# swoonge/SC-A-LOAM

Measured on AMD Instinct MI355X. Metric: scans/sec (feat-extract + scan-to-map ICP + SC loop search), KITTI HDL-64, higher is better.
Workload: dtype f32 points / f64 pose algebra

## Files before the change

### sc-a-loam_amd/csrc/common.cpp

```cpp
#include "common.hpp"
#include <atomic>
#include <chrono>
#include <cstdlib>
#include <memory>

namespace scal {

thread_local Recorder* g_recorder = nullptr;
long g_forced_flushes = 0;
static std::mutex g_flush_mu;
static std::vector<std::pair<std::string, long>> g_flush_sites;
void note_forced_flush(const char* file, int line) {
    std::lock_guard<std::mutex> lk(g_flush_mu);
    ++g_forced_flushes;
    const std::string key = std::string(file) + ":" + std::to_string(line);
    for (auto& s : g_flush_sites)
        if (s.first == key) {
            ++s.second;
            return;
        }
    g_flush_sites.push_back({key, 1});
}
void print_forced_flushes() {
    std::lock_guard<std::mutex> lk(g_flush_mu);
    for (auto& s : g_flush_sites) std::fprintf(stderr, "[scal_pipeline] forced flush at %s x %ld\n", s.first.c_str(), s.second);
}

static hipError_t run_op(const RecOp& o) {
    if (o.kind != RecOp::LAUNCH) return o.replay();
    const void* one = o.pack;
    return o.fn(o.name, o.grid, o.block, o.lds, o.stream, 1, &one);
}

hipError_t Recorder::flush() {
    Recorder* keep = g_recorder;
    g_recorder = nullptr;
    hipError_t first = hipSuccess;
    for (const RecOp& o : ops) {
        const hipError_t e = run_op(o);
        if (first == hipSuccess) first = e;
    }
    ops.clear();
    g_recorder = keep;
    return first;
}

namespace {
const char* merged_name(const char* a, const char* b) {
    static std::mutex mu;
    static std::vector<std::unique_ptr<std::string>> pool;
    const char* dot = std::strrchr(b, '.');
    const std::string key = std::string(a) + "+" + (dot ? dot + 1 : b);
    std::lock_guard<std::mutex> lk(mu);
    for (auto& s : pool)
        if (*s == key) return s->c_str();
    pool.push_back(std::make_unique<std::string>(key));
    return pool.back()->c_str();
}
struct Span {
    Recorder* r;
    size_t b, e;
};
bool same_op(const RecOp& a, const RecOp& b) {
    if (a.kind != b.kind) return false;
    if (a.kind != RecOp::LAUNCH) return true;
    return a.fn == b.fn && a.grid.x == b.grid.x && a.grid.y == b.grid.y && a.block.x == b.block.x && a.lds == b.lds && a.stream == b.stream &&
           a.pack_size == b.pack_size;
}
hipError_t zip_spans(const std::vector<Span>& spans) {
    hipError_t first = hipSuccess;
    auto note = [&](hipError_t e) { if (first == hipSuccess) first = e; };
    const int n = static_cast<int>(spans.size());
    std::vector<bool> done(n, false);
    for (int i = 0; i < n; ++i) {
        if (done[i]) continue;
        const Span& lead = spans[i];
        const size_t len = lead.e - lead.b;
        std::vector<const Span*> group{&lead};
        done[i] = true;
        if (!lead.r->broken)
            for (int j = i + 1; j < n && static_cast<int>(group.size()) < BATCH_WIDE; ++j) {
                const Span& c = spans[j];
                if (done[j] || c.r->broken || c.e - c.b != len) continue;
                bool ok = true;
                for (size_t k = 0; k < len && ok; ++k) ok = same_op(lead.r->ops[lead.b + k], c.r->ops[c.b + k]);
                if (ok) group.push_back(&c), done[j] = true;
            }
        for (size_t k = 0; k < len; ++k) {
            const RecOp& o = lead.r->ops[lead.b + k];
            if (o.kind == RecOp::LAUNCH) {
                for (size_t g0 = 0; g0 < group.size(); g0 += static_cast<size_t>(o.cap)) {
                    const size_t g1 = std::min(group.size(), g0 + static_cast<size_t>(o.cap));
                    const void* packs[BATCH_WIDE];
                    const char* name = o.name;
                    for (size_t g = g0; g < g1; ++g) {
                        const RecOp& og = group[g]->r->ops[group[g]->b + k];
                        packs[g - g0] = og.pack;
                        if (g > g0 && std::strcmp(og.name, o.name) != 0 && !std::strstr(name, "+")) name = merged_name(o.name, og.name);
                    }
                    note(o.fn(name, o.grid, o.block, o.lds, o.stream, static_cast<int>(g1 - g0), packs));
                }
            } else {
                for (const Span* g : group) note(g->r->ops[g->b + k].replay());
            }
        }
    }
    return first;
}
}

hipError_t zip_and_launch(Recorder* const* recs, int n) {
    Recorder* keep = g_recorder;
    g_recorder = nullptr;
    std::vector<Span> spans;
    for (int i = 0; i < n; ++i) spans.push_back({recs[i], 0, recs[i]->ops.size()});
    const hipError_t e = zip_spans(spans);
    for (int i = 0; i < n; ++i) recs[i]->ops.clear(), recs[i]->broken = false;
    g_recorder = keep;
    return e;
}

hipError_t zip_marked_and_launch(Recorder* const* recs, int n) {
    Recorder* keep = g_recorder;
    g_recorder = nullptr;
    std::vector<Span> before, seg, after;
    for (int i = 0; i < n; ++i) {
        Recorder* r = recs[i];
        size_t b = r->ops.size(), e = r->ops.size();
        for (size_t k = 0; k < r->ops.size(); ++k)
            if (r->ops[k].kind == RecOp::MARK_BEGIN) {
                b = k;
                break;
            }
        for (size_t k = b; k < r->ops.size(); ++k)
            if (r->ops[k].kind == RecOp::MARK_END) {
                e = k + 1;
                break;
            }
        if (r->broken || b == r->ops.size()) {
            before.push_back({r, 0, r->ops.size()});
            continue;
        }
        before.push_back({r, 0, b});
        seg.push_back({r, b, e});
        after.push_back({r, e, r->ops.size()});
    }
    hipError_t first = zip_spans(before);
    hipError_t e2 = zip_spans(seg);
    hipError_t e3 = zip_spans(after);
    if (first == hipSuccess) first = e2 != hipSuccess ? e2 : e3;
    for (int i = 0; i < n; ++i) recs[i]->ops.clear(), recs[i]->broken = false;
    g_recorder = keep;
    return first;
}

static thread_local char g_err[512] = "";

void set_error(const char* fmt, ...) {
    va_list ap;
    va_start(ap, fmt);
    vsnprintf(g_err, sizeof g_err, fmt, ap);
    va_end(ap);
}

int select_device(int device) {
    int n = 0;
    hipError_t e = hipGetDeviceCount(&n);
    if (e != hipSuccess || n <= 0) {
        set_error("no HIP device available (%s): libscaloam_hip has no CPU fallback", e == hipSuccess ? "count 0" : hipGetErrorString(e));
        return SCAL_E_NO_DEVICE;
    }
    if (device < 0 || device >= n) {
        set_error("device ordinal %d out of range (%d devices)", device, n);
        return SCAL_E_ARG;
    }
    hipDeviceProp_t prop;
    e = hipGetDeviceProperties(&prop, device);
    if (e != hipSuccess) {
        set_error("hipGetDeviceProperties failed: %s", hipGetErrorString(e));
        return SCAL_E_HIP;
    }
    if (std::strncmp(prop.gcnArchName, "gfx950", 6) != 0) {
        set_error("device %d is %s; this library carries gfx950 (MI355X) code objects only", device, prop.gcnArchName);
        return SCAL_E_NO_DEVICE;
    }
    e = hipSetDevice(device);
    if (e != hipSuccess) {
        set_error("hipSetDevice(%d) failed: %s", device, hipGetErrorString(e));
        return SCAL_E_HIP;
    }
    return SCAL_OK;
}

namespace {
std::mutex g_stream_mu;
struct DevStream {
    hipStream_t s = nullptr;
    int refs = 0;
};
DevStream g_streams[64][6];
std::atomic<int> g_stream_mode{0};

bool lane_has_own_queue(int lane) { return lane == 0 || lane == 1 || lane == 3 || lane == 4; }

hipStream_t own_queue_stream(int device) {
    int ncu = 0;
    if (hipDeviceGetAttribute(&ncu, hipDeviceAttributeMultiprocessorCount, device) != hipSuccess || ncu <= 0) return nullptr;
    std::vector<uint32_t> mask((ncu + 31) / 32, 0u);
    for (int cu = 0; cu < ncu; ++cu) mask[cu / 32] |= 1u << (cu % 32);
    hipStream_t s = nullptr;
    if (hipExtStreamCreateWithCUMask(&s, (uint32_t)mask.size(), mask.data()) != hipSuccess) {
        (void)hipGetLastError();
        return nullptr;
    }
    return s;
}
}

int acquire_stream(int device, hipStream_t* out, int lane) {
    if (device < 0 || device >= 64 || lane < 0 || lane > 5) {
        set_error("device ordinal %d out of range", device);
        return SCAL_E_ARG;
    }
    std::lock_guard<std::mutex> lk(g_stream_mu);
    DevStream& d = g_streams[device][lane];
    if (!d.s) {
        hipError_t e = hipSetDevice(device);
        if (e == hipSuccess && lane_has_own_queue(lane)) {
            d.s = own_queue_stream(device);
            if (!d.s) e = hipStreamCreateWithFlags(&d.s, hipStreamNonBlocking);
        } else if (e == hipSuccess) {
            e = hipStreamCreateWithFlags(&d.s, hipStreamNonBlocking);
        }
        if (e != hipSuccess) {
            set_error("hipStreamCreate failed: %s", hipGetErrorString(e));
            d.s = nullptr;
            return SCAL_E_HIP;
        }
    }
    d.refs++;
    *out = d.s;
    return SCAL_OK;
}

StreamLayout default_stream_layout() { return g_stream_mode.load() ? StreamLayout::PerStage : StreamLayout::Shared; }

int stage_lane(StreamLayout layout, int stage) {
    if (layout == StreamLayout::Shared) return stage == STAGE_MAP_PREFETCH ? 2 : 0;
    return (stage == STAGE_ODOM || stage == STAGE_SC) ? 3 : stage == STAGE_MAP ? 4 : (stage == STAGE_SC_FILTER || stage == STAGE_MAP_PREFETCH) ? 1 : 0;
}

__global__ void k_queue_ptr(unsigned long long* out) { out[0] = reinterpret_cast<unsigned long long>(__builtin_amdgcn_queue_ptr()); }

int lane_queue(int device, int lane, unsigned long long* out) {
    if (!out || device < 0 || device >= 64 || lane < -1 || lane > 5) {
        set_error("lane_queue: bad argument (device %d, lane %d)", device, lane);
        return SCAL_E_ARG;
    }
    hipStream_t s = nullptr;
    if (lane >= 0) {
        std::lock_guard<std::mutex> lk(g_stream_mu);
        DevStream& d = g_streams[device][lane];
        if (!d.s) {
            set_error("lane_queue: no context holds lane %d of device %d", lane, device);
            return SCAL_E_STATE;
        }
        d.refs++;
        s = d.s;
    }
    unsigned long long* dq = nullptr;
    hipError_t e = hipSetDevice(device);
    if (e == hipSuccess) e = hipMalloc(&dq, sizeof *dq);
    if (e == hipSuccess) {
        hipLaunchKernelGGL(k_queue_ptr, dim3(1), dim3(1), 0, s, dq);
        e = hipGetLastError();
    }
    if (e == hipSuccess) e = hipMemcpyAsync(out, dq, sizeof *dq, hipMemcpyDeviceToHost, s);
    if (e == hipSuccess) e = hipStreamSynchronize(s);
    if (dq) (void)hipFree(dq);
    if (lane >= 0) release_stream(device, lane);
    if (e != hipSuccess) {
        set_error("lane_queue: %s", hipGetErrorString(e));
        return SCAL_E_HIP;
    }
    return SCAL_OK;
}

void release_stream(int device, int lane) {
    if (device < 0 || device >= 64 || lane < 0 || lane > 5) return;
    std::lock_guard<std::mutex> lk(g_stream_mu);
    DevStream& d = g_streams[device][lane];
    if (d.refs > 0 && --d.refs == 0 && d.s) {
        (void)hipSetDevice(device);
        (void)hipStreamSynchronize(d.s);
        (void)hipStreamDestroy(d.s);
        d.s = nullptr;
    }
}

namespace {
struct ProfEntry {
    std::string name;
    std::vector<std::pair<hipEvent_t, hipEvent_t>> pending;
    std::vector<const void*> pending_tl;
    double total_ms = 0;
    long count = 0;
};
std::mutex g_prof_mu;
std::vector<ProfEntry> g_prof;
std::vector<hipEvent_t> g_event_pool;
bool g_prof_on = false;
std::string g_prof_filter;
struct TimelineRow {
    std::string name;
    float t0, t1;
    const void* stream;
};
bool g_timeline_on = false;
hipEvent_t g_timeline_base = nullptr;
std::vector<TimelineRow> g_timeline;

hipEvent_t take_event() {
    if (!g_event_pool.empty()) {
        hipEvent_t e = g_event_pool.back();
        g_event_pool.pop_back();
        return e;
    }
    hipEvent_t e = nullptr;
    (void)hipEventCreate(&e);
    return e;
}
void drain_entry(ProfEntry& p);
void drain_locked() {
    for (auto& p : g_prof) drain_entry(p);
}
void drain_entry(ProfEntry& p) {
    {
        for (size_t q = 0; q < p.pending.size(); ++q) {
            auto& ev = p.pending[q];
            float ms = 0.f;
            if (hipEventSynchronize(ev.second) == hipSuccess && hipEventElapsedTime(&ms, ev.first, ev.second) == hipSuccess) {
                p.total_ms += ms;
                p.count++;
                float a = 0.f;
                if (p.pending_tl[q] && g_timeline_base && hipEventElapsedTime(&a, g_timeline_base, ev.first) == hipSuccess)
                    g_timeline.push_back({p.name, a, a + ms, p.pending_tl[q]});
            }
            g_event_pool.push_back(ev.first);
            g_event_pool.push_back(ev.second);
        }
        p.pending.clear();
        p.pending_tl.clear();
    }
}
}

bool prof_begin(const char* name, hipStream_t stream, hipEvent_t* start, hipEvent_t* stop) {
    static const int delay_us = [] {
        const char* e = std::getenv("SCALOAM_HOST_DELAY_US");
        return e ? std::atoi(e) : 0;
    }();
    if (delay_us > 0) {
        const auto t0 = std::chrono::steady_clock::now();
        while (std::chrono::duration_cast<std::chrono::microseconds>(std::chrono::steady_clock::now() - t0).count() < delay_us) {
        }
    }
    if (!g_prof_on) return false;
    std::lock_guard<std::mutex> lk(g_prof_mu);
    if (!g_prof_filter.empty()) {
        const std::string f = "," + g_prof_filter + ",";
        if (f.find("," + std::string(name) + ",") == std::string::npos) return false;
    }
    int slot = -1;
    for (size_t i = 0; i < g_prof.size(); ++i)
        if (g_prof[i].name == name) slot = static_cast<int>(i);
    if (slot < 0) {
        g_prof.push_back(ProfEntry());
        g_prof.back().name = name;
        slot = static_cast<int>(g_prof.size()) - 1;
    }
    if (g_prof[slot].pending.size() >= 64) drain_entry(g_prof[slot]);
    hipEvent_t a = take_event(), b = take_event();
    if (!a || !b) return false;
    g_prof[slot].pending.push_back({a, b});
    g_prof[slot].pending_tl.push_back(g_timeline_on ? (stream ? static_cast<const void*>(stream) : static_cast<const void*>(&g_timeline_on)) : nullptr);
    *start = a, *stop = b;
    return true;
}

}

extern "C" int scal_prof_enable(int on) {
    std::lock_guard<std::mutex> lk(scal::g_prof_mu);
    scal::g_prof_on = on != 0;
    return SCAL_OK;
}
extern "C" int scal_prof_timeline(int on) {
    std::lock_guard<std::mutex> lk(scal::g_prof_mu);
    if (on && !scal::g_timeline_base) {
        if (hipEventCreate(&scal::g_timeline_base) != hipSuccess) return SCAL_E_HIP;
        if (hipEventRecord(scal::g_timeline_base, nullptr) != hipSuccess) return SCAL_E_HIP;
        if (hipEventSynchronize(scal::g_timeline_base) != hipSuccess) return SCAL_E_HIP;
    }
    scal::g_timeline_on = on != 0;
    return SCAL_OK;
}
extern "C" int scal_prof_timeline_dump(const char* path) {
    std::lock_guard<std::mutex> lk(scal::g_prof_mu);
    scal::drain_locked();
    FILE* f = std::fopen(path, "w");
    if (!f) return SCAL_E_ARG;
    for (auto& r : scal::g_timeline) std::fprintf(f, "%s,%.6f,%.6f,%p\n", r.name.c_str(), r.t0, r.t1, r.stream);
    std::fclose(f);
    scal::g_timeline.clear();
    return SCAL_OK;
}
extern "C" int scal_prof_filter(const char* kernel_name) {
    std::lock_guard<std::mutex> lk(scal::g_prof_mu);
    scal::g_prof_filter = kernel_name ? kernel_name : "";
    return SCAL_OK;
}
extern "C" int scal_prof_reset(void) {
    std::lock_guard<std::mutex> lk(scal::g_prof_mu);
    scal::drain_locked();
    for (auto& p : scal::g_prof) p.total_ms = 0, p.count = 0;
    return SCAL_OK;
}
extern "C" int scal_prof_read(const char* name, double* total_ms, long* count) {
    std::lock_guard<std::mutex> lk(scal::g_prof_mu);
    scal::drain_locked();
    for (auto& p : scal::g_prof)
        if (p.name == name) {
            if (total_ms) *total_ms = p.total_ms;
            if (count) *count = p.count;
            return SCAL_OK;
        }
    if (total_ms) *total_ms = 0;
    if (count) *count = 0;
    return SCAL_OK;
}
extern "C" int scal_prof_names(char* buf, int cap) {
    std::lock_guard<std::mutex> lk(scal::g_prof_mu);
    std::string all;
    for (auto& p : scal::g_prof) all += p.name + ";";
    if (buf && cap > 0) {
        std::strncpy(buf, all.c_str(), cap - 1);
        buf[cap - 1] = 0;
    }
    return static_cast<int>(all.size());
}

extern "C" int scal_set_stream_mode(int mode) {
    if (mode != 0 && mode != 1) {
        scal::set_error("scal_set_stream_mode: mode must be 0 or 1");
        return SCAL_E_ARG;
    }
    scal::g_stream_mode = mode;
    return SCAL_OK;
}

extern "C" int scal_debug_lane_queue(int device, int lane, unsigned long long* queue) { return scal::lane_queue(device, lane, queue); }

extern "C" const char* scal_last_error(void) { return scal::g_err; }
extern "C" int scal_device_count(void) {
    int n = 0;
    if (hipGetDeviceCount(&n) != hipSuccess) return -1;
    return n;
}
extern "C" const char* scal_version(void) { return "scaloam_hip 0.1 (gfx950)"; }
```

### sc-a-loam_amd/csrc/common.hpp

```cpp
#pragma once
#include <hip/hip_runtime.h>
#include <hip/hip_ext.h>
#include <cstdio>
#include <cstdarg>
#include <cstring>
#include <string>
#include <vector>
#include <utility>
#include <mutex>
#include "../../include/scaloam_hip.h"
#include "batch.hpp"

namespace scal {
constexpr unsigned EV_DEVICE_ONLY = hipEventDisableTiming | hipEventDisableSystemFence;


void set_error(const char* fmt, ...);

#define SCAL_HIP(expr)                                                                         \
    do {                                                                                       \
        hipError_t _e = (expr);                                                                \
        if (_e != hipSuccess) {                                                                \
            ::scal::set_error("%s failed: %s (%s:%d)", #expr, hipGetErrorString(_e), __FILE__, __LINE__); \
            return SCAL_E_HIP;                                                                 \
        }                                                                                      \
    } while (0)

#define SCAL_TRY(expr)           \
    do {                         \
        int _rc = (expr);        \
        if (_rc != SCAL_OK) return _rc; \
    } while (0)

int select_device(int device);
enum class StreamLayout { Shared, PerStage };
enum { STAGE_FEATURES = 0, STAGE_SC = 1, STAGE_ODOM = 3, STAGE_MAP = 4, STAGE_MAP_PREFETCH = 2, STAGE_SC_FILTER = 5 };
int stage_lane(StreamLayout layout, int stage);
StreamLayout default_stream_layout();
int acquire_stream(int device, hipStream_t* out, int lane = 0);
void release_stream(int device, int lane = 0);
int odom_create(const scal_odom_config* cfg, StreamLayout layout, scal_odom_t** out);
int map_create(const scal_map_config* cfg, StreamLayout layout, scal_map_t** out);
int sc_create(const scal_sc_config* cfg, StreamLayout layout, scal_sc_t** out);
int icp_create_on_lane(const scal_icp_config* cfg, int lane, scal_icp_t** out);
int refine_create_on_lane(const scal_refine_config* cfg, int lane, scal_refine_t** out);
int posegraph_create_on_lane(const scal_posegraph_config* cfg, int lane, scal_posegraph_t** out);
struct ScFilterOut {
    const float *x, *y, *z, *w;
    const int* d_n;
    int cap;
};
int sc_insert_features_then(scal_sc_t* ctx, scal_features_t* feat, int (*after)(void* user, hipStream_t s, const ScFilterOut& ds), void* user);

struct LaneStream {
    hipStream_t s = nullptr;
    int device = 0, lane = 0;
    LaneStream() = default;
    LaneStream(LaneStream&& o) noexcept { *this = std::move(o); }
    LaneStream& operator=(LaneStream&& o) noexcept {
        release();
        std::swap(s, o.s);
        device = o.device, lane = o.lane;
        return *this;
    }
    ~LaneStream() { release(); }
    operator hipStream_t() const { return s; }
    int acquire(int dev, int ln) {
        release();
        device = dev, lane = ln;
        return acquire_stream(dev, &s, ln);
    }
    void release() {
        if (s) release_stream(device, lane);
        s = nullptr;
    }
};
struct Event {
    hipEvent_t e = nullptr;
    Event() = default;
    Event(Event&& o) noexcept { *this = std::move(o); }
    Event& operator=(Event&& o) noexcept {
        reset();
        std::swap(e, o.e);
        return *this;
    }
    ~Event() { reset(); }
    operator hipEvent_t() const { return e; }
    int create(unsigned flags) {
        reset();
        return ensure(flags);
    }
    int ensure(unsigned flags) {
        const hipError_t r = e ? hipSuccess : hipEventCreateWithFlags(&e, flags);
        if (r == hipSuccess) return SCAL_OK;
        set_error("hipEventCreateWithFlags failed: %s", hipGetErrorString(r));
        e = nullptr;
        return SCAL_E_HIP;
    }
    void reset() {
        if (e) (void)hipEventDestroy(e);
        e = nullptr;
    }
};

template <class T>
struct DevBuf {
    T* p = nullptr;
    size_t n = 0;
    DevBuf() = default;
    DevBuf(const DevBuf&) = delete;
    DevBuf& operator=(const DevBuf&) = delete;
    ~DevBuf() { release(); }
    void release() {
        if (p) (void)hipFree(p);
        p = nullptr;
        n = 0;
    }
    int alloc(size_t count) {
        release();
        if (count == 0) count = 1;
        hipError_t e = hipMalloc(reinterpret_cast<void**>(&p), count * sizeof(T));
        if (e != hipSuccess) {
            set_error("hipMalloc(%zu bytes) failed: %s", count * sizeof(T), hipGetErrorString(e));
            p = nullptr;
            return SCAL_E_HIP;
        }
        n = count;
        return SCAL_OK;
    }
    int zero(hipStream_t s) {
        hipError_t e = op_memset_async(p, 0, n * sizeof(T), s);
        if (e != hipSuccess) {
            set_error("hipMemsetAsync failed: %s", hipGetErrorString(e));
            return SCAL_E_HIP;
        }
        return SCAL_OK;
    }
};

template <class T>
struct PinBuf {
    T* p = nullptr;
    size_t n = 0;
    PinBuf() = default;
    PinBuf(const PinBuf&) = delete;
    PinBuf& operator=(const PinBuf&) = delete;
    ~PinBuf() {
        if (p) (void)hipHostFree(p);
    }
    int alloc(size_t count) {
        if (p) (void)hipHostFree(p);
        p = nullptr;
        if (count == 0) count = 1;
        hipError_t e = hipHostMalloc(reinterpret_cast<void**>(&p), count * sizeof(T), hipHostMallocDefault);
        if (e != hipSuccess) {
            set_error("hipHostMalloc(%zu bytes) failed: %s", count * sizeof(T), hipGetErrorString(e));
            p = nullptr;
            return SCAL_E_HIP;
        }
        n = count;
        return SCAL_OK;
    }
};

inline int div_up(int a, int b) { return (a + b - 1) / b; }

struct HostStage {
    PinBuf<unsigned char> pin;
    size_t used = 0;
    struct Item {
        void* dst;
        size_t off, bytes;
    };
    std::vector<Item> items;
    bool reserve(size_t total) {
        if (pin.p && pin.n >= total) return true;
        if (used) return false;
        if (pin.alloc(total) != SCAL_OK) {
            (void)hipGetLastError();
            return false;
        }
        return true;
    }
    hipError_t d2h(void* user, const void* dev, size_t bytes, hipStream_t s) {
        if (!bytes) return hipSuccess;
        const size_t need = (bytes + 255) & ~static_cast<size_t>(255);
        if (!pin.p || used + need > pin.n) return hipMemcpyAsync(user, dev, bytes, hipMemcpyDeviceToHost, s);
        const hipError_t e = hipMemcpyAsync(pin.p + used, dev, bytes, hipMemcpyDeviceToHost, s);
        items.push_back({user, used, bytes});
        used += need;
        return e;
    }
    hipError_t h2d(void* dev, const void* user, size_t bytes, hipStream_t s) {
        if (!bytes) return hipSuccess;
        const size_t need = (bytes + 255) & ~static_cast<size_t>(255);
        if (!pin.p || used + need > pin.n) return hipMemcpyAsync(dev, user, bytes, hipMemcpyHostToDevice, s);
        std::memcpy(pin.p + used, user, bytes);
        const hipError_t e = hipMemcpyAsync(dev, pin.p + used, bytes, hipMemcpyHostToDevice, s);
        used += need;
        return e;
    }
    void finish() {
        for (const Item& it : items) std::memcpy(it.dst, pin.p + it.off, it.bytes);
        items.clear();
        used = 0;
    }
};

bool prof_begin(const char* name, hipStream_t stream, hipEvent_t* start, hipEvent_t* stop);

#define SCAL_LAUNCH_PROF(name, kernel, grid, block, lds, stream, ...)                                   \
    do {                                                                                                \
        hipEvent_t pe0_ = nullptr, pe1_ = nullptr;                                                      \
        if (::scal::prof_begin(name, stream, &pe0_, &pe1_))                                                     \
            hipExtLaunchKernelGGL(kernel, grid, block, lds, stream, pe0_, pe1_, 0, __VA_ARGS__);        \
        else                                                                                            \
            hipLaunchKernelGGL(kernel, grid, block, lds, stream, __VA_ARGS__);                          \
    } while (0)

}
```

### sc-a-loam_amd/csrc/mapping.hip

```cpp
#include "common.hpp"
#include <mutex>
#include <atomic>
#include "device_utils.hpp"
#include "voxel_dev.hpp"
#include "radix_sort.hpp"
#include "lm_host.hpp"
#include "features_dev.hpp"
#include <cmath>
#include <cstdlib>
#include <algorithm>
#include <deque>

namespace scal {

constexpr int CW = 21, CH = 21, CD = 11;
constexpr int GX = 250, GY = 250, GZ = 150;
constexpr int GCELLS = GX * GY * GZ;
constexpr unsigned long long MAP_NOMERGE = 127ull;

struct MapParams {
    int cenW, cenH, cenD;
    int cI, cJ, cK;
    int ox, oy, oz;
    float inv_line, inv_plane;
// ... 1016 lines not shown
            int cnt = 1;
            if (!key_nomerge(k)) {
                bool run = true;
#pragma unroll
                for (int j = 0; j < 8; ++j)
                    if (j >= cn) {
                        run = run && (e[j] >> MERGE_IDX_BITS) == k;
                        if (run) {
                            const int jn = static_cast<int>(e[j] & (MERGE_MAX - 1));
                            ax += nw.x[jn], ay += nw.y[jn], az += nw.z[jn], aw += nw.w[jn];
                            ++cnt;
                        }
                    }
                if (run) {
                    int u = lo + 8;
                    while (u < n_eff && (nw.sorted[u] >> MERGE_IDX_BITS) == k) {
                        const int jn = static_cast<int>(nw.sorted[u] & (MERGE_MAX - 1));
                        ax += nw.x[jn], ay += nw.y[jn], az += nw.z[jn], aw += nw.w[jn];
                        ++u, ++cnt;
                    }
                }
            }
            const float c = static_cast<float>(cnt);
            const float ox = ax / c, oy = ay / c, oz = az / c;
            out.x[o] = ox, out.y[o] = oy, out.z[o] = oz, out.w[o] = aw / c, out.cube[o] = cube;
            if (a.prebuild) prebuild(o, ox, oy, oz, cube, k);
        }
    } else {
        const int i = b * 256 + threadIdx.x;
        if (i < n_eff && (nw.hm[i] & 3) == 1) {
            const unsigned long long k = nw.sorted[i] >> MERGE_IDX_BITS;
            const int o = nw.lb[i] + pre_at(i);
            float ax = 0.f, ay = 0.f, az = 0.f, aw = 0.f;
            int u = i;
            do {
                const int j = static_cast<int>(nw.sorted[u] & (MERGE_MAX - 1));
                ax += nw.x[j], ay += nw.y[j], az += nw.z[j], aw += nw.w[j];
                ++u;
            } while (!key_nomerge(k) && u < n_eff && (nw.sorted[u] >> MERGE_IDX_BITS) == k);
            const float c = static_cast<float>(u - i);
            const int cube = nw.cube[static_cast<int>(nw.sorted[i] & (MERGE_MAX - 1))];
            const float ox = ax / c, oy = ay / c, oz = az / c;
            out.x[o] = ox, out.y[o] = oy, out.z[o] = oz, out.w[o] = aw / c;
            out.cube[o] = cube;
            if (a.prebuild) prebuild(o, ox, oy, oz, cube, k);
        }
    }
    if (!a.prebuild) return;
    if (drifted) S->next_unsorted = 1;
    if (over) S->next_over = 1;
    for (int o = 32; o >= 1; o >>= 1) n_in += __shfl_xor(n_in, o, 64);
    if (lane_id() == 0 && n_in) atomicAdd(&s_valid, n_in);
    __syncthreads();
    if (threadIdx.x == 0 && s_valid) atomicAdd(&S->next_valid[cls], s_valid);
}

struct MapResult {
    LMState st;
    MapCounters C1, C2;
    MapState S1, S2;
    unsigned seq_pose, seq_done;
};

struct MergeTail {
    int fused;
    unsigned seq;
    CSoA4 full;
    const int* d_nfull;
    int full_cap;
    const LMState* st;
    SoA4 full_out;
};
__device__ __forceinline__ void k_merge_write_body(const MergeArgs& a, MapState* S, MapCounters* C, const MergeTail& t) {
    merge_write_body(a, S, C);
    if (!t.fused) return;
    if (static_cast<int>(blockIdx.x) >= MERGE_WRITE_GRID && S->pose_seq == t.seq) {
        const int i = (blockIdx.x - MERGE_WRITE_GRID) * 256 + threadIdx.x;
        if (i < min(*t.d_nfull, t.full_cap)) {
            double x7[7];
#pragma unroll
            for (int k = 0; k < 7; ++k) x7[k] = t.st->x[k];
            float sel[3];
            associate_to_map(x7, t.full.x[i], t.full.y[i], t.full.z[i], sel);
            t.full_out.x[i] = sel[0], t.full_out.y[i] = sel[1], t.full_out.z[i] = sel[2], t.full_out.w[i] = t.full.w[i];
        }
    }
}
SCAL_KERNEL(256, k_merge_write)

__device__ __forceinline__ void k_transform_cloud_body(const CSoA4& in, const int* __restrict__ d_n, int cap, const LMState* __restrict__ st,
                                                         const MapState* __restrict__ S, const SoA4& out) {
    if (S->abort) return;
    const int i = blockIdx.x * blockDim.x + threadIdx.x;
    if (i >= min(*d_n, cap)) return;
    double x7[7];
#pragma unroll
    for (int k = 0; k < 7; ++k) x7[k] = st->x[k];
    float sel[3];
    associate_to_map(x7, in.x[i], in.y[i], in.z[i], sel);
    out.x[i] = sel[0], out.y[i] = sel[1], out.z[i] = sel[2], out.w[i] = in.w[i];
}
SCAL_KERNEL(256, k_transform_cloud)

__device__ __forceinline__ void k_map_gather_body(const float* __restrict__ less_aos, const int* __restrict__ d_n_less, const CSoA4& less_flat,
                                                    const int* __restrict__ d_n_less_flat, const SoA4& corner_in, const SoA4& surf_in, MapCounters* C, int cap,
                                                    int nbc, unsigned* surf_parts) {
    const bool corner = static_cast<int>(blockIdx.x) < nbc;
    const int b = corner ? blockIdx.x : blockIdx.x - nbc;
    const int n = min(corner ? *d_n_less : *d_n_less_flat, cap);
    const int i = b * 256 + threadIdx.x;
    if (blockIdx.x == 0) {
        int* w = reinterpret_cast<int*>(C);
        for (int t = 2 + threadIdx.x; t < static_cast<int>(sizeof(MapCounters) / sizeof(int)); t += 256) w[t] = 0;
    }
    if (i == 0) (corner ? C->n_corner_in : C->n_surf_in) = n;
    if (corner) {
        if (i >= n) return;
        const float4 p = reinterpret_cast<const float4*>(less_aos)[i];
        corner_in.x[i] = p.x, corner_in.y[i] = p.y, corner_in.z[i] = p.z, corner_in.w[i] = p.w;
    } else {
        float x = 0.f, y = 0.f, z = 0.f;
        if (i < n) {
            x = less_flat.x[i], y = less_flat.y[i], z = less_flat.z[i];
            surf_in.x[i] = x, surf_in.y[i] = y, surf_in.z[i] = z, surf_in.w[i] = less_flat.w[i];
        }
        if (surf_parts) vox_bbox_block_store(surf_parts, b, i < n, x, y, z);
    }
}
SCAL_KERNEL(256, k_map_gather)

__device__ __forceinline__ void k_export_valid_body(const MapCloud& m, const MapState* __restrict__ S, int cls, int* __restrict__ counter,
                                                      float* __restrict__ out, int cap) {
    const MapParams mp = S->mp;
    const int n = S->n_map[cls];
    for (int i = blockIdx.x * blockDim.x + threadIdx.x; i < n; i += gridDim.x * blockDim.x)
        if (cube_valid(mp, m.cube[i])) {
            const int p = atomicAdd(counter, 1);
            if (p < cap) reinterpret_cast<float4*>(out)[p] = make_float4(m.x[i], m.y[i], m.z[i], m.w[i]);
        }
}
SCAL_KERNEL(256, k_export_valid)


__device__ __forceinline__ void copy_words(void* dst, const void* src, int bytes) {
    const unsigned* s = static_cast<const unsigned*>(src);
    unsigned* d = static_cast<unsigned*>(dst);
    for (int i = threadIdx.x; i < bytes / 4; i += blockDim.x) d[i] = s[i];
}

struct PoseDoneNew {
    CSoA4 stack[2];
    const int* d_ns[2];
    float inv_leaf[2];
    float *x[2], *y[2], *z[2], *w[2];
    int* cube[2];
    unsigned long long* pkey[2];
};
struct MapPoseDone {
    int active;
    unsigned seq;
    MapState* S;
    const LMState* st;
    MapCounters* C;
    MapResult* host;
    PoseDoneNew nw;
    __device__ __forceinline__ void operator()(const double* x, int first, int stride, bool aborted) const {
        if (!active) return;
        const bool stop = aborted || S->abort;
        if (!stop) {
            const MapParams mp = S->mp;
            double x7[7];
#pragma unroll
            for (int k = 0; k < 7; ++k) x7[k] = x[k];
#pragma unroll
            for (int cls = 0; cls < 2; ++cls) {
                const int n_new = min(*nw.d_ns[cls], MERGE_MAX);
                const CSoA4 stack = nw.stack[cls];
                for (int i = first; i < n_new; i += stride) {
                    float sel[3];
                    associate_to_map(x7, stack.x[i], stack.y[i], stack.z[i], sel);
                    const int pc = pack_cube(cube_abs(sel[0]), cube_abs(sel[1]), cube_abs(sel[2]));
                    const unsigned long long k = map_key(mp, nw.inv_leaf[cls], sel[0], sel[1], sel[2], pc, C);
                    nw.x[cls][i] = sel[0], nw.y[cls][i] = sel[1], nw.z[cls][i] = sel[2], nw.w[cls][i] = stack.w[i], nw.cube[cls][i] = pc;
                    nw.pkey[cls][i] = k == ~0ull ? ~0ull : ((k << MERGE_IDX_BITS) | static_cast<unsigned long long>(i));
                }
            }
        }
        if (blockIdx.x != 0) return;
        if (first == 0 && !stop) {
            const double* q_wodom = S->q_wodom;
            const double n2 = q_wodom[0] * q_wodom[0] + q_wodom[1] * q_wodom[1] + q_wodom[2] * q_wodom[2] + q_wodom[3] * q_wodom[3];
            const double qi[4] = {-q_wodom[0] / n2, -q_wodom[1] / n2, -q_wodom[2] / n2, q_wodom[3] / n2};
            double qn[4];
            q_mul(x, qi, qn);
            double r2[3];
            q_rot(qn, S->t_wodom, r2);
#pragma unroll
            for (int i = 0; i < 4; ++i) S->q_wmap_wodom[i] = qn[i];
#pragma unroll
            for (int i = 0; i < 3; ++i) S->t_wmap_wodom[i] = x[4 + i] - r2[i];
            S->pose_seq = seq;
        }
        __syncthreads();
        copy_words(&host->st, st, sizeof(LMState));
        copy_words(&host->C1, C, sizeof(MapCounters));
        copy_words(&host->S1, S, sizeof(MapState));
        __threadfence_system();
        __syncthreads();
        if (threadIdx.x == 0) __hip_atomic_store(&host->seq_pose, seq, __ATOMIC_RELEASE, __HIP_MEMORY_SCOPE_SYSTEM);
    }
    __device__ __forceinline__ void operator()(int, int, int) const {}
};

__device__ __forceinline__ void k_map_pose_done_body(const MapPoseDone& pd) {
    pd(pd.st->x, blockIdx.x * blockDim.x + threadIdx.x, gridDim.x * blockDim.x, false);
}
SCAL_KERNEL(256, k_map_pose_done)

__device__ __forceinline__ void k_map_end_body(MapState* S, const MapCounters* C, MapResult* host, unsigned seq) {
    if (threadIdx.x == 0 && !S->abort) S->n_map[0] = C->n_map_new[0], S->n_map[1] = C->n_map_new[1];
    __syncthreads();
    copy_words(&host->C2, C, sizeof(MapCounters));
    copy_words(&host->S2, S, sizeof(MapState));
    __threadfence_system();
    __syncthreads();
    if (threadIdx.x == 0) __hip_atomic_store(&host->seq_done, seq, __ATOMIC_RELEASE, __HIP_MEMORY_SCOPE_SYSTEM);
}
SCAL_KERNEL(256, k_map_end)

struct MapStore {
    SoAStore pts[2];
    DevBuf<int> cube[2];
    int n = 0;
    MapCloud cloud(int b) { return MapCloud{pts[b].x.p, pts[b].y.p, pts[b].z.p, pts[b].w.p, cube[b].p}; }
};

struct GridStore {
    DevBuf<int2> cell[2];
    DevBuf<int> rank[2];
    DevBuf<float4> g;
    DevBuf<float4> fixed[2];
    DevBuf<unsigned long long> okeys[2];
    int fixed_cap = 0;
    GridPts pts(int par, bool fixed_pool = false) { return GridPts{fixed_pool ? fixed[par].p : g.p}; }
};

SCAL_DEFINE_STAMP_READER(scal_debug_stamps_map)
}

using namespace scal;

int voxels_per_cell_axis(float leaf) {
    const double inv = 1.0 / static_cast<double>(leaf);
    int most = 1;
    for (int c = 0; c < 1000; ++c) {
        const int lo = static_cast<int>(std::floor(c * inv + 1e-4)), hi = static_cast<int>(std::floor((c + 1) * inv - 1e-4));
        most = std::max(most, hi - lo + 1);
    }
    return most;
}


struct MapStep {
    scal_features_t* feat = nullptr;
    MapPoseIn pose{};
    int set = 0;
    int slot = 0;
    int par = 0;
    bool prefetched = false, have_full = false, fast = false;
    bool pose_collected = false;
    bool confirmed = false;
    bool failed = false;
    bool prebuilt = false;
    unsigned seq = 0;
    unsigned feat_generation = 0;
    int n_corner_bound = 0, n_surf_bound = 0;
    int insert_path = 0;
};

struct InputSet {
    SoAStore in[2], stack[2];
    DevBuf<MapCounters> C;
    DevBuf<unsigned> surf_parts;
    Event ev_pre;
    Event ev_pre_a;
    int* n_in(int k) const { return k == 0 ? &C.p->n_corner_in : &C.p->n_surf_in; }
    int* n_stack(int k) const { return k == 0 ? &C.p->n_corner_stack : &C.p->n_surf_stack; }
};

template <class T, int N>
struct Fifo {
    T item[N];
    int n = 0;
    void push(const T& v) { item[n++] = v; }
    const T& front() const { return item[0]; }
    void pop() { std::copy(item + 1, item + n, item), --n; }
    void clear() { n = 0; }
};

struct scal_map {
    scal_map_config cfg;
    LaneStream stream;
    LaneStream side;
    static constexpr int NSETS = 8;
    static constexpr int MAX_STEPS = 4;
    static constexpr int MAX_PF = 3;
    static constexpr int NSLOTS = MAX_STEPS + 1;
    struct Prefetch {
        scal_features_t* feat;
        int set;
        unsigned generation;
    };
    std::mutex pf_mu;
    Fifo<Prefetch, MAX_PF> pf_half;
    Fifo<Prefetch, MAX_PF> pf;
    int next_set = 0;
    std::deque<MapStep> steps;
    Event ev_pose[NSLOTS], ev_done[NSLOTS];
    int next_slot = 0;
    PinBuf<MapResult> res;
    bool adapter_active = false;
    MapStep adapter_step;
    BlockAdapter blocks;
    int n_fast = 0, n_general = 0, n_recover_pose = 0, n_recover_insert = 0;
    bool poll_on_enqueue = true;
    int cur = 0;
    bool initialised = false;
    double good_q[4] = {0, 0, 0, 1}, good_t[3] = {0, 0, 0};
    int scan_cap = 0, map_cap = 0;
    double q_wmap_wodom[4] = {0, 0, 0, 1}, t_wmap_wodom[3] = {0, 0, 0};
    bool have_mp = false;
    DevBuf<MapState> d_S;
    DevBuf<float> aos;
    DevBuf<float> export_buf;
    InputSet sets[NSETS];
    SoAStore full_in, full_out;
    float leaf(int k) const { return k == 0 ? cfg.line_res : cfg.plane_res; }
    float inv_leaf(int k) const { return 1.0f / leaf(k); }
    VoxelFilter vf, vf_side, vf_corner;
    MapStore map[2];
    GridStore grid[2];
    HostStage hs_reg;
    bool grid_fixed = false;
    unsigned seq_counter = 0;
    bool grid_prebuilt = false;
    int grid_cap_now[2] = {0, 0};
    RadixSort sorter;
    DevBuf<unsigned long long> keys;
    DevBuf<int> vals, blockcnt;
    bool merge_insert = true;
    int last_insert_path = 0;
    SoAStore mnew[2];
    DevBuf<int> mcube[2], mpre[2], mlb[2], mblocktot[2];
    DevBuf<unsigned long long> msorted[2], mpkey[2], msamp[2];
    DevBuf<unsigned char> mhm[2];
    MergeNew merge_new(int k) {
        return MergeNew{mnew[k].x.p, mnew[k].y.p, mnew[k].z.p, mnew[k].w.p, mcube[k].p, mpkey[k].p, msorted[k].p, msamp[k].p, mpre[k].p, mlb[k].p, mhm[k].p, mblocktot[k].p};
    }
    LMStore lm;
    DevBuf<float> nnrec;
    NNBuf nnbuf() { return NNBuf{nnrec.p, lm.slot_cap}; }
    DevBuf<int> d_nfull;
    PinBuf<MapCounters> h_C;
    PinBuf<MapState> h_S;
    PinBuf<int> h_misc;
    int alloc_set() {
        const int st = next_set;
        next_set = (next_set + 1) % NSETS;
        return st;
    }
};

int scal::map_create(const scal_map_config* cfg, StreamLayout layout, scal_map_t** out) {
    if (!cfg || !out || cfg->max_scan_points <= 0 || cfg->max_map_points <= 0 || !(cfg->line_res > 0) || !(cfg->plane_res > 0)) {
        set_error("scal_map_create: bad argument");
        return SCAL_E_ARG;
    }
    if (cfg->line_res < 0.11f || cfg->plane_res < 0.11f) {
        set_error("mapping resolutions below 0.11 m exceed the 512 voxel/cube key layout");
        return SCAL_E_ARG;
    }
    *out = nullptr;
    SCAL_TRY(select_device(cfg->device));
    auto* c = new scal_map();
    c->cfg = *cfg;
    c->scan_cap = cfg->max_scan_points;
    c->map_cap = cfg->max_map_points;
    int rc = SCAL_OK;
    auto A = [&](int r) { if (rc == SCAL_OK) rc = r; };
    const size_t sc = c->scan_cap, mc = c->map_cap;
    A(c->aos.alloc(sc * 4));
    for (InputSet& I : c->sets) {
        A(I.in[0].alloc(sc)); A(I.in[1].alloc(sc)); A(I.stack[0].alloc(sc)); A(I.stack[1].alloc(sc));
        A(I.C.alloc(1));
        A(I.surf_parts.alloc((size_t)6 * (div_up(c->scan_cap, 256) + 1)));
    }
    A(c->full_in.alloc(sc)); A(c->full_out.alloc(sc));
    A(c->vf.init(c->scan_cap));
    A(c->vf_side.init(c->scan_cap));
    A(c->vf_corner.init(c->scan_cap));
    c->vf.set_tag(".C"), c->vf_side.set_tag(".C"), c->vf_corner.set_tag(".C");
    for (int k = 0; k < 2; ++k) {
        for (int b = 0; b < 2; ++b) {
            A(c->map[k].pts[b].alloc(mc));
            A(c->map[k].cube[b].alloc(mc));
        }
        for (int par = 0; par < 2; ++par) { A(c->grid[k].cell[par].alloc(GCELLS)); A(c->grid[k].rank[par].alloc(mc)); A(c->grid[k].okeys[par].alloc(mc)); }
        A(c->grid[k].g.alloc(mc));
    }
    A(c->sorter.init(c->map_cap));
    A(c->keys.alloc(mc)); A(c->vals.alloc(mc)); A(c->blockcnt.alloc(div_up(c->map_cap, 256) + 1));
    for (int k = 0; k < 2; ++k) {
        A(c->mnew[k].alloc(MERGE_MAX)); A(c->mcube[k].alloc(MERGE_MAX)); A(c->mpre[k].alloc(MERGE_MAX + 1)); A(c->mlb[k].alloc(MERGE_MAX));
        A(c->msorted[k].alloc(MERGE_MAX)); A(c->mhm[k].alloc(MERGE_MAX)); A(c->mblocktot[k].alloc(MERGE_CHUNKS));
        A(c->mpkey[k].alloc(MERGE_MAX)); A(c->msamp[k].alloc(MERGE_MAX / 8));
    }
    A(c->lm.alloc(c->scan_cap));
    A(c->nnrec.alloc(16 * sc));
    A(c->d_S.alloc(1)); A(c->d_nfull.alloc(4));
    A(c->blocks.alloc(c->scan_cap));
    A(c->h_C.alloc(1)); A(c->h_S.alloc(1)); A(c->h_misc.alloc(4)); A(c->res.alloc(scal_map::NSLOTS));
    const char* fixed_env = std::getenv("SCALOAM_MAP_FIXED_GRID");
    if (rc == SCAL_OK && !(fixed_env && fixed_env[0] == '0')) {
        int cap[2];
        for (int k = 0; k < 2; ++k) {
            const int a = voxels_per_cell_axis(c->leaf(k));
            cap[k] = a * a * a;
        }
        if (cap[0] + cap[1] <= 48) {
            c->grid_fixed = true;
            for (int k = 0; k < 2 && c->grid_fixed; ++k) {
                for (int par = 0; par < 2; ++par)
                    if (c->grid[k].fixed[par].alloc(static_cast<size_t>(GCELLS) * cap[k]) != SCAL_OK) c->grid_fixed = false;
                c->grid[k].fixed_cap = c->grid_cap_now[k] = cap[k];
            }
            if (!c->grid_fixed) {
                (void)hipGetLastError();
                for (int k = 0; k < 2; ++k) c->grid[k].fixed[0].release(), c->grid[k].fixed[1].release();
            }
        }
    }
    if (rc == SCAL_OK) std::memset(static_cast<void*>(c->res.p), 0, sizeof(MapResult) * scal_map::NSLOTS);
    if (rc == SCAL_OK) rc = lm_check_residency<AssocFit, MapPoseDone>(c->cfg.device);
    if (rc == SCAL_OK && hipFuncSetAttribute(reinterpret_cast<const void*>(k_merge_keys), hipFuncAttributeMaxDynamicSharedMemorySize,
                                             static_cast<int>(sizeof(unsigned long long) * MERGE_MAX)) != hipSuccess)
        rc = SCAL_E_HIP;
    if (rc == SCAL_OK) rc = c->stream.acquire(c->cfg.device, stage_lane(layout, STAGE_MAP));
    if (rc == SCAL_OK) rc = c->side.acquire(c->cfg.device, stage_lane(layout, STAGE_MAP_PREFETCH));
    for (int k = 0; k < scal_map::NSLOTS && rc == SCAL_OK; ++k) {
        rc = c->ev_pose[k].create(hipEventDisableTiming);
        if (rc == SCAL_OK) rc = c->ev_done[k].create(hipEventDisableTiming);
    }
    if (rc == SCAL_OK) {
        for (int k = 0; k < 4 && rc == SCAL_OK; ++k) rc = c->grid[k & 1].cell[k >> 1].zero(c->stream);
        if (rc == SCAL_OK) rc = c->lm.init(c->stream);
        MapState& H = *c->h_S.p;
        std::memset(&H, 0, sizeof H);
        H.q_wmap_wodom[3] = 1.0;
        H.mp.cenW = 10, H.mp.cenH = 10, H.mp.cenD = 5;
        if (rc == SCAL_OK && op_memcpy_async(c->d_S.p, c->h_S.p, sizeof(MapState), hipMemcpyHostToDevice, c->stream) != hipSuccess) rc = SCAL_E_HIP;
        if (rc == SCAL_OK && op_stream_synchronize(c->stream) != hipSuccess) rc = SCAL_E_HIP;
    }
    if (rc != SCAL_OK) {
        if (rc == SCAL_E_HIP) set_error("scal_map_create: HIP resource creation failed");
        delete c;
        return rc;
    }
    *out = c;
    return SCAL_OK;
}

extern "C" int scal_map_create(const scal_map_config* cfg, scal_map_t** out) { return map_create(cfg, default_stream_layout(), out); }

extern "C" void scal_map_destroy(scal_map_t* c) {
    if (!c) return;
    (void)hipSetDevice(c->cfg.device);
    if (c->stream) (void)op_stream_synchronize(c->stream);
    if (c->side) (void)op_stream_synchronize(c->side);
    delete c;
}

namespace {

void copy_pose(double* q, double* t, const double* q_from, const double* t_from) {
    std::copy(q_from, q_from + 4, q);
    std::copy(t_from, t_from + 3, t);
}

int enqueue_stack_filter(scal_map* c, int k, VoxelFilter& vf, hipStream_t s, int n_bound, int st, bool surf_box_done = false) {
    InputSet& I = c->sets[st];
    VoxTail t;
    t.err_out = &I.C.p->error;
    const int bits = c->leaf(k) >= 0.35f ? 30 : 40;
    const bool box = k == 1 && surf_box_done && n_bound > 8192;
    return vf.run(s, I.in[k].cv(), I.n_in(k), n_bound, c->leaf(k), bits, I.stack[k].v(), I.n_stack(k), &t, box ? I.surf_parts.p : nullptr,
                  box ? std::max(1, div_up(n_bound, 256)) : 0);
}

GridArgs grid_args(scal_map* c, int par, bool fixed_pool = false) {
    GridArgs ga;
    for (int k = 0; k < 2; ++k) {
        GridStore& G = c->grid[k];
        ga.m[k] = c->map[k].cloud(par);
        ga.cell[k] = G.cell[par].p, ga.rank[k] = G.rank[par].p, ga.g[k] = G.pts(par, fixed_pool);
        ga.okeys[k] = G.okeys[par].p;
        ga.inv_leaf[k] = c->inv_leaf(k);
    }
    return ga;
}

int insert_full_sort(scal_map* c, const MapStep& e, const int* n_map) {
    hipStream_t s = c->stream;
    const InputSet& I = c->sets[e.set];
    MapCounters* C = I.C.p;
    LMState* st = c->lm.d_st.p;
    for (int k = 0; k < 2; ++k) {
        MapStore& M = c->map[k];
        const int n_tot_max = std::min(c->map_cap, n_map[k] + c->scan_cap);
        const int nb = std::max(1, div_up(n_tot_max, 256));
        MapCloud in = M.cloud(e.par), outc = M.cloud(e.par ^ 1);
        SCAL_LAUNCH("k_insert_keys", k_insert_keys, dim3(nb), dim3(256), 0, s, in, c->d_S.p, I.stack[k].cv(), I.n_stack(k), st, c->inv_leaf(k),
                           c->map_cap, c->keys.p, c->vals.p, C, k);
        SortedPairs sp;
        SCAL_TRY(c->sorter.sort(s, c->keys.p, c->vals.p, &C->n_total[k], n_tot_max, 36, nullptr, &sp));
        SCAL_LAUNCH("k_map_heads", k_map_heads, dim3(nb), dim3(256), 0, s, sp, &C->n_total[k], c->blockcnt.p);
        launch_scan_inplace(s, c->blockcnt.p, &C->n_total[k], 256, 1, &C->n_map_new[k]);
        SCAL_LAUNCH("k_map_reduce", k_map_reduce, dim3(nb), dim3(256), 0, s, sp, &C->n_total[k], c->blockcnt.p, in, outc);
    }
    SCAL_HIP(hipGetLastError());
    return SCAL_OK;
}

struct FullCloud {
    CSoA4 pts;
    const int* d_n;
};
FullCloud full_cloud(scal_map* c, const MapStep& e) {
    if (!(e.have_full && e.feat)) return FullCloud{c->full_in.cv(), c->d_nfull.p};
    FeatDeviceView v = features_view(e.feat);
    return FullCloud{CSoA4{v.x, v.y, v.z, v.i}, &v.P->n_kept};
}

int launch_insert_merge(scal_map* c, const MapStep& e, bool fused = false) {
    hipStream_t s = c->stream;
    const InputSet& I = c->sets[e.set];
    MapCounters* C = I.C.p;
    MergeArgs a;
    for (int k = 0; k < 2; ++k) {
        MapStore& M = c->map[k];
        a.in[k] = M.cloud(e.par), a.out[k] = M.cloud(e.par ^ 1);
        a.stack[k] = I.stack[k].cv();
        a.d_ns[k] = I.n_stack(k);
        a.inv_leaf[k] = c->inv_leaf(k);
        GridStore& G = c->grid[k];
        a.okeys[k] = G.okeys[e.par].p;
        a.nw[k] = c->merge_new(k);
        a.grid_cell[k] = G.cell[e.par].p, a.grid_rank[k] = G.rank[e.par].p;
        a.next_cell[k] = G.cell[e.par ^ 1].p, a.next_rank[k] = G.rank[e.par ^ 1].p, a.next_pool[k] = G.fixed[e.par ^ 1].p;
        a.next_okeys[k] = G.okeys[e.par ^ 1].p, a.next_cap[k] = c->grid_cap_now[k];
    }
    a.prebuild = fused && c->grid_fixed ? 1 : 0;
    a.cap = c->map_cap;
    const int lds = sizeof(unsigned long long) * MERGE_MAX;
    if (!(fused && c->grid_fixed)) SCAL_LAUNCH("k_merge_okeys", k_merge_okeys, dim3(MERGE_KB0 + MERGE_KB1), dim3(1024), 0, s, a, c->d_S.p, C);
    SCAL_LAUNCH("k_merge_keys", k_merge_keys, dim3(MERGE_KEYS_GRID), dim3(1024), lds, s, a, c->lm.d_st.p, c->d_S.p, C);
    SCAL_LAUNCH("k_merge_lookup", k_merge_lookup, dim3(2 * MERGE_CHUNKS), dim3(512), 0, s, a, c->d_S.p, C);
    MergeTail t{};
    int grid = MERGE_WRITE_GRID;
    if (fused) {
        t.fused = 1, t.seq = e.seq, t.st = c->lm.d_st.p, t.full_out = c->full_out.v(), t.full_cap = c->scan_cap;
        const FullCloud f = full_cloud(c, e);
        t.full = f.pts, t.d_nfull = f.d_n;
        if (e.have_full) grid += std::max(1, div_up(c->scan_cap, 256));
        else t.full_cap = 0;
    }
    SCAL_LAUNCH("k_merge_write", k_merge_write, dim3(grid), dim3(256), 0, s, a, c->d_S.p, C, t);
    SCAL_HIP(hipGetLastError());
    return SCAL_OK;
}

void launch_grid_clear(scal_map* c, int par) {
    SCAL_LAUNCH("k_grid_clear", k_grid_clear, dim3(GRID_BLOCKS), dim3(256), 0, c->stream, grid_args(c, par), c->d_S.p);
}
int clear_abort(scal_map* c) {
    hipStream_t s = c->stream;
    SCAL_HIP(op_memset_async(&c->d_S.p->abort, 0, sizeof(int), s));
    return SCAL_OK;
}
void launch_map_end(scal_map* c, const MapStep& e) {
    SCAL_LAUNCH("k_map_end", k_map_end, dim3(1), dim3(256), 0, c->stream, c->d_S.p, c->sets[e.set].C.p, c->res.p + e.slot, e.seq);
}
bool stopped_before_pose(const MapResult& R) { return R.S1.abort || R.st.termination == 5; }
bool stopped_in_insertion(const MapResult& R) { return R.S2.abort != 0; }

int launch_tail(scal_map* c, const MapStep& e, bool registered = false) {
    hipStream_t s = c->stream;
    if (e.have_full && !registered) {
        const int nb = std::max(1, div_up(c->scan_cap, 256));
        const FullCloud f = full_cloud(c, e);
        SCAL_LAUNCH("k_transform_cloud", k_transform_cloud, dim3(nb), dim3(256), 0, s, f.pts, f.d_n, c->scan_cap, c->lm.d_st.p, c->d_S.p, c->full_out.v());
    }
    launch_map_end(c, e);
    SCAL_HIP(hipGetLastError());
    SCAL_HIP(op_event_record(c->ev_done[e.slot], s));
    if (e.feat && !registered) SCAL_TRY(features_note_reader(e.feat, s));
    return SCAL_OK;
}

MapPoseDone make_pose_done(scal_map* c, const MapStep& e) {
    const InputSet& I = c->sets[e.set];
    MapPoseDone pd;
    pd.active = 1, pd.seq = e.seq;
    pd.S = c->d_S.p, pd.st = c->lm.d_st.p, pd.C = I.C.p, pd.host = c->res.p + e.slot;
    for (int k = 0; k < 2; ++k) {
        pd.nw.stack[k] = I.stack[k].cv();
        pd.nw.d_ns[k] = I.n_stack(k);
        pd.nw.inv_leaf[k] = c->inv_leaf(k);
        pd.nw.x[k] = c->mnew[k].x.p, pd.nw.y[k] = c->mnew[k].y.p, pd.nw.z[k] = c->mnew[k].z.p, pd.nw.w[k] = c->mnew[k].w.p;
        pd.nw.cube[k] = c->mcube[k].p, pd.nw.pkey[k] = c->mpkey[k].p;
    }
    return pd;
}

int launch_pose_part(scal_map* c, const MapStep& e, bool prepare_only = false) {
    hipStream_t s = c->stream;
    const int st_ = e.set;
    InputSet& I = c->sets[st_];
    MapCounters* C = I.C.p;
    LMState* st = c->lm.d_st.p;
    MapState* S = c->d_S.p;
    if (e.feat) {
        if (e.prefetched) {
            SCAL_HIP(op_stream_wait_event(s, I.ev_pre, 0));
        } else {
            FeatDeviceView v = features_view(e.feat);
            SCAL_TRY(features_wait_done(e.feat, s));
            const int nbc = std::max(1, div_up(e.n_corner_bound, 256));
            SCAL_LAUNCH("k_map_gather", k_map_gather, dim3(nbc + std::max(1, div_up(e.n_surf_bound, 256))), dim3(256), 0, s, v.less_xyzi, &v.P->n_less_sharp,
                               CSoA4{v.lfx, v.lfy, v.lfz, v.lfi}, &v.P->n_less_flat, I.in[0].v(), I.in[1].v(), C, c->scan_cap, nbc,
                               static_cast<unsigned*>(nullptr));
        }
    }
    if (!e.prefetched) {
        SCAL_TRY(enqueue_stack_filter(c, 0, c->vf, s, e.n_corner_bound, st_));
        SCAL_TRY(enqueue_stack_filter(c, 1, c->vf, s, e.n_surf_bound, st_));
    }
    MapBeginArgs mb;
    mb.active = 0, mb.in = e.pose, mb.allow_window_change = e.fast ? 0 : 1, mb.inv_line = c->inv_leaf(0), mb.inv_plane = c->inv_leaf(1);
    mb.slot_cap = c->lm.slot_cap, mb.prebuilt = e.prebuilt ? 1 : 0, mb.S = S;
    const bool begin_in_knn = e.fast && e.prebuilt && c->grid_fixed && !prepare_only;
    if (!begin_in_knn) SCAL_LAUNCH("k_map_begin", k_map_begin, dim3(1), dim3(64), 0, s, mb, st, C);
    const bool fixed_pool = e.fast && c->grid_fixed && !prepare_only;
    const GridArgs ga = grid_args(c, e.par, fixed_pool);
    if (fixed_pool) {
        if (!e.prebuilt) SCAL_LAUNCH("k_grid_build", k_grid_build, dim3(GRID_BLOCKS), dim3(256), 0, s, ga, c->grid_cap_now[0], c->grid_cap_now[1], S, C);
    } else {
        SCAL_LAUNCH("k_grid_count", k_grid_count, dim3(GRID_BLOCKS), dim3(256), 0, s, ga, S, C);
        SCAL_LAUNCH("k_grid_alloc", k_grid_alloc, dim3(GRID_BLOCKS), dim3(256), 0, s, ga, S, C);
        SCAL_LAUNCH("k_grid_fill", k_grid_fill, dim3(GRID_BLOCKS), dim3(256), 0, s, ga, S);
    }
    if (prepare_only) {
        SCAL_HIP(hipGetLastError());
        return SCAL_OK;
    }
    FactorSoA F = c->lm.factors();
    const int assoc_blocks = std::max(1, std::min(3072, div_up(c->lm.slot_cap, 8)));
    MapPoseDone pd = make_pose_done(c, e);
    const AssocFit fit{I.stack[0].cv(), I.stack[1].cv(), c->nnbuf(), C, F};
    for (int outer = 0; outer < 2; ++outer) {
        {
            mb.active = (begin_in_knn && outer == 0) ? 1 : 0;
            SCAL_LAUNCH(mb.active ? "k_assoc_knn.0" : "k_assoc_knn", k_assoc_knn, dim3(assoc_blocks), dim3(256), 0, s, I.stack[0].cv(), I.stack[1].cv(), S,
                             c->grid[0].cell[e.par].p, c->grid[0].pts(e.par, fixed_pool), c->grid[1].cell[e.par].p, c->grid[1].pts(e.par, fixed_pool), st, C, c->nnbuf(), mb);
        }
        pd.active = outer == 1;
        launch_lm_solve(s, F, &C->n_slots, st, &C->solve_on, c->lm.partials.p, c->lm.lm_sync.p, outer, &S->abort, fit, pd, "k_lm_solve_map");
    }
    SCAL_HIP(hipGetLastError());
    if (!e.fast) SCAL_HIP(op_event_record(c->ev_pose[e.slot], s));
    return SCAL_OK;
}

static bool step_flag_set(const volatile unsigned* w, unsigned seq) {
    if (*w != seq) return false;
    std::atomic_thread_fence(std::memory_order_acquire);
    return true;
}
static int step_flag_wait(scal_map* c, const volatile unsigned* w, unsigned seq) {
    if (g_recorder) SCAL_HIP(op_flush_for_wait(__FILE__, __LINE__));
    for (unsigned spins = 0;; ++spins) {
        if (step_flag_set(w, seq)) return SCAL_OK;
        if ((spins & 0xfff) == 0xfff && hipStreamQuery(c->stream) == hipSuccess) {
            if (step_flag_set(w, seq)) return SCAL_OK;
            set_error("scal_map: the stream is idle and the step never reported (a kernel launch failed?)");
            return SCAL_E_HIP;
        }
        __builtin_ia32_pause();
    }
}
static int wait_pose(scal_map* c, const MapStep& e) {
    if (e.fast) return step_flag_wait(c, &c->res.p[e.slot].seq_pose, e.seq);
    SCAL_HIP(op_event_synchronize(c->ev_pose[e.slot]));
    return SCAL_OK;
}
static int wait_done(scal_map* c, const MapStep& e) {
    if (e.fast) return step_flag_wait(c, &c->res.p[e.slot].seq_done, e.seq);
    SCAL_HIP(op_event_synchronize(c->ev_done[e.slot]));
    return SCAL_OK;
}
static bool done_ready(scal_map* c, const MapStep& e) {
    if (e.fast) return step_flag_set(&c->res.p[e.slot].seq_done, e.seq);
    return op_event_query(c->ev_done[e.slot]) == hipSuccess;
}

int report_device_error(scal_map* c, int err) {
    set_error("scal_map_step: device capacity exceeded (map pool of %d points per class, or a voxel outside its cube)", c->map_cap);
    return err;
}

constexpr int MAP_RC_LM = 1000;
bool lm_gave_up(const MapResult& R) { return R.st.termination == 5 || R.S1.abort == MAP_ABORT_LM; }
int lm_reset(scal_map* c, bool restore_pose) {
    hipStream_t s = c->stream;
    SCAL_TRY(c->lm.clear_exchange(s));
    SCAL_TRY(clear_abort(c));
    if (restore_pose) {
        static_assert(offsetof(MapState, t_wmap_wodom) == offsetof(MapState, q_wmap_wodom) + 4 * sizeof(double), "pose fields are contiguous");
        SCAL_TRY(c->blocks.set_pose(s, c->d_S.p->q_wmap_wodom, c->good_q, c->good_t));
    }
    SCAL_HIP(op_stream_synchronize(s));
    return SCAL_OK;
}

int general_insert(scal_map* c, MapStep& e);
int drop_prebuilt_grid(scal_map* c) {
    if (!c->grid_prebuilt) return SCAL_OK;
    launch_grid_clear(c, c->cur);
    SCAL_HIP(hipGetLastError());
    c->grid_prebuilt = false;
    return SCAL_OK;
}
int run_general_once(scal_map* c, MapStep& e) {
    e.fast = false, e.prebuilt = false;
    e.par = c->cur;
    e.seq = ++c->seq_counter;
    SCAL_TRY(drop_prebuilt_grid(c));
    c->n_general++;
    SCAL_TRY(launch_pose_part(c, e));
    SCAL_HIP(op_event_synchronize(c->ev_pose[e.slot]));
    if (lm_gave_up(c->res.p[e.slot])) return MAP_RC_LM;
    return general_insert(c, e);
}
int run_general(scal_map* c, MapStep& e) {
    int rc = run_general_once(c, e);
    for (int attempt = 0; rc == MAP_RC_LM; ++attempt) {
        SCAL_TRY(lm_reset(c, true));
        launch_grid_clear(c, e.par);
        if (attempt == 1) {
            SCAL_HIP(op_stream_synchronize(c->stream));
            e.failed = true;
            set_error("LM solve abandoned: grid barrier timed out");
            return SCAL_E_HIP;
        }
        rc = run_general_once(c, e);
    }
    return rc;
}

int finish_step_sync(scal_map* c, MapStep& e, const int* n_map_before, bool registered) {
    if (n_map_before) {
        e.insert_path = 0;
        SCAL_TRY(insert_full_sort(c, e, n_map_before));
    }
    SCAL_TRY(launch_tail(c, e, registered));
    SCAL_HIP(op_event_synchronize(c->ev_done[e.slot]));
    const MapResult& R = c->res.p[e.slot];
    if (R.C2.error) return report_device_error(c, R.C2.error);
    c->cur = e.par ^ 1;
    return SCAL_OK;
}

// ... 68 lines not shown
}

int recover(scal_map* c) {
    hipStream_t s = c->stream;
    SCAL_HIP(op_stream_synchronize(s));
    size_t origin = 0;
    for (; origin < c->steps.size(); ++origin) {
        MapStep& f = c->steps[origin];
        if (f.confirmed) continue;
        const MapResult& Rf = c->res.p[f.slot];
        if (stopped_before_pose(Rf) || stopped_in_insertion(Rf)) break;
        if (Rf.C2.error) return report_device_error(c, Rf.C2.error);
        confirm(c, f);
    }
    if (origin == c->steps.size()) return SCAL_OK;
    MapStep& e = c->steps[origin];
    const MapResult& R = c->res.p[e.slot];
    trace_stop(R);
    c->cur = e.par;
    c->grid_prebuilt = false;
    bool dropped = false;
    if (stopped_before_pose(R)) {
        c->n_recover_pose++;
        const bool lm = lm_gave_up(R);
        if (lm) SCAL_TRY(lm_reset(c, true));
        else SCAL_TRY(clear_abort(c));
        if (lm || R.S1.abort == MAP_ABORT_GRID || e.prebuilt) launch_grid_clear(c, e.par);
        SCAL_TRY(check_generation(e, !e.prefetched));
        const int rc = run_general(c, e);
        if (rc != SCAL_OK && !e.failed) return rc;
        dropped = e.failed;
    } else {
        c->n_recover_insert++;
        const bool lm = R.S2.abort == MAP_ABORT_LM;
        if (lm) {
            SCAL_TRY(lm_reset(c, false));
            launch_grid_clear(c, e.par);
        } else {
            SCAL_TRY(clear_abort(c));
        }
        const bool registered = R.S2.pose_seq == e.seq;
        if (!registered) SCAL_TRY(check_generation(e, false));
        const int n_map[2] = {R.S2.n_map[0], R.S2.n_map[1]};
        e.fast = false;
        SCAL_TRY(finish_step_sync(c, e, n_map, registered));
    }
    if (dropped) e.confirmed = true;
    else confirm(c, e);
    for (size_t i = origin + 1; i < c->steps.size(); ++i) {
        SCAL_TRY(check_generation(c->steps[i], !c->steps[i].prefetched));
        SCAL_TRY(launch_fast(c, c->steps[i]));
    }
    return SCAL_OK;
}

int confirm_steps(scal_map* c, bool wait) {
    for (size_t i = 0; i < c->steps.size(); ++i) {
        if (c->steps[i].confirmed) continue;
        if (wait) {
            SCAL_TRY(wait_done(c, c->steps[i]));
        } else if (!done_ready(c, c->steps[i])) {
            break;
        }
        const MapResult& R = c->res.p[c->steps[i].slot];
        if (stopped_before_pose(R) || stopped_in_insertion(R)) {
            SCAL_TRY(recover(c));
            if (!c->steps[i].confirmed) {
                set_error("scal_map: internal error (recovery did not complete the stopped step)");
                return SCAL_E_STATE;
            }
            continue;
        }
        confirm(c, c->steps[i]);
        if (R.C2.error) return report_device_error(c, R.C2.error);
    }
    return SCAL_OK;
}
int map_settle(scal_map* c, bool wait) {
    SCAL_TRY(confirm_steps(c, wait));
    pop_done(c);
    return SCAL_OK;
}
int map_make_room(scal_map* c) {
    if (c->poll_on_enqueue) SCAL_TRY(map_settle(c, false));
    while (static_cast<int>(c->steps.size()) >= scal_map::MAX_STEPS) {
        if (!c->steps.front().pose_collected) {
            set_error("scal_map: %d steps are queued and not collected", scal_map::MAX_STEPS);
            return SCAL_E_STATE;
        }
        SCAL_TRY(wait_done(c, c->steps.front()));
        SCAL_TRY(map_settle(c, false));
    }
    return SCAL_OK;
}

MapStep new_step(scal_map* c) {
    MapStep e;
    e.slot = c->next_slot;
    c->next_slot = (c->next_slot + 1) % scal_map::NSLOTS;
    return e;
}

int run_general_and_confirm(scal_map* c, MapStep& e) {
    SCAL_TRY(run_general(c, e));
    c->steps.push_back(e);
    confirm(c, c->steps.back());
    return SCAL_OK;
}

int map_enqueue(scal_map* c, MapStep& e) {
    const int queued = static_cast<int>(c->steps.size()) + 1;
    const bool room = c->map[0].n + queued * MERGE_MAX <= c->map_cap && c->map[1].n + queued * MERGE_MAX <= c->map_cap;
    const bool fast = c->initialised && c->merge_insert && room && e.feat != nullptr;
    if (fast) {
        SCAL_TRY(launch_fast(c, e));
        c->steps.push_back(e);
        return SCAL_OK;
    }
    SCAL_TRY(map_settle(c, true));
    return run_general_and_confirm(c, e);
}

void stats_at_pose(const MapCounters& H, scal_map_stats* stats) {
    std::memset(stats, 0, sizeof *stats);
    stats->n_corner_stack = H.n_corner_stack, stats->n_surf_stack = H.n_surf_stack;
    stats->n_corner_map = H.n_valid[0], stats->n_surf_map = H.n_valid[1];
    stats->solved = H.solve_on;
}

void publish_correction(scal_map* c, const MapState& S1) {
    copy_pose(c->q_wmap_wodom, c->t_wmap_wodom, S1.q_wmap_wodom, S1.t_wmap_wodom);
    c->have_mp = true;
}

int map_collect_pose(scal_map* c, double* q_out, double* t_out, scal_map_stats* stats) {
    MapStep* pe = nullptr;
    for (auto& e : c->steps)
        if (!e.pose_collected) {
            pe = &e;
            break;
        }
    if (!pe) {
        set_error("scal_map_collect: no step enqueued");
        return SCAL_E_STATE;
    }
    const int slot = pe->slot;
    for (int round = 0;; ++round) {
        SCAL_TRY(wait_pose(c, *pe));
        if (pe->failed || !stopped_before_pose(c->res.p[slot])) break;
        if (round > scal_map::MAX_STEPS + 1) {
            set_error("scal_map_collect: internal error (recovery does not converge)");
            return SCAL_E_STATE;
        }
        SCAL_TRY(recover(c));
    }
    pe->pose_collected = true;
    const MapResult& R = c->res.p[slot];
    const MapCounters& H = R.C1;
    if (pe->failed) {
        pop_done(c);
        set_error("LM solve abandoned: grid barrier timed out");
        return SCAL_E_HIP;
    }
    if (H.error) return report_device_error(c, H.error);
    copy_pose(q_out, t_out, R.st.x, R.st.x + 4);
    publish_correction(c, R.S1);
    if (stats) {
        stats_at_pose(H, stats);
        for (int o = 0; o < 2; ++o) {
            const LMState& L = R.st;
            stats->n_edge[o] = H.solve_on ? L.log_n_edge[o] : 0, stats->n_plane[o] = H.solve_on ? L.log_n_plane[o] : 0;
            stats->lm_iters[o] = H.solve_on ? L.log_iters[o] : 0, stats->lm_success[o] = H.solve_on ? L.log_success[o] : 0;
            stats->cost_init[o] = H.solve_on ? L.log_cost_init[o] : 0.0, stats->cost_final[o] = H.solve_on ? L.log_cost_final[o] : 0.0;
        }
        stats->n_map_corner_total = R.S1.n_map[0], stats->n_map_surf_total = R.S1.n_map[1];
        stats->insert_path = -1;
    }
    pop_done(c);
    return SCAL_OK;
}

int check_host_arrays(const char* fn, const scal_map* c, const float* corner_last, int n_corner, const float* surf_last, int n_surf, int n_full,
                      const double* q_wodom, const double* t_wodom, const double* q_w_curr, const double* t_w_curr) {
    if (!c || !q_wodom || !t_wodom || !q_w_curr || !t_w_curr || n_corner < 0 || n_surf < 0 || n_full < 0 || (n_corner > 0 && !corner_last) ||
        (n_surf > 0 && !surf_last)) {
        set_error("%s: bad argument", fn);
        return SCAL_E_ARG;
    }
    if (n_corner > c->scan_cap || n_surf > c->scan_cap || n_full > c->scan_cap) {
        set_error("%s: input cloud larger than max_scan_points (%d)", fn, c->scan_cap);
        return SCAL_E_TOO_MANY;
    }
    return SCAL_OK;
}

void drop_prefetches(scal_map* c) { c->pf.clear(), c->pf_half.clear(); }

int begin_sync_step(scal_map* c, bool adapter_counts, const char* open_text, MapStep* e) {
    SCAL_HIP(hipSetDevice(c->cfg.device));
    SCAL_TRY(map_settle(c, true));
    if (!c->steps.empty() || (adapter_counts && c->adapter_active)) {
        set_error("%s", open_text);
        return SCAL_E_STATE;
    }
    *e = new_step(c);
    std::lock_guard<std::mutex> lk(c->pf_mu);
    drop_prefetches(c);
    e->set = c->alloc_set();
    return SCAL_OK;
}

int upload_step_inputs(scal_map* c, MapStep& e, const float* corner_last, int n_corner, const float* surf_last, int n_surf, const float* full_res,
                       int n_full) {
    hipStream_t s = c->stream;
    InputSet& I = c->sets[e.set];
    MapCounters z;
    std::memset(&z, 0, sizeof z);
    z.n_corner_in = n_corner, z.n_surf_in = n_surf;
    *c->h_C.p = z;
    SCAL_HIP(op_memcpy_async(I.C.p, c->h_C.p, sizeof(MapCounters), hipMemcpyHostToDevice, s));
    c->h_misc.p[0] = n_full;
    SCAL_HIP(op_memcpy_async(c->d_nfull.p, c->h_misc.p, sizeof(int), hipMemcpyHostToDevice, s));
    auto up = [&](const float* src, int n, SoAStore& dst) -> int {
        if (n > 0) {
            SCAL_HIP(op_memcpy_async(c->aos.p, src, sizeof(float) * 4 * n, hipMemcpyHostToDevice, s));
            launch_deinterleave(s, c->aos.p, n, dst.v());
            SCAL_HIP(op_stream_synchronize(s));
        }
        return SCAL_OK;
    };
    SCAL_TRY(up(corner_last, n_corner, I.in[0]));
    SCAL_TRY(up(surf_last, n_surf, I.in[1]));
    if (n_full > 0) SCAL_TRY(up(full_res, n_full, c->full_in));
    e.have_full = n_full > 0, e.n_corner_bound = n_corner, e.n_surf_bound = n_surf;
    return SCAL_OK;
}

int download_registered(scal_map* c, float* registered, int n_full) {
    hipStream_t s = c->stream;
    launch_interleave(s, c->d_nfull.p, n_full, c->full_out.cv(), c->aos.p);
    (void)c->hs_reg.reserve((size_t)c->scan_cap * 16 + 4096);
    SCAL_HIP(c->hs_reg.d2h(registered, c->aos.p, sizeof(float) * 4 * n_full, s));
    SCAL_HIP(op_stream_synchronize(s));
    c->hs_reg.finish();
    return SCAL_OK;
}

void stats_after_insertion(const scal_map* c, scal_map_stats* stats) {
    if (!stats) return;
    stats->n_map_corner_total = c->map[0].n, stats->n_map_surf_total = c->map[1].n;
    stats->insert_path = c->last_insert_path;
}

int need_adapter_step(const scal_map* c, const char* fn) {
    if (c->adapter_active) return SCAL_OK;
    set_error("%s: no scal_map_adapter_begin", fn);
    return SCAL_E_STATE;
}

int check_features_device(const scal_map* c, const FeatDeviceView& v) {
    if (v.device == c->cfg.device) return SCAL_OK;
    set_error("features context lives on device %d, map context on %d", v.device, c->cfg.device);
    return SCAL_E_ARG;
}

}

extern "C" int scal_map_step(scal_map_t* c, const float* corner_last, int n_corner, const float* surf_last, int n_surf, const float* full_res,
                             int n_full, const double* q_wodom, const double* t_wodom, double* q_w_curr, double* t_w_curr, float* registered,
                             scal_map_stats* stats) {
    SCAL_TRY(check_host_arrays("scal_map_step", c, corner_last, n_corner, surf_last, n_surf, n_full, q_wodom, t_wodom, q_w_curr, t_w_curr));
    const bool have_full = full_res != nullptr && n_full > 0;
    MapStep e;
    SCAL_TRY(begin_sync_step(c, false, "scal_map_step: a queued step has not been collected", &e));
    SCAL_TRY(upload_step_inputs(c, e, corner_last, n_corner, surf_last, n_surf, full_res, have_full ? n_full : 0));
    copy_pose(e.pose.q_wodom, e.pose.t_wodom, q_wodom, t_wodom);
    SCAL_TRY(run_general_and_confirm(c, e));
    SCAL_TRY(map_collect_pose(c, q_w_curr, t_w_curr, stats));
    SCAL_TRY(map_settle(c, true));
    stats_after_insertion(c, stats);
    if (have_full && registered) SCAL_TRY(download_registered(c, registered, n_full));
    return SCAL_OK;
}

extern "C" int scal_map_prefetch_begin(scal_map_t* c, scal_features_t* feat) {
    if (!c || !feat) {
        set_error("scal_map_prefetch_begin: null argument");
        return SCAL_E_ARG;
    }
    FeatDeviceView v = features_view(feat);
    SCAL_TRY(check_features_device(c, v));
    SCAL_HIP(hipSetDevice(c->cfg.device));
    const int ls_cap = std::min(c->scan_cap, v.n_scans * 120);
    const int cap = std::min(c->scan_cap, v.cap);
    std::lock_guard<std::mutex> lk(c->pf_mu);
    if (c->pf.n + c->pf_half.n >= scal_map::MAX_PF) {
        set_error("scal_map_prefetch_features: %d prefetches are already queued ahead of their steps", scal_map::MAX_PF);
        return SCAL_E_STATE;
    }
    const int nset = c->alloc_set();
    InputSet& I = c->sets[nset];
    SCAL_TRY(I.ev_pre.ensure(EV_DEVICE_ONLY));
    SCAL_TRY(I.ev_pre_a.ensure(EV_DEVICE_ONLY));
    hipStream_t sa = v.stream;
    const int nbc = std::max(1, div_up(ls_cap, 256));
    SCAL_LAUNCH("k_map_gather", k_map_gather, dim3(nbc + std::max(1, div_up(cap, 256))), dim3(256), 0, sa, v.less_xyzi, &v.P->n_less_sharp,
                     CSoA4{v.lfx, v.lfy, v.lfz, v.lfi}, &v.P->n_less_flat, I.in[0].v(), I.in[1].v(), I.C.p, c->scan_cap, nbc, I.surf_parts.p);
    SCAL_HIP(hipGetLastError());
    SCAL_TRY(enqueue_stack_filter(c, 0, c->vf_corner, sa, ls_cap, nset));
    SCAL_HIP(op_event_record(I.ev_pre_a, sa));
    c->pf_half.push(scal_map::Prefetch{feat, nset, v.generation});
    return SCAL_OK;
}

extern "C" int scal_map_prefetch_finish(scal_map_t* c, scal_features_t* feat) {
    if (!c || !feat) {
        set_error("scal_map_prefetch_finish: null argument");
        return SCAL_E_ARG;
    }
    SCAL_HIP(hipSetDevice(c->cfg.device));
    FeatDeviceView v = features_view(feat);
    const int cap = std::min(c->scan_cap, v.cap);
    std::lock_guard<std::mutex> lk(c->pf_mu);
    if (c->pf_half.n == 0 || c->pf_half.front().feat != feat) {
        set_error("scal_map_prefetch_finish: no scal_map_prefetch_begin of this features context is waiting (halves are finished in the order they were begun)");
        return SCAL_E_STATE;
    }
    const scal_map::Prefetch h = c->pf_half.front();
    c->pf_half.pop();
    InputSet& I = c->sets[h.set];
    SCAL_HIP(op_stream_wait_event(c->side, I.ev_pre_a, 0));
    SCAL_TRY(enqueue_stack_filter(c, 1, c->vf_side, c->side, cap, h.set, true));
    SCAL_HIP(op_event_record(I.ev_pre, c->side));
    c->pf.push(h);
    return SCAL_OK;
}

extern "C" int scal_map_prefetch_features(scal_map_t* c, scal_features_t* feat) {
    SCAL_TRY(scal_map_prefetch_begin(c, feat));
    return scal_map_prefetch_finish(c, feat);
}

static int map_enqueue_features(scal_map* c, scal_features_t* feat, const double* q_wodom, const double* t_wodom) {
    FeatDeviceView v = features_view(feat);
    SCAL_TRY(check_features_device(c, v));
    SCAL_HIP(hipSetDevice(c->cfg.device));
    SCAL_TRY(map_make_room(c));
    MapStep e = new_step(c);
    e.feat = feat;
    e.feat_generation = v.generation;
    e.n_corner_bound = std::min(c->scan_cap, v.n_scans * 120);
    e.n_surf_bound = std::min(c->scan_cap, v.cap);
    e.have_full = true;
    copy_pose(e.pose.q_wodom, e.pose.t_wodom, q_wodom, t_wodom);
    {
        std::lock_guard<std::mutex> lk(c->pf_mu);
        if (c->pf.n > 0 && c->pf.front().feat == feat) {
            if (c->pf.front().generation != v.generation) {
                drop_prefetches(c);
                set_error("scal_map_enqueue_features: the features context was run again between scal_map_prefetch_features and this call");
                return SCAL_E_STATE;
            }
            e.prefetched = true;
            e.set = c->pf.front().set;
            c->pf.pop();
        } else {
            drop_prefetches(c);
            e.set = c->alloc_set();
        }
    }
    return map_enqueue(c, e);
}

extern "C" int scal_map_step_features(scal_map_t* c, scal_features_t* feat, const double* q_wodom, const double* t_wodom, double* q_w_curr,
                                      double* t_w_curr, scal_map_stats* stats) {
    if (!c || !feat || !q_wodom || !t_wodom || !q_w_curr || !t_w_curr) {
        set_error("scal_map_step_features: null argument");
        return SCAL_E_ARG;
    }
    SCAL_TRY(map_enqueue_features(c, feat, q_wodom, t_wodom));
    SCAL_TRY(map_collect_pose(c, q_w_curr, t_w_curr, stats));
    SCAL_TRY(map_settle(c, true));
    stats_after_insertion(c, stats);
    return SCAL_OK;
}

extern "C" int scal_map_enqueue_features(scal_map_t* c, scal_features_t* feat, const double* q_wodom, const double* t_wodom) {
    if (!c || !feat || !q_wodom || !t_wodom) {
        set_error("scal_map_enqueue_features: null argument");
        return SCAL_E_ARG;
    }
    return map_enqueue_features(c, feat, q_wodom, t_wodom);
}

extern "C" int scal_map_collect(scal_map_t* c, double* q_w_curr, double* t_w_curr, scal_map_stats* stats) {
    if (!c || !q_w_curr || !t_w_curr) {
        set_error("scal_map_collect: null argument");
        return SCAL_E_ARG;
    }
    SCAL_HIP(hipSetDevice(c->cfg.device));
    return map_collect_pose(c, q_w_curr, t_w_curr, stats);
}

extern "C" int scal_map_finish(scal_map_t* c) {
    if (!c) return SCAL_E_ARG;
    SCAL_HIP(hipSetDevice(c->cfg.device));
    return map_settle(c, true);
}

extern "C" int scal_map_export(scal_map_t* c, int which, float* out_xyzi, int cap) {
    if (!c || (which != 0 && which != 1) || cap < 0) {
        set_error("scal_map_export: bad argument");
        return SCAL_E_ARG;
    }
    SCAL_HIP(hipSetDevice(c->cfg.device));
    if (map_settle(c, true) != SCAL_OK) return -1;
    if (!c->have_mp || c->map[which].n == 0) return 0;
    hipStream_t s = c->stream;
    MapStore& M = c->map[which];
    c->h_misc.p[1] = 0;
    SCAL_HIP(op_memcpy_async(c->d_nfull.p + 1, c->h_misc.p + 1, sizeof(int), hipMemcpyHostToDevice, s));
    if (out_xyzi && c->export_buf.n < static_cast<size_t>(c->map_cap) * 4) SCAL_TRY(c->export_buf.alloc(static_cast<size_t>(c->map_cap) * 4));
    const int room = std::min(cap, c->map_cap);
    SCAL_LAUNCH("k_export_valid", k_export_valid, dim3(std::max(1, std::min(1024, div_up(M.n, 256)))), dim3(256), 0, s, M.cloud(c->cur), c->d_S.p, which,
                       c->d_nfull.p + 1, out_xyzi ? c->export_buf.p : nullptr, out_xyzi ? room : 0);
    SCAL_HIP(op_memcpy_async(c->h_misc.p + 2, c->d_nfull.p + 1, sizeof(int), hipMemcpyDeviceToHost, s));
    SCAL_HIP(op_stream_synchronize(s));
    const int n = c->h_misc.p[2];
    if (out_xyzi && room > 0) {
        const int m = std::min(n, room);
        SCAL_HIP(op_memcpy_async(out_xyzi, c->export_buf.p, sizeof(float) * 4 * m, hipMemcpyDeviceToHost, s));
        SCAL_HIP(op_stream_synchronize(s));
        return m;
    }
    return n;
}

extern "C" int scal_map_export_all(scal_map_t* c, int which, float* out_xyzi, int cap) {
    if (!c || (which != 0 && which != 1) || cap < 0) {
        set_error("scal_map_export_all: bad argument");
        return SCAL_E_ARG;
    }
    SCAL_HIP(hipSetDevice(c->cfg.device));
    if (map_settle(c, true) != SCAL_OK) return -1;
    MapStore& M = c->map[which];
    if (!out_xyzi || cap == 0) return M.n;
    const int m = std::min(M.n, cap);
    if (m == 0) return 0;
    hipStream_t s = c->stream;
    if (c->export_buf.n < static_cast<size_t>(c->map_cap) * 4) SCAL_TRY(c->export_buf.alloc(static_cast<size_t>(c->map_cap) * 4));
    c->h_misc.p[1] = m;
    SCAL_HIP(op_memcpy_async(c->d_nfull.p + 1, c->h_misc.p + 1, sizeof(int), hipMemcpyHostToDevice, s));
    const MapCloud mc = M.cloud(c->cur);
    launch_interleave(s, c->d_nfull.p + 1, m, CSoA4{mc.x, mc.y, mc.z, mc.w}, c->export_buf.p);
    SCAL_HIP(op_memcpy_async(out_xyzi, c->export_buf.p, sizeof(float) * 4 * m, hipMemcpyDeviceToHost, s));
    SCAL_HIP(op_stream_synchronize(s));
    return m;
}

extern "C" int scal_map_set_merge_insert(scal_map_t* c, int enable) {
    if (!c) return SCAL_E_ARG;
    c->merge_insert = enable != 0;
    return SCAL_OK;
}

extern "C" int scal_map_get_wmap_wodom(scal_map_t* c, double* q, double* t) {
    if (!c || !q || !t) return SCAL_E_ARG;
    copy_pose(q, t, c->q_wmap_wodom, c->t_wmap_wodom);
    return SCAL_OK;
}

extern "C" int scal_map_get_path_counters(scal_map_t* c, int* out4) {
    if (!c || !out4) return SCAL_E_ARG;
    out4[0] = c->n_fast, out4[1] = c->n_general, out4[2] = c->n_recover_pose, out4[3] = c->n_recover_insert;
    return SCAL_OK;
}

extern "C" int scal_map_set_poll(scal_map_t* c, int enable) {
    if (!c) return SCAL_E_ARG;
    c->poll_on_enqueue = enable != 0;
    return SCAL_OK;
}

extern "C" int scal_map_adapter_begin(scal_map_t* c, const float* corner_last, int n_corner, const float* surf_last, int n_surf, const float* full_res,
                                      int n_full, const double* q_wodom, const double* t_wodom, double* q_w_curr, double* t_w_curr) {
    SCAL_TRY(check_host_arrays("scal_map_adapter_begin", c, corner_last, n_corner, surf_last, n_surf, n_full, q_wodom, t_wodom, q_w_curr, t_w_curr));
    const bool have_full = full_res != nullptr && n_full > 0;
    MapStep e;
    SCAL_TRY(begin_sync_step(c, true, "scal_map_adapter_begin: a step is still open", &e));
    SCAL_TRY(upload_step_inputs(c, e, corner_last, n_corner, surf_last, n_surf, full_res, have_full ? n_full : 0));
    copy_pose(e.pose.q_wodom, e.pose.t_wodom, q_wodom, t_wodom);
    e.fast = false, e.par = c->cur;
    SCAL_TRY(drop_prebuilt_grid(c));
    c->n_general++;
    SCAL_TRY(launch_pose_part(c, e, true));
    hipStream_t s = c->stream;
    SCAL_HIP(op_memcpy_async(c->h_S.p, c->d_S.p, sizeof(MapState), hipMemcpyDeviceToHost, s));
    SCAL_HIP(op_memcpy_async(c->res.p + e.slot, c->lm.d_st.p, sizeof(LMState), hipMemcpyDeviceToHost, s));
    SCAL_HIP(op_stream_synchronize(s));
    const double* x = c->res.p[e.slot].st.x;
    copy_pose(q_w_curr, t_w_curr, x, x + 4);
    c->adapter_step = e;
    c->adapter_active = true;
    return SCAL_OK;
}

extern "C" int scal_map_associate(scal_map_t* c, const double* q_w_curr, const double* t_w_curr, int* n_blocks, int* n_residuals) {
    if (!c || !q_w_curr || !t_w_curr || !n_blocks || !n_residuals) {
        set_error("scal_map_associate: null argument");
        return SCAL_E_ARG;
    }
    SCAL_TRY(need_adapter_step(c, "scal_map_associate"));
    SCAL_HIP(hipSetDevice(c->cfg.device));
    hipStream_t s = c->stream;
    const MapStep& e = c->adapter_step;
    const InputSet& I = c->sets[e.set];
    MapCounters* C = I.C.p;
    SCAL_TRY(c->blocks.set_pose(s, c->lm.d_st.p->x, q_w_curr, t_w_curr));
    FactorSoA F = c->lm.factors();
    const int assoc_blocks = std::max(1, std::min(3072, div_up(c->lm.slot_cap, 8)));
    SCAL_LAUNCH("k_assoc_knn", k_assoc_knn, dim3(assoc_blocks), dim3(256), 0, s, I.stack[0].cv(), I.stack[1].cv(), c->d_S.p,
                     c->grid[0].cell[e.par].p, c->grid[0].pts(e.par), c->grid[1].cell[e.par].p, c->grid[1].pts(e.par), c->lm.d_st.p, C, c->nnbuf(), MapBeginArgs{});
    const AssocFit fit{I.stack[0].cv(), I.stack[1].cv(), c->nnbuf(), C, F};
    SCAL_LAUNCH("k_assoc_fit", k_assoc_fit, dim3(std::max(1, div_up(c->lm.slot_cap, 64))), dim3(64), 0, s, fit, c->d_S.p);
    SCAL_TRY(c->blocks.compact(s, F, &C->n_slots));
    SCAL_HIP(op_memcpy_async(c->h_C.p, C, sizeof(MapCounters), hipMemcpyDeviceToHost, s));
    SCAL_HIP(op_stream_synchronize(s));
    if (!c->h_C.p->solve_on) c->blocks.set_empty();
    *n_blocks = c->blocks.n_blocks(), *n_residuals = c->blocks.n_residuals();
    return SCAL_OK;
}

extern "C" int scal_map_get_blocks(scal_map_t* c, scal_block* out, int cap) {
    if (!c || (!out && cap > 0) || cap < 0) {
        set_error("scal_map_get_blocks: bad argument");
        return SCAL_E_ARG;
    }
    SCAL_TRY(need_adapter_step(c, "scal_map_get_blocks"));
    SCAL_HIP(hipSetDevice(c->cfg.device));
    return c->blocks.get_blocks(c->stream, c->lm.factors(), out, cap);
}

extern "C" int scal_map_eval_blocks(scal_map_t* c, const double* x7, int want_jac, double* residuals, double* jacobians) {
    if (!c || !x7 || !residuals || (want_jac && !jacobians)) {
        set_error("scal_map_eval_blocks: bad argument");
        return SCAL_E_ARG;
    }
    SCAL_TRY(need_adapter_step(c, "scal_map_eval_blocks"));
    SCAL_HIP(hipSetDevice(c->cfg.device));
    return c->blocks.eval_blocks(c->stream, c->lm.factors(), x7, want_jac, residuals, jacobians);
}

extern "C" int scal_map_adapter_finish(scal_map_t* c, const double* q_w_curr, const double* t_w_curr, float* registered, scal_map_stats* stats) {
    if (!c || !q_w_curr || !t_w_curr) {
        set_error("scal_map_adapter_finish: null argument");
        return SCAL_E_ARG;
    }
    SCAL_TRY(need_adapter_step(c, "scal_map_adapter_finish"));
    SCAL_HIP(hipSetDevice(c->cfg.device));
    hipStream_t s = c->stream;
    MapStep& e = c->adapter_step;
    c->adapter_active = false;
    SCAL_TRY(c->blocks.set_pose(s, c->lm.d_st.p->x, q_w_curr, t_w_curr));
    SCAL_LAUNCH("k_map_pose_done", k_map_pose_done, dim3(64), dim3(256), 0, s, make_pose_done(c, e));
    SCAL_HIP(hipGetLastError());
    SCAL_HIP(op_event_record(c->ev_pose[e.slot], s));
    SCAL_HIP(op_event_synchronize(c->ev_pose[e.slot]));
    SCAL_TRY(general_insert(c, e));
    const MapResult& R = c->res.p[e.slot];
    publish_correction(c, R.S1);
    for (int k = 0; k < 2; ++k) c->map[k].n = R.S2.n_map[k];
    c->last_insert_path = e.insert_path;
    if (stats) stats_at_pose(R.C1, stats);
    stats_after_insertion(c, stats);
    if (e.have_full && registered) SCAL_TRY(download_registered(c, registered, c->h_misc.p[0]));
    return SCAL_OK;
}

extern "C" void* scal_map_stream(scal_map_t* c) { return c ? static_cast<void*>(c->stream) : nullptr; }

extern "C" int scal_map_debug_set_grid_cap(scal_map_t* c, int cap_corner, int cap_surf) {
    if (!c || cap_corner < 1 || cap_surf < 1) {
        set_error("scal_map_debug_set_grid_cap: bad argument");
        return SCAL_E_ARG;
    }
    if (!c->grid_fixed) return SCAL_OK;
    SCAL_TRY(map_settle(c, true));
    SCAL_HIP(hipSetDevice(c->cfg.device));
    SCAL_TRY(drop_prebuilt_grid(c));
    c->grid_cap_now[0] = std::min(cap_corner, c->grid[0].fixed_cap);
    c->grid_cap_now[1] = std::min(cap_surf, c->grid[1].fixed_cap);
    return SCAL_OK;
}

extern "C" int scal_map_debug_set_lm_polls(scal_map_t* c, int polls) {
    if (!c || polls < 0) return SCAL_E_ARG;
    SCAL_HIP(hipSetDevice(c->cfg.device));
    SCAL_HIP(op_stream_synchronize(c->stream));
    return lm_set_poll_budget(polls);
}
```

### sc-a-loam_amd/csrc/odometry.hip

```cpp
#include "common.hpp"
#include <deque>
#include "device_utils.hpp"
#include "voxel_dev.hpp"
#include "lm_host.hpp"
#include "features_dev.hpp"
#include <cmath>
#include <algorithm>

namespace scal {

struct OdomCounters {
    int n_corner_last, n_surf_last;
    int n_sharp, n_flat, n_less_sharp, n_less_flat;
    int n_slots, enable;
    int n_live[2], n_edge[2], n_plane[2];
};

__device__ __forceinline__ float sqdist(float ax, float ay, float az, float bx, float by, float bz) {
    return (ax - bx) * (ax - bx) + (ay - by) * (ay - by) + (az - bz) * (az - bz);
}

__device__ __forceinline__ unsigned long long make_key(float d, unsigned seq) {
    return (static_cast<unsigned long long>(__float_as_uint(d)) << 32) | seq;
}

constexpr int RING_TAB = 96;

__device__ __forceinline__ void transform_to_start(const double* x7, float ox, float oy, float oz, float* o) {
    double r[3];
    quat_rotate(x7, static_cast<double>(ox), static_cast<double>(oy), static_cast<double>(oz), r);
    o[0] = static_cast<float>(r[0] + 1.0 * x7[4]);
    o[1] = static_cast<float>(r[1] + 1.0 * x7[5]);
    o[2] = static_cast<float>(r[2] + 1.0 * x7[6]);
}

constexpr int OD_H = 8192;
constexpr int OD_LEVELS = 2;
__device__ constexpr float OD_INV_CELL[OD_LEVELS] = {1.0f, 0.2f};
__device__ constexpr float OD_EXACT_D2[OD_LEVELS] = {0.99f, 24.9f};
struct CellIndex {
    const int* start[OD_LEVELS];
    const float4* pts[OD_LEVELS];
};
__device__ __forceinline__ int od_cell(float v, int level) { return static_cast<int>(floorf(v * OD_INV_CELL[level])); }
__device__ __forceinline__ unsigned od_hash(int cx, int cy, int cz) {
    return (static_cast<unsigned>(cx) * 73856093u ^ static_cast<unsigned>(cy) * 19349663u ^ static_cast<unsigned>(cz) * 83492791u) & (OD_H - 1);
}
__device__ __forceinline__ unsigned od_bucket(float x, float y, float z, int level) { return od_hash(od_cell(x, level), od_cell(y, level), od_cell(z, level)); }
__device__ __forceinline__ unsigned long long od_cell_nn(const int* __restrict__ start, const float4* __restrict__ pts, int level, float sx, float sy, float sz,
                                                          int* s_beg, int* s_pre, unsigned long long* s_nn) {
    const int lane = lane_id(), wv = wave_id();
    if (wv == 0) {
        int b = 0, cnt = 0;
        if (lane < 27) {
            const unsigned h = od_hash(od_cell(sx, level) + lane % 3 - 1, od_cell(sy, level) + (lane / 3) % 3 - 1, od_cell(sz, level) + lane / 9 - 1);
            b = start[h];
            cnt = start[h + 1] - b;
        }
        int incl = cnt;
#pragma unroll
        for (int o = 1; o < 32; o <<= 1) {
            const int v = __shfl_up(incl, o, 64);
            if (lane >= o) incl += v;
        }
        if (lane < 27) s_beg[lane] = b, s_pre[lane + 1] = incl;
        if (lane == 0) s_pre[0] = 0;
    }
    __syncthreads();
    unsigned long long best = ~0ull;
    const int n_cand = s_pre[27];
    for (int m = threadIdx.x; m < n_cand; m += 256) {
        int j = 0;
#pragma unroll
        for (int o = 16; o >= 1; o >>= 1)
            if (j + o <= 26 && s_pre[j + o] <= m) j += o;
        const float4 p = pts[s_beg[j] + (m - s_pre[j])];
        const float dx = sx - p.x, dy = sy - p.y, dz = sz - p.z;
        float d = dx * dx;
        d += dy * dy;
        d += dz * dz;
        best = min(best, make_key(d, __float_as_uint(p.w)));
    }
    best = wave_min_u64(best);
    if (lane == 0) s_nn[wv] = best;
    __syncthreads();
    best = min(min(s_nn[0], s_nn[1]), min(s_nn[2], s_nn[3]));
    __syncthreads();
    return best;
}

__device__ __forceinline__ void k_odom_assoc_body(const CSoA4& sharp, const CSoA4& flat, const CSoA4& CL, const CSoA4& SL, const LMState* __restrict__ st, OdomCounters* C,
                                                    int outer, const FactorSoA& f, const CellIndex& ci_corner, const CellIndex& ci_surf,
                                                    const int* __restrict__ ring_tab) {
    if (!C->enable) return;
    const int ns = C->n_sharp, nf = C->n_flat;
    if (blockIdx.x == 0 && threadIdx.x == 0) C->n_slots = min(ns + nf, f.cap);
    __shared__ unsigned long long s_k2[4], s_k3[4];
    const int q = blockIdx.x;
    if (q >= ns + nf || q >= f.cap) return;
    const int lane = lane_id(), wv = wave_id();
    const bool is_edge = q < ns;
    const int j = is_edge ? q : q - ns;
    const CSoA4& Q = is_edge ? sharp : flat;
    const CSoA4& T = is_edge ? CL : SL;
    const int nT = is_edge ? C->n_corner_last : C->n_surf_last;
    double x7[7];
#pragma unroll
    for (int k = 0; k < 7; ++k) x7[k] = st->x[k];
    const float ox = Q.x[j], oy = Q.y[j], oz = Q.z[j];
    float sel[3];
    transform_to_start(x7, ox, oy, oz, sel);
    const float sx = sel[0], sy = sel[1], sz = sel[2];

    __shared__ int s_beg[27], s_pre[28];
    __shared__ unsigned long long s_nn[4];
    const CellIndex& ci = is_edge ? ci_corner : ci_surf;
    unsigned long long best = od_cell_nn(ci.start[0], ci.pts[0], 0, sx, sy, sz, s_beg, s_pre, s_nn);
    auto dist_of = [](unsigned long long k) { return __uint_as_float(static_cast<unsigned>(k >> 32)); };
    if (best == ~0ull || !(dist_of(best) < OD_EXACT_D2[0])) {
        best = od_cell_nn(ci.start[1], ci.pts[1], 1, sx, sy, sz, s_beg, s_pre, s_nn);
        if (best == ~0ull || !(dist_of(best) < OD_EXACT_D2[1])) {
            best = ~0ull;
            for (int t0 = threadIdx.x; t0 < nT; t0 += 1024) {
                float txx[4], tyy[4], tzz[4];
#pragma unroll
                for (int u = 0; u < 4; ++u) {
                    const int t = min(t0 + 256 * u, nT - 1);
                    txx[u] = T.x[t], tyy[u] = T.y[t], tzz[u] = T.z[t];
                }
#pragma unroll
                for (int u = 0; u < 4; ++u) {
                    const int t = min(t0 + 256 * u, nT - 1);
                    const float dx = sx - txx[u], dy = sy - tyy[u], dz = sz - tzz[u];
                    float d = dx * dx;
                    d += dy * dy;
                    d += dz * dz;
                    best = min(best, make_key(d, static_cast<unsigned>(t)));
                }
            }
            best = wave_min_u64(best);
            if (lane == 0) s_nn[wv] = best;
            __syncthreads();
            best = min(min(s_nn[0], s_nn[1]), min(s_nn[2], s_nn[3]));
        }
    }
    int valid = 0;
    int kind = is_edge ? 0 : 1;
    double pa[3] = {0, 0, 0}, pb[3] = {0, 0, 0};
    const float nnd = __uint_as_float(static_cast<unsigned>(best >> 32));
    if (best != ~0ull && static_cast<double>(nnd) < 25.0) {
        const int c = static_cast<int>(best & 0xffffffffu);
        const int id = static_cast<int>(T.w[c]);
        unsigned long long k2 = ~0ull, k3 = ~0ull;
        const int* first_idx = ring_tab + (is_edge ? 0 : 2 * RING_TAB);
        const int* last_idx = first_idx + RING_TAB;
        int fi = 0x7f7f7f7f, li = -1;
        for (int r = lane; r < RING_TAB; r += 64) {
            if (r >= id + 3) fi = min(fi, first_idx[r]);
            if (r <= id - 3) li = max(li, last_idx[r]);
        }
        const int hi = min(wave_min_i(fi), nT);
        const int lo = wave_max_i(li);
        for (int t0 = c + 1 + lane + 64 * wv; t0 < hi; t0 += 1024) {
            float tw[4], txx[4], tyy[4], tzz[4];
#pragma unroll
            for (int u = 0; u < 4; ++u) {
                const int t = t0 + 256 * u;
                if (t < hi) tw[u] = T.w[t], txx[u] = T.x[t], tyy[u] = T.y[t], tzz[u] = T.z[t];
            }
#pragma unroll
            for (int u = 0; u < 4; ++u) {
                const int t = t0 + 256 * u;
                if (t < hi) {
                    const int rj = static_cast<int>(tw[u]);
                    const float d = sqdist(txx[u], tyy[u], tzz[u], sx, sy, sz);
                    if (static_cast<double>(d) < 25.0) {
                        const unsigned seq = static_cast<unsigned>(t - c - 1);
                        if (is_edge) {
                            if (rj > id) k2 = min(k2, make_key(d, seq));
                        } else {
                            if (rj <= id) k2 = min(k2, make_key(d, seq));
                            else k3 = min(k3, make_key(d, seq));
                        }
                    }
                }
            }
        }
        for (int t0 = c - 1 - lane - 64 * wv; t0 > lo; t0 -= 1024) {
            float tw[4], txx[4], tyy[4], tzz[4];
#pragma unroll
            for (int u = 0; u < 4; ++u) {
                const int t = t0 - 256 * u;
                if (t > lo) tw[u] = T.w[t], txx[u] = T.x[t], tyy[u] = T.y[t], tzz[u] = T.z[t];
            }
#pragma unroll
            for (int u = 0; u < 4; ++u) {
                const int t = t0 - 256 * u;
                if (t > lo) {
                    const int rj = static_cast<int>(tw[u]);
                    const float d = sqdist(txx[u], tyy[u], tzz[u], sx, sy, sz);
                    if (static_cast<double>(d) < 25.0) {
                        const unsigned seq = 0x40000000u + static_cast<unsigned>(c - 1 - t);
                        if (is_edge) {
                            if (rj < id) k2 = min(k2, make_key(d, seq));
                        } else {
                            if (rj >= id) k2 = min(k2, make_key(d, seq));
                            else k3 = min(k3, make_key(d, seq));
                        }
                    }
                }
            }
        }
        k2 = wave_min_u64(k2);
        k3 = wave_min_u64(k3);
        if (lane == 0) s_k2[wv] = k2, s_k3[wv] = k3;
        __syncthreads();
        k2 = min(min(s_k2[0], s_k2[1]), min(s_k2[2], s_k2[3]));
        k3 = min(min(s_k3[0], s_k3[1]), min(s_k3[2], s_k3[3]));
        auto decode = [&](unsigned long long k) {
            const unsigned seq = static_cast<unsigned>(k & 0xffffffffu);
            return (seq & 0x40000000u) ? c - 1 - static_cast<int>(seq & 0x3fffffffu) : c + 1 + static_cast<int>(seq);
        };
        if (is_edge) {
            if (k2 != ~0ull) {
                const int i2 = decode(k2);
                valid = 1;
                pa[0] = T.x[c], pa[1] = T.y[c], pa[2] = T.z[c];
                pb[0] = T.x[i2], pb[1] = T.y[i2], pb[2] = T.z[i2];
            }
        } else if (k2 != ~0ull && k3 != ~0ull) {
            const int i2 = decode(k2), i3 = decode(k3);
            valid = 1;
            const double jx = T.x[c], jy = T.y[c], jz = T.z[c];
            const double lx = T.x[i2], ly = T.y[i2], lz = T.z[i2];
            const double mx = T.x[i3], my = T.y[i3], mz = T.z[i3];
            const double ax = jx - lx, ay = jy - ly, az = jz - lz, bx = jx - mx, by = jy - my, bz = jz - mz;
            double nx = ay * bz - az * by, ny = az * bx - ax * bz, nz = ax * by - ay * bx;
            const double z = nx * nx + ny * ny + nz * nz;
            if (z > 0) {
                const double s = sqrt(z);
                nx /= s, ny /= s, nz /= s;
            }
            pa[0] = jx, pa[1] = jy, pa[2] = jz;
            pb[0] = nx, pb[1] = ny, pb[2] = nz;
        }
    }
    if (lane == 0 && wv == 0) {
        f.valid[q] = valid;
        f.kind[q] = kind;
        f.cp[q] = ox, f.cp[f.cap + q] = oy, f.cp[2 * f.cap + q] = oz;
        f.pa[q] = pa[0], f.pa[f.cap + q] = pa[1], f.pa[2 * f.cap + q] = pa[2];
        f.pb[q] = pb[0], f.pb[f.cap + q] = pb[1], f.pb[2 * f.cap + q] = pb[2];
    }
}
SCAL_KERNEL(256, k_odom_assoc)

__device__ __forceinline__ void k_odom_init_pose_body(LMState* st, int* ring_tab) {
    if (threadIdx.x == 0) {
        st->x[0] = st->x[1] = st->x[2] = 0.0, st->x[3] = 1.0;
        st->x[4] = st->x[5] = st->x[6] = 0.0;
    }
    for (int t = threadIdx.x; t < 8 * RING_TAB; t += blockDim.x) ring_tab[t] = ((t / RING_TAB) & 1) ? -1 : 0x7f7f7f7f;
}
SCAL_KERNEL(1024, k_odom_init_pose)
struct HandoverArgs {
    CSoA4 in[2];
    const int* d_n[2];
    SoA4 out[2];
    int* d_n_out[2];
    int cap[2];
    int nb0;
    int* tab_write;
    int* tab_reset;
    const LMState* st;
    LMState* host_st;
    const LMSync* sync;
    int* cell_cnt[2][OD_LEVELS];
    int* cell_rank[2][OD_LEVELS];
};
__device__ __forceinline__ void k_odom_handover_body(const HandoverArgs& a) {
    int b = blockIdx.x;
    const int k = b < a.nb0 ? 0 : 1;
    if (k) b -= a.nb0;
    if (blockIdx.x == 0) {
        for (int t = threadIdx.x; t < 4 * RING_TAB; t += 256) a.tab_reset[t] = ((t / RING_TAB) & 1) ? -1 : 0x7f7f7f7f;
        const unsigned* src = reinterpret_cast<const unsigned*>(a.st);
        unsigned* dst = reinterpret_cast<unsigned*>(a.host_st);
        const bool abandoned = a.sync->abandoned != 0;
        constexpr int TERM_WORD = static_cast<int>(offsetof(LMState, termination) / 4);
        for (int t = threadIdx.x; t < static_cast<int>(sizeof(LMState) / 4); t += 256) dst[t] = (abandoned && t == TERM_WORD) ? 5u : src[t];
    }
    int* first_idx = a.tab_write + 2 * k * RING_TAB;
    int* last_idx = first_idx + RING_TAB;
    const CSoA4 in = a.in[k];
    const SoA4 out = a.out[k];
    const int n = min(*a.d_n[k], a.cap[k]);
    const int i = b * 256 + threadIdx.x;
    if (i == 0) *a.d_n_out[k] = n;
    if (b * 256 >= n) return;
    const int lane = lane_id();
    float x = 0, y = 0, z = 0;
    if (i < n) {
        const float w = in.w[i];
        x = in.x[i], y = in.y[i], z = in.z[i];
        out.x[i] = x, out.y[i] = y, out.z[i] = z, out.w[i] = w;
        const int r = min(max(static_cast<int>(w), 0), RING_TAB - 1);
        const int rp = __shfl_up(r, 1, 64);
        const int rn = __shfl_down(r, 1, 64);
        if (lane == 0 || rp != r) atomicMin(&first_idx[r], i);
        if (lane == 63 || rn != r || i == n - 1) atomicMax(&last_idx[r], i);
    }
#pragma unroll
    for (int l = 0; l < OD_LEVELS; ++l) {
        const unsigned h = i < n ? od_bucket(x, y, z, l) : 0xffffffffu;
        const unsigned hp = __shfl_up(h, 1, 64);
        const unsigned long long heads = __ballot(lane == 0 || hp != h);
        const int head = 63 - __clzll(heads & (~0ull >> (63 - lane)));
        const unsigned long long above = lane == 63 ? 0ull : heads & (~0ull << (lane + 1));
        const int next = above ? __ffsll(static_cast<long long>(above)) - 1 : 64;
        int base = 0;
        if (lane == head && i < n) {
            base = atomicAdd(&a.cell_cnt[k][l][h], next - head);
        }
        base = __shfl(base, head, 64);
        if (i < n) a.cell_rank[k][l][i] = base + (lane - head);
    }
}
SCAL_KERNEL(256, k_odom_handover)
constexpr int OD_START_STRIDE = OD_H + 4;
__device__ __forceinline__ void k_odom_cellscan_body(int* cnt_all, int* start_all) {
    constexpr int PER = OD_H / 1024;
    static_assert(PER % 4 == 0, "int4 loads");
    int* cnt = cnt_all + blockIdx.x * OD_H;
    int* start = start_all + blockIdx.x * OD_START_STRIDE;
    __shared__ int s_w[16];
    int v[PER];
    int4* c4 = reinterpret_cast<int4*>(cnt + threadIdx.x * PER);
    int sum = 0;
#pragma unroll
    for (int u = 0; u < PER / 4; ++u) {
        const int4 q = c4[u];
        v[4 * u] = q.x, v[4 * u + 1] = q.y, v[4 * u + 2] = q.z, v[4 * u + 3] = q.w;
        sum += q.x + q.y + q.z + q.w;
        c4[u] = make_int4(0, 0, 0, 0);
    }
    int incl = sum;
    const int lane = lane_id(), wv = wave_id();
#pragma unroll
    for (int o = 1; o < 64; o <<= 1) {
        const int t = __shfl_up(incl, o, 64);
        if (lane >= o) incl += t;
    }
    if (lane == 63) s_w[wv] = incl;
    __syncthreads();
    int base = incl - sum;
    for (int w = 0; w < wv; ++w) base += s_w[w];
    int4* s4 = reinterpret_cast<int4*>(start + threadIdx.x * PER);
#pragma unroll
    for (int u = 0; u < PER / 4; ++u) {
        int4 o;
        o.x = base, base += v[4 * u];
        o.y = base, base += v[4 * u + 1];
        o.z = base, base += v[4 * u + 2];
        o.w = base, base += v[4 * u + 3];
        s4[u] = o;
    }
    if (threadIdx.x == 1023) start[OD_H] = base;
}
SCAL_KERNEL(1024, k_odom_cellscan)
struct CellFillArgs {
    CSoA4 in[2];
    const int* d_n[2];
    const int* rank[2][OD_LEVELS];
    const int* start[2][OD_LEVELS];
    float4* pts[2][OD_LEVELS];
    int nb0;
};
__device__ __forceinline__ void k_odom_cellfill_body(const CellFillArgs& a) {
    int b = blockIdx.x;
    const int k = b < a.nb0 ? 0 : 1;
    if (k) b -= a.nb0;
    const int i = b * 256 + threadIdx.x;
    if (i >= *a.d_n[k]) return;
    const float x = a.in[k].x[i], y = a.in[k].y[i], z = a.in[k].z[i];
    const float4 rec = make_float4(x, y, z, __uint_as_float(static_cast<unsigned>(i)));
#pragma unroll
    for (int l = 0; l < OD_LEVELS; ++l) a.pts[k][l][a.start[k][l][od_bucket(x, y, z, l)] + a.rank[k][l][i]] = rec;
}
SCAL_KERNEL(256, k_odom_cellfill)
struct OdomGatherArgs {
    const float *sharp, *flat, *less;
    CSoA4 less_flat;
    const int *n_sharp, *n_flat, *n_less, *n_less_flat;
    SoA4 o_sharp, o_flat, o_less, o_less_flat;
    int slot_cap, feat_cap, cap, nbs, nbf;
};
__device__ __forceinline__ void k_odom_gather_body(const OdomGatherArgs& a, OdomCounters* C) {
    int b = blockIdx.x;
    const float* aos = nullptr;
    const int* d_n;
    int* d_n_out;
    SoA4 out;
    int cap;
    if (b < a.nbs) {
        aos = a.sharp, d_n = a.n_sharp, d_n_out = &C->n_sharp, out = a.o_sharp, cap = a.slot_cap;
        if (b == 0 && threadIdx.x == 0) {
            C->n_slots = 0, C->enable = 1;
            C->n_live[0] = C->n_live[1] = C->n_edge[0] = C->n_edge[1] = C->n_plane[0] = C->n_plane[1] = 0;
        }
    } else if (b < 2 * a.nbs) {
        b -= a.nbs, aos = a.flat, d_n = a.n_flat, d_n_out = &C->n_flat, out = a.o_flat, cap = a.slot_cap;
    } else if (b < 2 * a.nbs + a.nbf) {
        b -= 2 * a.nbs, aos = a.less, d_n = a.n_less, d_n_out = &C->n_less_sharp, out = a.o_less, cap = a.feat_cap;
    } else {
        b -= 2 * a.nbs + a.nbf, d_n = a.n_less_flat, d_n_out = &C->n_less_flat, out = a.o_less_flat, cap = a.cap;
    }
    const int n = min(*d_n, cap);
    const int i = b * 256 + threadIdx.x;
    if (i == 0) *d_n_out = n;
    if (i >= n) return;
    if (aos) {
        const float4 p = reinterpret_cast<const float4*>(aos)[i];
        out.x[i] = p.x, out.y[i] = p.y, out.z[i] = p.z, out.w[i] = p.w;
    } else {
        out.x[i] = a.less_flat.x[i], out.y[i] = a.less_flat.y[i], out.z[i] = a.less_flat.z[i], out.w[i] = a.less_flat.w[i];
    }
}
SCAL_KERNEL(256, k_odom_gather)

}

using namespace scal;

struct scal_odom {
    scal_odom_config cfg;
    LaneStream stream;
    int cap = 0, feat_cap = 0;
    bool systemInited = false;
    static constexpr int MAX_STEPS = 4;
    struct Pending {
        int slot;
        bool solve;
    };
    std::deque<Pending> pending;
    Event ev[MAX_STEPS];
    int next_slot = 0;
    double q_w_curr[4] = {0, 0, 0, 1}, t_w_curr[3] = {0, 0, 0};
    DevBuf<float> aos;
    SoAStore sharp, flat, less_sharp, less_flat;
    SoAStore corner_last, surf_last;
    LMStore lm;
    DevBuf<int> cell_cnt, cell_start, cell_rank;
    DevBuf<float4> cell_pts;
    int* cell_cnt_of(int k, int l) const { return cell_cnt.p + (k * OD_LEVELS + l) * OD_H; }
    int* cell_start_of(int k, int l) const { return cell_start.p + (k * OD_LEVELS + l) * OD_START_STRIDE; }
    int* cell_rank_of(int k, int l) const { return cell_rank.p + (size_t)l * (feat_cap + cap) + (k ? feat_cap : 0); }
    float4* cell_pts_of(int k, int l) const { return cell_pts.p + (size_t)l * (feat_cap + cap) + (k ? feat_cap : 0); }
    CellIndex cell_index(int k) const {
        CellIndex ci;
        for (int l = 0; l < OD_LEVELS; ++l) ci.start[l] = cell_start_of(k, l), ci.pts[l] = cell_pts_of(k, l);
        return ci;
    }
    DevBuf<int> ring_tab;
    int tab_cur = 0;
    DevBuf<OdomCounters> d_C;
    PinBuf<LMState> h_st;
    PinBuf<OdomCounters> h_up;
    HostStage hs;
    bool adapter_active = false, adapter_solve = false;
    BlockAdapter blocks;
    int outer_next = 0;
};

int scal::odom_create(const scal_odom_config* cfg, StreamLayout layout, scal_odom_t** out) {
    if (!cfg || !out || cfg->max_points <= 0) {
        set_error("scal_odom_create: bad argument");
        return SCAL_E_ARG;
    }
    *out = nullptr;
    SCAL_TRY(select_device(cfg->device));
    auto* c = new scal_odom();
    c->cfg = *cfg;
    c->cap = cfg->max_points;
    c->feat_cap = 120 * 64;
    int rc = SCAL_OK;
    auto A = [&](int r) { if (rc == SCAL_OK) rc = r; };
    A(c->lm.alloc(36 * 64));
    A(c->aos.alloc((size_t)c->cap * 4));
    A(c->sharp.alloc(c->lm.slot_cap)); A(c->flat.alloc(c->lm.slot_cap));
    A(c->less_sharp.alloc(c->feat_cap)); A(c->corner_last.alloc(c->feat_cap));
    A(c->less_flat.alloc(c->cap)); A(c->surf_last.alloc(c->cap));
    A(c->cell_cnt.alloc(2 * OD_LEVELS * OD_H)); A(c->cell_start.alloc(2 * OD_LEVELS * OD_START_STRIDE));
    A(c->cell_rank.alloc(OD_LEVELS * ((size_t)c->feat_cap + c->cap))); A(c->cell_pts.alloc(OD_LEVELS * ((size_t)c->feat_cap + c->cap)));
    A(c->ring_tab.alloc(8 * RING_TAB));
    A(c->blocks.alloc(c->lm.slot_cap));
    A(c->d_C.alloc(1)); A(c->h_st.alloc(scal_odom::MAX_STEPS)); A(c->h_up.alloc(1));
    if (rc == SCAL_OK) rc = lm_check_residency<LMNoHook, LMNoHook>(c->cfg.device);
    if (rc == SCAL_OK) rc = c->stream.acquire(c->cfg.device, stage_lane(layout, STAGE_ODOM));
    for (int k = 0; k < scal_odom::MAX_STEPS && rc == SCAL_OK; ++k) rc = c->ev[k].create(hipEventDisableTiming);
    if (rc == SCAL_OK) {
        rc = c->lm.init(c->stream);
        if (rc == SCAL_OK && op_memset_async(c->d_C.p, 0, sizeof(OdomCounters), c->stream) != hipSuccess) rc = SCAL_E_HIP;
        if (rc == SCAL_OK) rc = c->cell_cnt.zero(c->stream);
        if (rc == SCAL_OK) rc = c->cell_start.zero(c->stream);
        SCAL_LAUNCH("k_odom_init_pose", k_odom_init_pose, dim3(1), dim3(256), 0, c->stream, c->lm.d_st.p, c->ring_tab.p);
        if (rc == SCAL_OK && op_stream_synchronize(c->stream) != hipSuccess) rc = SCAL_E_HIP;
    }
    if (rc != SCAL_OK) {
        if (rc == SCAL_E_HIP) set_error("scal_odom_create: HIP resource creation failed");
        delete c;
        return rc;
    }
    *out = c;
    return SCAL_OK;
}

extern "C" int scal_odom_create(const scal_odom_config* cfg, scal_odom_t** out) { return odom_create(cfg, default_stream_layout(), out); }

extern "C" void scal_odom_destroy(scal_odom_t* c) {
    if (!c) return;
    (void)hipSetDevice(c->cfg.device);
    if (c->stream) (void)op_stream_synchronize(c->stream);
    delete c;
}

namespace {

int launch_handover(scal_odom* c, int slot, hipEvent_t ev);
int odom_enqueue(scal_odom* c) {
    hipStream_t s = c->stream;
    OdomCounters* C = c->d_C.p;
    LMState* st = c->lm.d_st.p;
    FactorSoA F = c->lm.factors();
    const bool solve = c->systemInited;
    c->systemInited = true;
    const int slot = c->next_slot;
    c->next_slot = (c->next_slot + 1) % scal_odom::MAX_STEPS;
    if (solve) {
        for (int outer = 0; outer < 2; ++outer) {
            {
                SCAL_LAUNCH("k_odom_assoc", k_odom_assoc, dim3(std::max(1, c->lm.slot_cap)), dim3(256), 0, s, c->sharp.cv(), c->flat.cv(),
                                   c->corner_last.cv(), c->surf_last.cv(), st, C, outer, F, c->cell_index(0), c->cell_index(1), c->ring_tab.p + c->tab_cur * 4 * RING_TAB);
            }
            {
                                launch_lm_solve(s, F, &C->n_slots, st, &C->enable, c->lm.partials.p, c->lm.lm_sync.p, outer, nullptr, LMNoHook(), LMNoHook(), "k_lm_solve_odom");
            }
        }
    }
    SCAL_TRY(launch_handover(c, slot, c->ev[slot]));
    c->pending.push_back({slot, solve});
    return SCAL_OK;
}

int launch_handover(scal_odom* c, int slot, hipEvent_t ev) {
    hipStream_t s = c->stream;
    OdomCounters* C = c->d_C.p;
    LMState* st = c->lm.d_st.p;
    {
        HandoverArgs h;
        h.in[0] = c->less_sharp.cv(), h.in[1] = c->less_flat.cv();
        h.d_n[0] = &C->n_less_sharp, h.d_n[1] = &C->n_less_flat;
        h.out[0] = c->corner_last.v(), h.out[1] = c->surf_last.v();
        h.d_n_out[0] = &C->n_corner_last, h.d_n_out[1] = &C->n_surf_last;
        h.cap[0] = c->feat_cap, h.cap[1] = c->cap;
        h.nb0 = std::max(1, div_up(c->feat_cap, 256));
        h.tab_write = c->ring_tab.p + (c->tab_cur ^ 1) * 4 * RING_TAB;
        h.tab_reset = c->ring_tab.p + c->tab_cur * 4 * RING_TAB;
        h.st = st, h.host_st = c->h_st.p + slot, h.sync = c->lm.lm_sync.p;
        for (int k = 0; k < 2; ++k)
            for (int l = 0; l < OD_LEVELS; ++l) h.cell_cnt[k][l] = c->cell_cnt_of(k, l), h.cell_rank[k][l] = c->cell_rank_of(k, l);
        const dim3 grid(h.nb0 + std::max(1, div_up(c->cap, 256)));
        SCAL_LAUNCH("k_odom_handover", k_odom_handover, grid, dim3(256), 0, s, h);
        c->tab_cur ^= 1;
        if (ev) SCAL_HIP(op_event_record(ev, s));
        SCAL_LAUNCH("k_odom_cellscan", k_odom_cellscan, dim3(2 * OD_LEVELS), dim3(1024), 0, s, c->cell_cnt.p, c->cell_start.p);
        CellFillArgs f;
        f.in[0] = c->corner_last.cv(), f.in[1] = c->surf_last.cv();
        f.d_n[0] = &C->n_corner_last, f.d_n[1] = &C->n_surf_last;
        for (int k = 0; k < 2; ++k)
            for (int l = 0; l < OD_LEVELS; ++l) f.rank[k][l] = c->cell_rank_of(k, l), f.start[k][l] = c->cell_start_of(k, l), f.pts[k][l] = c->cell_pts_of(k, l);
        f.nb0 = h.nb0;
        SCAL_LAUNCH("k_odom_cellfill", k_odom_cellfill, grid, dim3(256), 0, s, f);
    }
    SCAL_HIP(hipGetLastError());
    return SCAL_OK;
}

int odom_collect(scal_odom* c, double* q_lc, double* t_lc, double* q_w, double* t_w, scal_odom_stats* stats) {
    if (c->pending.empty()) {
        set_error("scal_odom_collect: no step enqueued");
        return SCAL_E_STATE;
    }
    const int slot = c->pending.front().slot;
    const bool solve = c->pending.front().solve;
    c->pending.pop_front();
    SCAL_HIP(op_event_synchronize(c->ev[slot]));
    const LMState& L = c->h_st.p[slot];
    if (L.termination == 5) {
        (void)c->lm.clear_exchange(c->stream);
        set_error("LM solve abandoned: grid barrier timed out");
        return SCAL_E_HIP;
    }
    const double* x = L.x;
    if (solve) {
        double r[3];
        q_rot(c->q_w_curr, x + 4, r);
        for (int i = 0; i < 3; ++i) c->t_w_curr[i] = c->t_w_curr[i] + r[i];
        double qn[4];
        q_mul(c->q_w_curr, x, qn);
        for (int i = 0; i < 4; ++i) c->q_w_curr[i] = qn[i];
    }
    for (int i = 0; i < 4; ++i) q_lc[i] = x[i], q_w[i] = c->q_w_curr[i];
    for (int i = 0; i < 3; ++i) t_lc[i] = x[4 + i], t_w[i] = c->t_w_curr[i];
    if (stats) {
        std::memset(stats, 0, sizeof *stats);
        if (solve) {
            for (int o = 0; o < 2; ++o) {
                stats->n_edge[o] = L.log_n_edge[o], stats->n_plane[o] = L.log_n_plane[o];
                stats->lm_iters[o] = L.log_iters[o], stats->lm_success[o] = L.log_success[o];
                stats->cost_init[o] = L.log_cost_init[o], stats->cost_final[o] = L.log_cost_final[o];
            }
        }
    }
    return SCAL_OK;
}

}

static int odom_upload(scal_odom* c, const float* sharp, int n_sharp, const float* less_sharp, int n_less_sharp, const float* flat, int n_flat,
                       const float* less_flat, int n_less_flat) {
    hipStream_t s = c->stream;
    SCAL_HIP(op_stream_synchronize(s));
    c->hs.finish();
    (void)c->hs.reserve(((size_t)2 * c->lm.slot_cap + c->feat_cap + c->cap) * 16 + 4096);
    OdomCounters& H = *c->h_up.p;
    OdomCounters fresh;
    std::memset(&fresh, 0, sizeof fresh);
    fresh.n_sharp = n_sharp, fresh.n_flat = n_flat, fresh.n_less_sharp = n_less_sharp, fresh.n_less_flat = n_less_flat, fresh.enable = 1;
    H = fresh;
    const size_t off = offsetof(OdomCounters, n_sharp);
    SCAL_HIP(op_memcpy_async(reinterpret_cast<char*>(c->d_C.p) + off, reinterpret_cast<char*>(&H) + off, sizeof(OdomCounters) - off,
                            hipMemcpyHostToDevice, s));
    auto up = [&](const float* src, int n, SoAStore& dst) -> int {
        if (n > 0) {
            SCAL_HIP(c->hs.h2d(c->aos.p, src, sizeof(float) * 4 * n, s));
            launch_deinterleave(s, c->aos.p, n, dst.v());
        }
        return SCAL_OK;
    };
    SCAL_TRY(up(sharp, n_sharp, c->sharp));
    SCAL_TRY(up(flat, n_flat, c->flat));
    SCAL_TRY(up(less_sharp, n_less_sharp, c->less_sharp));
    SCAL_TRY(up(less_flat, n_less_flat, c->less_flat));
    return SCAL_OK;
}

extern "C" int scal_odom_step(scal_odom_t* c, const float* sharp, int n_sharp, const float* less_sharp, int n_less_sharp, const float* flat,
                              int n_flat, const float* less_flat, int n_less_flat, double* q_lc, double* t_lc, double* q_w, double* t_w,
                              scal_odom_stats* stats) {
    if (!c || !q_lc || !t_lc || !q_w || !t_w || n_sharp < 0 || n_less_sharp < 0 || n_flat < 0 || n_less_flat < 0 || (n_sharp && !sharp) ||
        (n_less_sharp && !less_sharp) || (n_flat && !flat) || (n_less_flat && !less_flat)) {
        set_error("scal_odom_step: bad argument");
        return SCAL_E_ARG;
    }
    if (n_sharp + n_flat > c->lm.slot_cap || n_sharp > c->lm.slot_cap || n_flat > c->lm.slot_cap || n_less_sharp > c->feat_cap || n_less_flat > c->cap) {
        set_error("scal_odom_step: cloud larger than the context capacity (sharp+flat <= %d, lessSharp <= %d, lessFlat <= %d)", c->lm.slot_cap,
                  c->feat_cap, c->cap);
        return SCAL_E_TOO_MANY;
    }
    SCAL_HIP(hipSetDevice(c->cfg.device));
    if (!c->pending.empty()) {
        set_error("scal_odom_step: a queued step has not been collected");
        return SCAL_E_STATE;
    }
    SCAL_TRY(odom_upload(c, sharp, n_sharp, less_sharp, n_less_sharp, flat, n_flat, less_flat, n_less_flat));
    SCAL_TRY(odom_enqueue(c));
    return odom_collect(c, q_lc, t_lc, q_w, t_w, stats);
}

extern "C" int scal_odom_enqueue_features(scal_odom_t* c, scal_features_t* feat) {
    if (!c || !feat) {
        set_error("scal_odom_enqueue_features: null argument");
        return SCAL_E_ARG;
    }
    if (static_cast<int>(c->pending.size()) >= scal_odom::MAX_STEPS) {
        set_error("scal_odom_enqueue_features: %d steps are queued and not collected", scal_odom::MAX_STEPS);
        return SCAL_E_STATE;
    }
    FeatDeviceView v = features_view(feat);
    if (v.device != c->cfg.device) {
        set_error("features context lives on device %d, odometry context on %d", v.device, c->cfg.device);
        return SCAL_E_ARG;
    }
    SCAL_HIP(hipSetDevice(c->cfg.device));
    hipStream_t s = c->stream;
    OdomGatherArgs a;
    a.sharp = v.sharp_xyzi, a.flat = v.flat_xyzi, a.less = v.less_xyzi;
    a.less_flat = CSoA4{v.lfx, v.lfy, v.lfz, v.lfi};
    a.n_sharp = &v.P->n_sharp, a.n_flat = &v.P->n_flat, a.n_less = &v.P->n_less_sharp, a.n_less_flat = &v.P->n_less_flat;
    a.o_sharp = c->sharp.v(), a.o_flat = c->flat.v(), a.o_less = c->less_sharp.v(), a.o_less_flat = c->less_flat.v();
    a.slot_cap = c->lm.slot_cap, a.feat_cap = c->feat_cap, a.cap = std::min(c->cap, v.cap);
    a.nbs = std::max(1, div_up(c->lm.slot_cap, 256)), a.nbf = std::max(1, div_up(c->feat_cap, 256));
    SCAL_TRY(features_wait_done(feat, s));
    SCAL_LAUNCH("k_odom_gather", k_odom_gather, dim3(2 * a.nbs + a.nbf + std::max(1, div_up(a.cap, 256))), dim3(256), 0, s, a, c->d_C.p);
    SCAL_TRY(features_note_reader(feat, s));
    return odom_enqueue(c);
}

extern "C" int scal_odom_collect(scal_odom_t* c, double* q_lc, double* t_lc, double* q_w, double* t_w, scal_odom_stats* stats) {
    if (!c || !q_lc || !t_lc || !q_w || !t_w) {
        set_error("scal_odom_collect: null argument");
        return SCAL_E_ARG;
    }
    SCAL_HIP(hipSetDevice(c->cfg.device));
    return odom_collect(c, q_lc, t_lc, q_w, t_w, stats);
}

extern "C" int scal_odom_step_features(scal_odom_t* c, scal_features_t* feat, double* q_lc, double* t_lc, double* q_w, double* t_w,
                                       scal_odom_stats* stats) {
    if (!c || !feat || !q_lc || !t_lc || !q_w || !t_w) {
        set_error("scal_odom_step_features: null argument");
        return SCAL_E_ARG;
    }
    SCAL_TRY(scal_odom_enqueue_features(c, feat));
    return odom_collect(c, q_lc, t_lc, q_w, t_w, stats);
}

extern "C" int scal_odom_adapter_begin(scal_odom_t* c, const float* sharp, int n_sharp, const float* less_sharp, int n_less_sharp, const float* flat,
                                       int n_flat, const float* less_flat, int n_less_flat, double* q_last_curr, double* t_last_curr, int* need_solve) {
    if (!c || !q_last_curr || !t_last_curr || !need_solve || n_sharp < 0 || n_less_sharp < 0 || n_flat < 0 || n_less_flat < 0 || (n_sharp && !sharp) ||
        (n_less_sharp && !less_sharp) || (n_flat && !flat) || (n_less_flat && !less_flat)) {
        set_error("scal_odom_adapter_begin: bad argument");
        return SCAL_E_ARG;
    }
    if (n_sharp + n_flat > c->lm.slot_cap || n_less_sharp > c->feat_cap || n_less_flat > c->cap) {
        set_error("scal_odom_adapter_begin: cloud larger than the context capacity");
        return SCAL_E_TOO_MANY;
    }
    if (!c->pending.empty() || c->adapter_active) {
        set_error("scal_odom_adapter_begin: a step is still open");
        return SCAL_E_STATE;
    }
    SCAL_HIP(hipSetDevice(c->cfg.device));
    hipStream_t s = c->stream;
    SCAL_HIP(op_stream_synchronize(s));
    SCAL_TRY(odom_upload(c, sharp, n_sharp, less_sharp, n_less_sharp, flat, n_flat, less_flat, n_less_flat));
    SCAL_HIP(op_memcpy_async(c->h_st.p, c->lm.d_st.p, sizeof(LMState), hipMemcpyDeviceToHost, s));
    SCAL_HIP(op_stream_synchronize(s));
    for (int i = 0; i < 4; ++i) q_last_curr[i] = c->h_st.p->x[i];
    for (int i = 0; i < 3; ++i) t_last_curr[i] = c->h_st.p->x[4 + i];
    c->adapter_solve = c->systemInited;
    c->systemInited = true;
    *need_solve = c->adapter_solve ? 1 : 0;
    c->adapter_active = true;
    c->outer_next = 0;
    return SCAL_OK;
}

extern "C" int scal_odom_associate(scal_odom_t* c, const double* q_last_curr, const double* t_last_curr, int* n_blocks, int* n_residuals) {
    if (!c || !q_last_curr || !t_last_curr || !n_blocks || !n_residuals) {
        set_error("scal_odom_associate: null argument");
        return SCAL_E_ARG;
    }
    if (!c->adapter_active || !c->adapter_solve) {
        set_error("scal_odom_associate: no open step that needs a solve");
        return SCAL_E_STATE;
    }
    SCAL_HIP(hipSetDevice(c->cfg.device));
    hipStream_t s = c->stream;
    OdomCounters* C = c->d_C.p;
    LMState* st = c->lm.d_st.p;
    FactorSoA F = c->lm.factors();
    SCAL_TRY(c->blocks.set_pose(c->stream, c->lm.d_st.p->x, q_last_curr, t_last_curr));
    SCAL_LAUNCH("k_odom_assoc", k_odom_assoc, dim3(std::max(1, c->lm.slot_cap)), dim3(256), 0, s, c->sharp.cv(), c->flat.cv(), c->corner_last.cv(),
                     c->surf_last.cv(), st, C, std::min(c->outer_next, 1), F, c->cell_index(0), c->cell_index(1), c->ring_tab.p + c->tab_cur * 4 * RING_TAB);
    c->outer_next++;
    SCAL_TRY(c->blocks.compact(s, F, &C->n_slots));
    SCAL_HIP(op_stream_synchronize(s));
    *n_blocks = c->blocks.n_blocks(), *n_residuals = c->blocks.n_residuals();
    return SCAL_OK;
}

extern "C" int scal_odom_get_blocks(scal_odom_t* c, scal_block* out, int cap) {
    if (!c || (!out && cap > 0) || cap < 0) {
        set_error("scal_odom_get_blocks: bad argument");
        return SCAL_E_ARG;
    }
    if (!c->adapter_active) {
        set_error("scal_odom_get_blocks: no scal_odom_adapter_begin");
        return SCAL_E_STATE;
    }
    SCAL_HIP(hipSetDevice(c->cfg.device));
    return c->blocks.get_blocks(c->stream, c->lm.factors(), out, cap);
}

extern "C" int scal_odom_eval_blocks(scal_odom_t* c, const double* x7, int want_jac, double* residuals, double* jacobians) {
    if (!c || !x7 || !residuals || (want_jac && !jacobians)) {
        set_error("scal_odom_eval_blocks: bad argument");
        return SCAL_E_ARG;
    }
    if (!c->adapter_active) {
        set_error("scal_odom_eval_blocks: no scal_odom_adapter_begin");
        return SCAL_E_STATE;
    }
    SCAL_HIP(hipSetDevice(c->cfg.device));
    return c->blocks.eval_blocks(c->stream, c->lm.factors(), x7, want_jac, residuals, jacobians);
}

extern "C" int scal_odom_adapter_finish(scal_odom_t* c, const double* q_last_curr, const double* t_last_curr, double* q_w_curr, double* t_w_curr) {
    if (!c || !q_last_curr || !t_last_curr || !q_w_curr || !t_w_curr) {
        set_error("scal_odom_adapter_finish: null argument");
        return SCAL_E_ARG;
    }
    if (!c->adapter_active) {
        set_error("scal_odom_adapter_finish: no scal_odom_adapter_begin");
        return SCAL_E_STATE;
    }
    SCAL_HIP(hipSetDevice(c->cfg.device));
    c->adapter_active = false;
    SCAL_TRY(c->blocks.set_pose(c->stream, c->lm.d_st.p->x, q_last_curr, t_last_curr));
    const int slot = c->next_slot;
    c->next_slot = (c->next_slot + 1) % scal_odom::MAX_STEPS;
    SCAL_TRY(launch_handover(c, slot, c->ev[slot]));
    c->pending.push_back({slot, c->adapter_solve});
    double q_lc[4], t_lc[3];
    return odom_collect(c, q_lc, t_lc, q_w_curr, t_w_curr, nullptr);
}

extern "C" void* scal_odom_stream(scal_odom_t* c) { return c ? static_cast<void*>(c->stream) : nullptr; }
```

### sc-a-loam_amd/csrc/pipeline.cpp

```cpp
#include "common.hpp"
#include "keyframes.hpp"
#include <algorithm>
#include <cmath>
#include <condition_variable>
#include <deque>
#include <chrono>
#include <cstdlib>
#include <string>
#include <thread>

namespace scal {
void print_forced_flushes();
}
using namespace scal;

namespace {
constexpr int REC_N = 64;
constexpr int MAX_UNPOPPED = 32;
constexpr int MAX_LOOPS_UNPOPPED = 64;
int env_int(const char* name, int dflt, int lo, int hi) {
    const char* e = std::getenv(name);
    if (!e) return dflt;
    const int v = std::atoi(e);
    return v < lo ? lo : (v > hi ? hi : v);
}
const int B_AHEAD = env_int("SCALOAM_PIPE_B_AHEAD", 2, 1, 3);
const int PF_AHEAD = env_int("SCALOAM_PIPE_PF_AHEAD", 3, 1, 3);

const bool TIMING = env_int("SCALOAM_PIPE_TIMING", 0, 0, 1) != 0;
struct HostTimer {
    const char* name[12] = {};
    double total[12] = {};
    long calls[12] = {};
    template <class F>
    int run(int slot, const char* nm, F&& f) {
        if (!TIMING) return f();
        const auto t0 = std::chrono::steady_clock::now();
        const int rc = f();
        name[slot] = nm;
        total[slot] += std::chrono::duration<double, std::micro>(std::chrono::steady_clock::now() - t0).count();
        calls[slot]++;
        return rc;
    }
    void print(const char* thread) const {
        for (int i = 0; i < 12; ++i)
            if (calls[i]) std::fprintf(stderr, "[scal_pipeline] %-6s %-28s %8.1f us/call x %ld\n", thread, name[i], total[i] / calls[i], calls[i]);
    }
};

constexpr int SMAX = scal::BATCH_MAX;
struct Rec {
    const float* d_xyz[SMAX] = {};
    const void* h_xyz[SMAX] = {};
    int n[SMAX] = {};
    int stride = 0;
    bool host = false;
    scal_pipeline_result res[SMAX] = {};
};
}

struct scal_pipeline {
    scal_pipeline_config cfg{};
    int ring = 6, depth = 2;
    int S = 1;
    std::vector<scal_features_t*> regs[SMAX];
    scal_odom_t* od[SMAX] = {};
    scal_map_t* mp[SMAX] = {};
    scal_sc_t* sc[SMAX] = {};
    double* d_desc = nullptr;
    bool own_desc = false;
    Rec rec[REC_N];
    std::mutex mu;
    std::condition_variable cv;
    long long pushed = 0, a_run = 0, a_done = 0, pf_done = 0, b_enq = 0, b_coll = 0, c_enq = 0, c_coll = 0, d_ins = 0, d_coll = 0, popped = 0;
    int pop_waiting = 0;
    bool drain_req = false, drained = true;
    bool stop = false;
    int err = SCAL_OK;
    std::string errmsg;
    std::thread t_front, t_side, t_odom, t_pose, t_loop;
    HostTimer tm_front, tm_side, tm_odom, tm_pose, tm_loop;
    KeyframeStore* kf = nullptr;
    scal_keyframe_gate_state gate{};
    double fitness_thres = 0.3;
    std::deque<KfLoopJob> jobs;
    std::deque<scal_pipeline_loop> loops;
    bool verifying = false;
    long long verifying_seq = 0;
    long long loops_owed = 0;
    std::thread t_verify;
    struct AcceptedLoop {
        int curr_kf, loop_kf;
        double q[4], t[3];
    };
    std::vector<AcceptedLoop> accepted;
    int verifying_kf = -1;
    int kf_passed_end = 0;
    scal_posegraph_t* pg = nullptr;

    bool sc_on() const { return cfg.sc_mode != SCAL_PIPE_SC_OFF; }
    bool side_sc() const { return cfg.sc_mode == SCAL_PIPE_SC_EVERY_SCAN || cfg.sc_mode == SCAL_PIPE_SC_DESCRIPTOR; }
    bool kf_mode() const { return cfg.sc_mode == SCAL_PIPE_SC_KEYFRAME; }
    bool verify_idle() const { return jobs.empty() && !verifying; }
    Rec& r(long long k) { return rec[k % REC_N]; }
    template <class F>
    int for_all(F&& f) {
        if (S == 1) return f(0);
        Recorder recs[SMAX];
        Recorder* ptr[SMAX];
        int rc = SCAL_OK;
        for (int q = 0; q < S && rc == SCAL_OK; ++q) {
            ptr[q] = &recs[q];
            g_recorder = &recs[q];
            rc = f(q);
            g_recorder = nullptr;
        }
        if (rc != SCAL_OK) {
            for (int q = 0; q < S; ++q) (void)recs[q].flush();
            return rc;
        }
        if (zip_and_launch(ptr, S) != hipSuccess) {
            set_error("scal_pipeline: a batched launch failed: %s", hipGetErrorString(hipGetLastError()));
            return SCAL_E_HIP;
        }
        return SCAL_OK;
    }
    template <class F>
    int for_each(F&& f) {
        for (int q = 0; q < S; ++q) SCAL_TRY(f(q));
        return SCAL_OK;
    }
    void fail(int rc) {
        if (err == SCAL_OK) {
            err = rc;
            errmsg = scal_last_error();
        }
        cv.notify_all();
    }
};

namespace {

void front_thread(scal_pipeline* p) {
    std::unique_lock<std::mutex> lk(p->mu);
    for (;;) {
        const long long k = p->a_done;
        p->cv.wait(lk, [&] {
            if (p->stop || p->err) return true;
            if (p->pushed <= k) return false;
            const long long old = k - p->ring;
            if (old >= 0 && (p->c_coll <= old || p->b_enq <= old || (p->sc_on() && p->d_ins <= old))) return false;
            return k - p->c_enq < PF_AHEAD;
        });
        if (p->stop || p->err) return;
        const Rec& rc = p->r(k);
        const int slot = static_cast<int>(k % p->ring);
        lk.unlock();
        int st = p->tm_front.run(0, "A: features_run", [&] {
            return p->for_all([&](int q) {
                scal_features_t* reg = p->regs[q][slot];
                return rc.host ? scal_features_enqueue_host(reg, rc.h_xyz[q], rc.n[q], rc.stride) : scal_features_run_device(reg, rc.d_xyz[q], rc.n[q], rc.stride);
            });
        });
        if (st == SCAL_OK) {
            lk.lock();
            p->a_run = k + 1;
            p->cv.notify_all();
            lk.unlock();
            st = p->tm_front.run(1, "C: prefetch, lane 0 half", [&] { return p->for_all([&](int q) { return scal_map_prefetch_begin(p->mp[q], p->regs[q][slot]); }); });
        }
        lk.lock();
        if (st != SCAL_OK) {
            p->fail(st);
            return;
        }
        p->a_done = k + 1;
        p->cv.notify_all();
    }
}

void side_thread(scal_pipeline* p) {
    std::unique_lock<std::mutex> lk(p->mu);
    const bool search = p->cfg.sc_mode == SCAL_PIPE_SC_EVERY_SCAN;
    for (;;) {
        const long long k = p->pf_done;
        p->cv.wait(lk, [&] {
            if (p->stop || p->err) return true;
            if (p->a_done <= k) return false;
            return !(p->side_sc() && k - p->d_coll >= 3);
        });
        if (p->stop || p->err) return;
        const int slot = static_cast<int>(k % p->ring);
        lk.unlock();
        double* dd = p->d_desc ? p->d_desc + static_cast<size_t>(slot) * 1200 : nullptr;
        int st = p->tm_side.run(1, "C: prefetch, side half + D: insert", [&]() -> int {
            if (!p->side_sc() && p->S == 1) return scal_map_prefetch_finish(p->mp[0], p->regs[0][slot]);
            Recorder recs[2 * SMAX];
            Recorder* ptr[2 * SMAX];
            int nr = 0, rc2 = SCAL_OK;
            rc2 = p->tm_side.run(3, "   record prefetch", [&] {
                int r3 = SCAL_OK;
                for (int q = 0; q < p->S && r3 == SCAL_OK; ++q) {
                    g_recorder = ptr[nr] = &recs[nr];
                    ++nr;
                    r3 = scal_map_prefetch_finish(p->mp[q], p->regs[q][slot]);
                    g_recorder = nullptr;
                }
                return r3;
            });
            if (rc2 == SCAL_OK && p->side_sc())
                rc2 = p->tm_side.run(4, "   record insert", [&] {
                    int r3 = SCAL_OK;
                    for (int q = 0; q < p->S && r3 == SCAL_OK; ++q) {
                        g_recorder = ptr[nr] = &recs[nr];
                        ++nr;
                        r3 = search ? scal_sc_insert_features(p->sc[q], p->regs[q][slot]) : scal_sc_make_features_enqueue(p->sc[q], p->regs[q][slot], dd);
                        g_recorder = nullptr;
                    }
                    return r3;
                });
            if (rc2 != SCAL_OK) {
                for (int i = 0; i < nr; ++i) (void)recs[i].flush();
                return rc2;
            }
            return p->tm_side.run(5, "   zip + launch", [&]() -> int {
                if (zip_marked_and_launch(ptr, nr) != hipSuccess) {
                    set_error("scal_pipeline: a batched launch failed: %s", hipGetErrorString(hipGetLastError()));
                    return SCAL_E_HIP;
                }
                return SCAL_OK;
            });
        });
        if (st == SCAL_OK && search) st = p->tm_side.run(2, "D: sc_detect_enqueue", [&] { return p->for_all([&](int q) { return scal_sc_detect_enqueue(p->sc[q]); }); });
        lk.lock();
        if (st != SCAL_OK) {
            p->fail(st);
            return;
        }
        p->r(k).res[0].d_descriptor = dd;
        p->pf_done = k + 1;
        if (p->side_sc()) p->d_ins = k + 1;
        p->cv.notify_all();
    }
}

void odom_thread(scal_pipeline* p) {
    std::unique_lock<std::mutex> lk(p->mu);
    for (;;) {
        enum { NONE, B_ENQ, B_COLL } what = NONE;
        p->cv.wait(lk, [&] {
            if (p->stop || p->err) return true;
            if (p->b_enq < p->a_run && p->b_enq - p->b_coll < B_AHEAD) { what = B_ENQ; return true; }
            if (p->b_coll < p->b_enq && p->b_coll - p->c_enq < 2) { what = B_COLL; return true; }
            return false;
        });
        if (p->stop || p->err) return;
        int st = SCAL_OK;
        if (what == B_ENQ) {
            const long long k = p->b_enq;
            const int slot = static_cast<int>(k % p->ring);
            lk.unlock();
            st = p->tm_odom.run(0, "B: odom_enqueue_features", [&] { return p->for_all([&](int q) { return scal_odom_enqueue_features(p->od[q], p->regs[q][slot]); }); });
            lk.lock();
            if (st == SCAL_OK) p->b_enq = k + 1;
        } else {
            const long long k = p->b_coll;
            scal_pipeline_result* R = p->r(k).res;
            lk.unlock();
            st = p->tm_odom.run(1, "B: odom_collect (wait)", [&] {
                return p->for_each([&](int q) {
                    double qlc[4], tlc[3];
                    return scal_odom_collect(p->od[q], qlc, tlc, R[q].q_odom, R[q].t_odom, &R[q].odom);
                });
            });
            lk.lock();
            if (st == SCAL_OK) p->b_coll = k + 1;
        }
        if (st != SCAL_OK) {
            p->fail(st);
            return;
        }
        p->cv.notify_all();
    }
}

void pose_thread(scal_pipeline* p) {
    std::unique_lock<std::mutex> lk(p->mu);
    for (;;) {
        enum { NONE, C_ENQ, C_COLL, FINISH } what = NONE;
        p->cv.wait(lk, [&] {
            if (p->stop || p->err) return true;
            const long long inflight = p->c_enq - p->c_coll;
            if (p->c_enq < p->b_coll && p->c_enq < p->pf_done && inflight <= p->depth) { what = C_ENQ; return true; }
            if (inflight > p->depth || (inflight > 0 && (p->pop_waiting || p->drain_req) && p->c_enq == p->pushed)) { what = C_COLL; return true; }
            if (p->drain_req && p->c_coll == p->pushed) { what = FINISH; return true; }
            return false;
        });
        if (p->stop || p->err) return;
        int st = SCAL_OK;
        if (what == C_ENQ) {
            const long long k = p->c_enq;
            const int slot = static_cast<int>(k % p->ring);
            scal_pipeline_result* R = p->r(k).res;
            lk.unlock();
            st = p->tm_pose.run(2, "C: map_enqueue_features", [&] {
                return p->for_all([&](int q) { return scal_map_enqueue_features(p->mp[q], p->regs[q][slot], R[q].q_odom, R[q].t_odom); });
            });
            lk.lock();
            if (st == SCAL_OK) p->c_enq = k + 1;
        } else if (what == C_COLL) {
            const long long k = p->c_coll;
            scal_pipeline_result* R = p->r(k).res;
            lk.unlock();
            st = p->tm_pose.run(3, "C: map_collect (wait)", [&] {
                return p->for_each([&](int q) { return scal_map_collect(p->mp[q], R[q].q_w_curr, R[q].t_w_curr, &R[q].map); });
            });
            lk.lock();
            if (st == SCAL_OK) p->c_coll = k + 1;
        } else if (what == FINISH) {
            lk.unlock();
            st = p->for_each([&](int q) { return scal_map_finish(p->mp[q]); });
            lk.lock();
            if (st == SCAL_OK) p->drain_req = false, p->drained = true;
        }
        if (st != SCAL_OK) {
            p->fail(st);
            return;
        }
        p->cv.notify_all();
    }
}

void loop_thread(scal_pipeline* p) {
    std::unique_lock<std::mutex> lk(p->mu);
    const bool search = p->cfg.sc_mode == SCAL_PIPE_SC_EVERY_SCAN;
    for (;;) {
        p->cv.wait(lk, [&] {
            if (p->stop || p->err) return true;
            const long long infl = p->d_ins - p->d_coll;
            return infl >= 2 || (infl > 0 && (p->pop_waiting || p->drain_req));
        });
        if (p->stop || p->err) return;
        const long long k = p->d_coll;
        scal_pipeline_result* R = p->r(k).res;
        lk.unlock();
        int st;
        if (search) {
            st = p->tm_loop.run(2, "D: sc_detect_collect (wait)", [&] {
                return p->for_each([&](int q) {
                    const int rc = scal_sc_detect_collect(p->sc[q], &R[q].loop);
                    R[q].have_loop = rc == SCAL_OK;
                    return rc;
                });
            });
        } else {
            st = scal_sc_wait_descriptor(p->sc[0]);
        }
        lk.lock();
        if (st != SCAL_OK) {
            p->fail(st);
            return;
        }
        p->d_coll = k + 1;
        p->cv.notify_all();
    }
}

void keyframe_thread(scal_pipeline* p) {
    std::unique_lock<std::mutex> lk(p->mu);
    for (;;) {
        const long long k = p->d_coll;
        p->cv.wait(lk, [&] { return p->stop || p->err || p->c_coll > k; });
        if (p->stop || p->err) return;
        scal_pipeline_result& R = p->r(k).res[0];
        const int slot = static_cast<int>(k % p->ring);
        lk.unlock();
        int is_kf = 0;
        bool detect = false;
        int st = scal_keyframe_gate(&p->gate, R.q_w_curr, R.t_w_curr, &is_kf);
        R.is_keyframe = is_kf, R.keyframe_id = -1, R.have_loop = 0;
        if (st == SCAL_OK && is_kf) {
            const int id = scal_sc_size(p->sc[0]);
            double p6[6];
            pose6_from(R.q_w_curr, R.t_w_curr, p6);
            st = p->tm_loop.run(0, "D: insert + append", [&] { return p->kf->insert(p->sc[0], p->regs[0][slot], id, p6); });
            if (st == SCAL_OK) {
                R.keyframe_id = id;
                detect = p->kf->own_count() >= 30;
                if (detect) st = p->tm_loop.run(1, "D: sc_detect_enqueue", [&] { return scal_sc_detect_enqueue(p->sc[0]); });
            }
        }
        lk.lock();
        if (st != SCAL_OK) {
            p->fail(st);
            return;
        }
        p->d_ins = k + 1;
        p->cv.notify_all();
        lk.unlock();
        if (detect) {
            st = p->tm_loop.run(2, "D: sc_detect_collect (wait)", [&] { return scal_sc_detect_collect(p->sc[0], &R.loop); });
            R.have_loop = st == SCAL_OK;
        }
        if (st == SCAL_OK && is_kf) st = p->kf->check();
        lk.lock();
        if (st != SCAL_OK) {
            p->fail(st);
            return;
        }
        if (detect && R.loop.loop_id >= 0) {
            p->jobs.push_back(KfLoopJob{k, R.keyframe_id, R.loop.loop_id, R.loop.yaw_rad, R.loop.min_dist});
            p->loops_owed++;
        }
        if (is_kf) p->kf_passed_end = R.keyframe_id + 1;
        p->d_coll = k + 1;
        p->cv.notify_all();
    }
}

void verify_thread(scal_pipeline* p) {
    std::unique_lock<std::mutex> lk(p->mu);
    for (;;) {
        p->cv.wait(lk, [&] { return p->stop || p->err || !p->jobs.empty(); });
        if (p->stop || p->err) return;
        const KfLoopJob job = p->jobs.front();
        p->jobs.pop_front();
        p->verifying = true, p->verifying_seq = job.seq, p->verifying_kf = job.curr_kf;
        lk.unlock();
        scal_pipeline_loop rec;
        const int st = p->kf->verify(job, p->fitness_thres, &rec);
        lk.lock();
        p->verifying = false;
        if (st != SCAL_OK) {
            p->fail(st);
            return;
        }
        p->loops.push_back(rec);
        if (rec.verified == 1) {
            scal_pipeline::AcceptedLoop a{rec.curr_kf, rec.loop_kf, {rec.q_rel[0], rec.q_rel[1], rec.q_rel[2], rec.q_rel[3]}, {rec.t_rel[0], rec.t_rel[1], rec.t_rel[2]}};
            p->accepted.push_back(a);
        }
        p->cv.notify_all();
    }
}

int report(scal_pipeline* p) {
    set_error("%s", p->errmsg.c_str());
    return p->err;
}

int push(scal_pipeline* p, const float* const* d_xyz, const void* const* h_xyz, const int* n, int stride, bool host) {
    std::unique_lock<std::mutex> lk(p->mu);
    if (p->err) return report(p);
    if (p->pushed - p->popped >= MAX_UNPOPPED) {
        set_error("scal_pipeline_push: %d results wait to be popped", MAX_UNPOPPED);
        return SCAL_E_STATE;
    }
    if (p->loops_owed >= MAX_LOOPS_UNPOPPED) {
        set_error("scal_pipeline_push: %d loop records wait to be popped (scal_pipeline_pop_loop)", MAX_LOOPS_UNPOPPED);
        return SCAL_E_STATE;
    }
    const long long k = p->pushed;
    Rec& rc = p->r(k);
    rc = Rec();
    for (int q = 0; q < p->S; ++q) {
        rc.d_xyz[q] = d_xyz ? d_xyz[q] : nullptr, rc.h_xyz[q] = h_xyz ? h_xyz[q] : nullptr, rc.n[q] = n[q];
        rc.res[q].seq = k;
    }
    rc.stride = stride, rc.host = host;
    p->pushed = k + 1;
    p->drained = false;
    p->cv.notify_all();
    p->cv.wait(lk, [&] { return p->err || (host ? p->a_done > k : p->a_done + p->ring > k); });
    if (p->err) return report(p);
    return SCAL_OK;
}

int pop(scal_pipeline* p, scal_pipeline_result* out) {
    std::unique_lock<std::mutex> lk(p->mu);
    if (p->popped >= p->pushed && !p->err) {
        set_error("scal_pipeline_pop: nothing pushed");
        return SCAL_E_STATE;
    }
    const long long k = p->popped;
    p->pop_waiting++;
    p->cv.notify_all();
    p->cv.wait(lk, [&] { return p->err || (p->c_coll > k && (!p->sc_on() || p->d_coll > k)); });
    p->pop_waiting--;
    if (p->err) return report(p);
    for (int q = 0; q < p->S; ++q) out[q] = p->r(k).res[q];
    p->popped = k + 1;
    p->cv.notify_all();
    return SCAL_OK;
}

int create(const scal_pipeline_config* cfg, int n_seqs, scal_pipeline_t** out) {
    if (!cfg || !out) {
        set_error("scal_pipeline_create: null argument");
        return SCAL_E_ARG;
    }
    *out = nullptr;
    const int ring = cfg->ring == 0 ? 6 : cfg->ring, depth = cfg->depth == 0 ? 2 : cfg->depth;
    if (ring < 4 || ring > 16 || depth < 1 || depth > 3 || cfg->sc_mode < 0 || cfg->sc_mode > 3) {
        set_error("scal_pipeline_create: ring must be 4..16, depth 1..3, sc_mode 0..3");
        return SCAL_E_ARG;
    }
    if (n_seqs < 1 || n_seqs > SMAX || (n_seqs > 1 && (cfg->sc_mode == SCAL_PIPE_SC_DESCRIPTOR || cfg->sc_mode == SCAL_PIPE_SC_KEYFRAME))) {
        set_error("scal_pipeline_create_multi: 1..%d sequences (sc_mode 2 and 3 only with one)", SMAX);
        return SCAL_E_ARG;
    }
    scal_keyframe_gate_state gate{};
    if (cfg->sc_mode == SCAL_PIPE_SC_KEYFRAME) {
        if (cfg->kf_max_points < 0 || !(cfg->loop_fitness_thres >= 0) || cfg->sc_max_keyframes <= 0 ||
            scal_keyframe_gate_init(&gate, cfg->keyframe_meter_gap == 0 ? 2.0 : cfg->keyframe_meter_gap,
                                    cfg->keyframe_deg_gap == 0 ? 10.0 : cfg->keyframe_deg_gap) != SCAL_OK) {
            set_error("scal_pipeline_create: sc_mode 3 needs keyframe gaps >= 0, kf_max_points >= 0, loop_fitness_thres >= 0, sc_max_keyframes > 0");
            return SCAL_E_ARG;
        }
    }
    if (cfg->pgo_map_max_points < 0 || (cfg->pgo_map_max_points > 0 && (cfg->sc_mode != SCAL_PIPE_SC_KEYFRAME || cfg->kf_max_points == 0))) {
        set_error("scal_pipeline_create: pgo_map_max_points must be >= 0, and > 0 only in sc_mode 3 with kf_max_points > 0");
        return SCAL_E_ARG;
    }
    SCAL_TRY(select_device(cfg->device));
    auto* p = new scal_pipeline();
    p->cfg = *cfg, p->ring = ring, p->depth = depth, p->S = n_seqs;
    p->gate = gate;
    p->fitness_thres = cfg->loop_fitness_thres == 0 ? 0.3 : cfg->loop_fitness_thres;
    int rc = SCAL_OK;
    if (p->kf_mode()) {
        p->kf = new KeyframeStore();
        rc = p->kf->init(cfg->device, cfg->kf_max_points, cfg->sc_max_keyframes, cfg->pgo_map_max_points);
    }
    scal_features_config fc{};
    fc.lidar_type = cfg->lidar_type, fc.n_scans = cfg->n_scans, fc.minimum_range = cfg->minimum_range, fc.max_points = cfg->max_points;
    fc.float_math = cfg->float_math, fc.check_finite = cfg->check_finite, fc.device = cfg->device;
    for (int q = 0; q < n_seqs && rc == SCAL_OK; ++q) {
        for (int i = 0; i < ring && rc == SCAL_OK; ++i) {
            scal_features_t* f = nullptr;
            rc = scal_features_create(&fc, &f);
            if (rc == SCAL_OK) p->regs[q].push_back(f);
        }
        if (rc == SCAL_OK) {
            scal_odom_config oc{};
            oc.max_points = cfg->max_points, oc.device = cfg->device;
            rc = odom_create(&oc, StreamLayout::PerStage, &p->od[q]);
        }
        if (rc == SCAL_OK) {
            scal_map_config mc{};
            mc.line_res = cfg->line_res, mc.plane_res = cfg->plane_res, mc.max_scan_points = cfg->max_points, mc.max_map_points = cfg->max_map_points;
            mc.device = cfg->device;
            rc = map_create(&mc, StreamLayout::PerStage, &p->mp[q]);
        }
        if (rc == SCAL_OK && p->sc_on()) {
            scal_sc_config sc{};
            sc.max_radius = cfg->sc_max_radius, sc.dist_thres = cfg->sc_dist_thres, sc.max_keyframes = cfg->sc_max_keyframes;
            sc.float_math = cfg->float_math, sc.device = cfg->device, sc.n_shards = 1, sc.shard = 0, sc.side_stream = env_int("SCALOAM_PIPE_SC_LANE", 1, 0, 5);
            rc = sc_create(&sc, StreamLayout::PerStage, &p->sc[q]);
            if (rc == SCAL_OK && cfg->sc_mode == SCAL_PIPE_SC_DESCRIPTOR) {
                if (cfg->d_desc_ring) {
                    p->d_desc = cfg->d_desc_ring;
                } else if (hipMalloc(reinterpret_cast<void**>(&p->d_desc), sizeof(double) * 1200 * ring) != hipSuccess) {
                    set_error("scal_pipeline_create: hipMalloc of the descriptor ring failed");
                    rc = SCAL_E_HIP;
                } else {
                    p->own_desc = true;
                }
            }
        }
    }
    if (rc != SCAL_OK) {
        const std::string keep = scal_last_error();
        scal_pipeline_destroy(p);
        set_error("%s", keep.c_str());
        return rc;
    }
    p->t_front = std::thread(front_thread, p);
    p->t_side = std::thread(side_thread, p);
    p->t_odom = std::thread(odom_thread, p);
    p->t_pose = std::thread(pose_thread, p);
    if (p->side_sc()) p->t_loop = std::thread(loop_thread, p);
    if (p->kf_mode()) p->t_loop = std::thread(keyframe_thread, p), p->t_verify = std::thread(verify_thread, p);
    *out = p;
    return SCAL_OK;
}

}

extern "C" int scal_pipeline_create(const scal_pipeline_config* cfg, scal_pipeline_t** out) { return create(cfg, 1, out); }
extern "C" int scal_pipeline_create_multi(const scal_pipeline_config* cfg, int n_seqs, scal_pipeline_t** out) { return create(cfg, n_seqs, out); }
extern "C" int scal_pipeline_seqs(scal_pipeline_t* p) { return p ? p->S : 0; }

extern "C" void scal_pipeline_destroy(scal_pipeline_t* p) {
    if (!p) return;
    {
        std::lock_guard<std::mutex> lk(p->mu);
        p->stop = true;
        p->cv.notify_all();
    }
    if (p->t_front.joinable()) p->t_front.join();
    if (p->t_side.joinable()) p->t_side.join();
    if (p->t_odom.joinable()) p->t_odom.join();
    if (p->t_pose.joinable()) p->t_pose.join();
    if (p->t_loop.joinable()) p->t_loop.join();
    if (p->t_verify.joinable()) p->t_verify.join();
    if (TIMING) {
        p->tm_front.print("front"), p->tm_side.print("side"), p->tm_odom.print("odom"), p->tm_pose.print("pose"), p->tm_loop.print("loop");
        std::fprintf(stderr, "[scal_pipeline] sequences %d, recorded lists flushed in the middle of an entry point: %ld\n", p->S, g_forced_flushes);
        print_forced_flushes();
    }
    (void)hipSetDevice(p->cfg.device);
    for (int q = 0; q < SMAX; ++q) {
        if (p->sc[q]) scal_sc_destroy(p->sc[q]);
        if (p->mp[q]) scal_map_destroy(p->mp[q]);
        if (p->od[q]) scal_odom_destroy(p->od[q]);
    }
    for (int q = 0; q < SMAX; ++q)
        for (auto* f : p->regs[q]) scal_features_destroy(f);
    if (p->pg) scal_posegraph_destroy(p->pg);
    delete p->kf;
    if (p->d_desc && p->own_desc) (void)hipFree(p->d_desc);
    delete p;
}

static int check_scan(scal_pipeline_t* p, const void* ptr, int n) {
    if ((!ptr && n > 0) || n < 0) {
        set_error("scal_pipeline_push: bad argument");
        return SCAL_E_ARG;
    }
    if (n > p->cfg.max_points) {
        set_error("scan has %d points, capacity is %d", n, p->cfg.max_points);
        return SCAL_E_TOO_MANY;
    }
    return SCAL_OK;
}

extern "C" int scal_pipeline_push_device(scal_pipeline_t* p, const float* d_xyz, int n, int stride_floats) {
    if (!p || stride_floats < 3 || p->S != 1) {
        set_error("scal_pipeline_push_device: bad argument (a pipeline of several sequences takes scal_pipeline_push_device_multi)");
        return SCAL_E_ARG;
    }
    SCAL_TRY(check_scan(p, d_xyz, n));
    return push(p, &d_xyz, nullptr, &n, stride_floats, false);
}

extern "C" int scal_pipeline_push_device_multi(scal_pipeline_t* p, const float* const* d_xyz, const int* n, int stride_floats) {
    if (!p || !d_xyz || !n || stride_floats < 3) {
        set_error("scal_pipeline_push_device_multi: bad argument");
        return SCAL_E_ARG;
    }
    for (int q = 0; q < p->S; ++q) SCAL_TRY(check_scan(p, d_xyz[q], n[q]));
    return push(p, d_xyz, nullptr, n, stride_floats, false);
}

extern "C" int scal_pipeline_push_host(scal_pipeline_t* p, const void* xyz, int n, int stride_bytes) {
    if (!p || stride_bytes < 12 || (stride_bytes % 4) != 0 || stride_bytes > 32 || p->S != 1) {
        set_error("scal_pipeline_push_host: bad argument (stride_bytes must be a multiple of 4 in [12, 32]; one sequence)");
        return SCAL_E_ARG;
    }
    SCAL_TRY(check_scan(p, xyz, n));
    return push(p, nullptr, &xyz, &n, stride_bytes, true);
}

extern "C" int scal_pipeline_pop(scal_pipeline_t* p, scal_pipeline_result* out) {
    if (!p || !out || p->S != 1) {
        set_error("scal_pipeline_pop: bad argument (a pipeline of several sequences takes scal_pipeline_pop_multi)");
        return SCAL_E_ARG;
    }
    return pop(p, out);
}

extern "C" int scal_pipeline_pop_multi(scal_pipeline_t* p, scal_pipeline_result* out) {
    if (!p || !out) {
        set_error("scal_pipeline_pop_multi: null argument");
        return SCAL_E_ARG;
    }
    return pop(p, out);
}

extern "C" int scal_pipeline_drain(scal_pipeline_t* p) {
    if (!p) return SCAL_E_ARG;
    std::unique_lock<std::mutex> lk(p->mu);
    if (p->err) return report(p);
    if (p->drained) return SCAL_OK;
    p->drain_req = true;
    p->pop_waiting++;
    p->cv.notify_all();
    p->cv.wait(lk, [&] { return p->err || (p->drained && (!p->sc_on() || p->d_coll == p->pushed) && p->verify_idle()); });
    p->pop_waiting--;
    if (p->err) return report(p);
    return SCAL_OK;
}

extern "C" int scal_pipeline_pop_loop(scal_pipeline_t* p, scal_pipeline_loop* out, int wait) {
    if (!p || !out) {
        set_error("scal_pipeline_pop_loop: null argument");
        return SCAL_E_ARG;
    }
    std::unique_lock<std::mutex> lk(p->mu);
    if (!p->kf_mode()) {
        set_error("scal_pipeline_pop_loop: only in sc_mode 3");
        return SCAL_E_STATE;
    }
    for (;;) {
        if (p->err) return report(p);
        if (!p->loops.empty()) {
            *out = p->loops.front();
            p->loops.pop_front();
            p->loops_owed--;
            return 1;
        }
        if (!wait || p->verify_idle()) return 0;
        p->cv.wait(lk);
    }
}

extern "C" int scal_pipeline_keyframe(scal_pipeline_t* p, int kf, double pose6[6], float* xyzi, int cap, int* n) {
    if (!p || !pose6 || !n || cap < 0 || (cap > 0 && !xyzi)) {
        set_error("scal_pipeline_keyframe: bad argument");
        return SCAL_E_ARG;
    }
    std::lock_guard<std::mutex> lk(p->mu);
    if (p->err) return report(p);
    if (!p->kf_mode() || !p->drained || p->d_coll != p->pushed || !p->verify_idle()) {
        set_error("scal_pipeline_keyframe: only in sc_mode 3, while the pipeline is drained");
        return SCAL_E_STATE;
    }
    return p->kf->read(kf, pose6, xyzi, cap, n);
}

static int update_poses_locked(scal_pipeline_t* p, const int* kf, const double* pose6, int n);

extern "C" int scal_pipeline_update_keyframe_poses(scal_pipeline_t* p, const int* kf, const double* pose6, int n) {
    if (!p || n < 0 || (n > 0 && (!kf || !pose6))) {
        set_error("scal_pipeline_update_keyframe_poses: bad argument");
        return SCAL_E_ARG;
    }
    std::lock_guard<std::mutex> lk(p->mu);
    if (p->err) return report(p);
    if (!p->kf_mode()) {
        set_error("scal_pipeline_update_keyframe_poses: only in sc_mode 3");
        return SCAL_E_STATE;
    }
    return update_poses_locked(p, kf, pose6, n);
}

static int update_poses_locked(scal_pipeline_t* p, const int* kf, const double* pose6, int n) {
    long long floor = p->d_coll;
    if (!p->jobs.empty()) floor = std::min(floor, p->jobs.front().seq);
    if (p->verifying) floor = std::min(floor, p->verifying_seq);
    return p->kf->update_poses(kf, pose6, n, p->pushed, floor);
}

static int pgo_map_state(scal_pipeline_t* p) {
    std::lock_guard<std::mutex> lk(p->mu);
    if (p->err) return report(p);
    if (!p->kf_mode() || p->cfg.pgo_map_max_points == 0) {
        set_error("scal_pipeline_pgo_map: only in sc_mode 3 with pgo_map_max_points > 0");
        return SCAL_E_STATE;
    }
    return SCAL_OK;
}

extern "C" int scal_pipeline_pgo_map(scal_pipeline_t* p, int kf_end, int skip, float leaf, float* out_xyzi, long long cap, long long* n_out) {
    if (!p || !n_out || cap < 0 || (cap > 0 && !out_xyzi)) {
        set_error("scal_pipeline_pgo_map: bad argument");
        return SCAL_E_ARG;
    }
    *n_out = 0;
    SCAL_TRY(pgo_map_state(p));
    if (!(leaf > 0.f) || !std::isfinite(leaf) || skip < 1 || kf_end < 0) {
        set_error("scal_pipeline_pgo_map: leaf must be finite and > 0, skip >= 1, kf_end >= 0");
        return SCAL_E_ARG;
    }
    return p->kf->pgo_map(kf_end, skip, leaf, out_xyzi, cap, n_out);
}

extern "C" const float* scal_pipeline_pgo_map_device(scal_pipeline_t* p, long long* n) {
    if (n) *n = 0;
    if (!p || !n || !p->kf_mode() || p->cfg.pgo_map_max_points == 0) return nullptr;
    return p->kf->pgo_map_device(n);
}

namespace {
void pose7_from6(const double* p6, double* p7) {
    const double cr = std::cos(p6[3] / 2), sr = std::sin(p6[3] / 2), cp = std::cos(p6[4] / 2), sp = std::sin(p6[4] / 2);
    const double cy = std::cos(p6[5] / 2), sy = std::sin(p6[5] / 2);
    p7[0] = sr * cp * cy - cr * sp * sy, p7[1] = cr * sp * cy + sr * cp * sy, p7[2] = cr * cp * sy - sr * sp * cy, p7[3] = cr * cp * cy + sr * sp * sy;
    p7[4] = p6[0], p7[5] = p6[1], p7[6] = p6[2];
}
void pose7_between(const double* a, const double* b, double* o) {
    const double x = -a[0], y = -a[1], z = -a[2], w = a[3];
    o[0] = w * b[0] + x * b[3] + y * b[2] - z * b[1];
    o[1] = w * b[1] - x * b[2] + y * b[3] + z * b[0];
    o[2] = w * b[2] + x * b[1] - y * b[0] + z * b[3];
    o[3] = w * b[3] - x * b[0] - y * b[1] - z * b[2];
    const double d[3] = {b[4] - a[4], b[5] - a[5], b[6] - a[6]};
    const double R[3][3] = {{1 - 2 * (y * y + z * z), 2 * (x * y - w * z), 2 * (x * z + w * y)},
                            {2 * (x * y + w * z), 1 - 2 * (x * x + z * z), 2 * (y * z - w * x)},
                            {2 * (x * z - w * y), 2 * (y * z + w * x), 1 - 2 * (x * x + y * y)}};
    for (int r = 0; r < 3; ++r) o[4 + r] = (R[r][0] * d[0] + R[r][1] * d[1]) + R[r][2] * d[2];
}
}

extern "C" int scal_pipeline_optimize_keyframes(scal_pipeline_t* p, int kf_end, int apply, int* kf_ids, double* pose6, int cap, scal_pipeline_pgo_result* res) {
    if (res) std::memset(res, 0, sizeof *res);
    if (!p || cap < 0 || (cap > 0 && (!kf_ids || !pose6))) {
        set_error("scal_pipeline_optimize_keyframes: bad argument");
        return SCAL_E_ARG;
    }
    {
        std::lock_guard<std::mutex> lk(p->mu);
        if (p->err) return report(p);
        if (!p->kf_mode()) {
            set_error("scal_pipeline_optimize_keyframes: only in sc_mode 3");
            return SCAL_E_STATE;
        }
    }
    if (kf_end < 0) {
        set_error("scal_pipeline_optimize_keyframes: kf_end must be >= 0");
        return SCAL_E_ARG;
    }
    std::vector<int> ids;
    std::vector<std::array<double, 6>> gated, current;
    SCAL_TRY(p->kf->pgo_snapshot(kf_end, &ids, &gated, &current));
    const int n = static_cast<int>(ids.size());
    if (res) res->n_nodes = n;
    if (cap < n) {
        set_error("scal_pipeline_optimize_keyframes: %d keyframes, room for %d", n, cap);
        return SCAL_E_CAPACITY;
    }
    if (n == 0) return SCAL_OK;
    std::vector<scal_pipeline::AcceptedLoop> loops;
    {
        std::unique_lock<std::mutex> lk(p->mu);
        const int need = ids.back() + 1;
        auto pending = [&] {
            if (p->verifying && p->verifying_kf < kf_end) return true;
            for (const KfLoopJob& j : p->jobs)
                if (j.curr_kf < kf_end) return true;
            return false;
        };
        p->cv.wait(lk, [&] { return p->err || p->stop || (p->kf_passed_end >= need && !pending()); });
        if (p->err) return report(p);
        if (p->stop) {
            set_error("scal_pipeline_optimize_keyframes: the pipeline is being destroyed");
            return SCAL_E_STATE;
        }
        for (const auto& a : p->accepted)
            if (a.curr_kf < kf_end) loops.push_back(a);
    }
    std::vector<double> x7(7 * static_cast<size_t>(n)), g7(7 * static_cast<size_t>(n));
    scal_posegraph_stats st{};
    {
        std::lock_guard<std::mutex> map_lk(p->kf->map_mu);
// ... 64 lines not shown
```

Before: 4530.

## Add prep stream for odometry/map input gathering with multi-buffered target sets

Splits odometry input preparation (gathering features into SoA, building ring tables and cell indices for the last-scan targets) into a separate prep step on its own lane, with triple-buffered target sets and double-buffered query sets so the next scan's prep can overlap the current solve. The map prefetch gather likewise moves to a prep stream. By default the prep lane resolves to the same lane as before (PREP_HOME), and an env var selects a side lane. The change adds extra device buffers and event dependencies, and with the default placement the cross-stage overlap is limited.

```diff
diff --git a/sc-a-loam_amd/csrc/common.cpp b/sc-a-loam_amd/csrc/common.cpp
--- a/sc-a-loam_amd/csrc/common.cpp
+++ b/sc-a-loam_amd/csrc/common.cpp
@@ -250,6 +250,12 @@
     return (stage == STAGE_ODOM || stage == STAGE_SC) ? 3 : stage == STAGE_MAP ? 4 : (stage == STAGE_SC_FILTER || stage == STAGE_MAP_PREFETCH) ? 1 : 0;
 }
 
+int prep_lane(StreamLayout layout, int placement, int home_stage) {
+    const int before = stage_lane(layout, home_stage == STAGE_ODOM ? STAGE_ODOM : STAGE_FEATURES);
+    if (layout == StreamLayout::Shared || placement != PREP_SIDE) return before;
+    return stage_lane(layout, STAGE_MAP_PREFETCH);
+}
+
 __global__ void k_queue_ptr(unsigned long long* out) { out[0] = reinterpret_cast<unsigned long long>(__builtin_amdgcn_queue_ptr()); }
 
 int lane_queue(int device, int lane, unsigned long long* out) {
diff --git a/sc-a-loam_amd/csrc/common.hpp b/sc-a-loam_amd/csrc/common.hpp
--- a/sc-a-loam_amd/csrc/common.hpp
+++ b/sc-a-loam_amd/csrc/common.hpp
@@ -36,11 +36,13 @@
 enum class StreamLayout { Shared, PerStage };
 enum { STAGE_FEATURES = 0, STAGE_SC = 1, STAGE_ODOM = 3, STAGE_MAP = 4, STAGE_MAP_PREFETCH = 2, STAGE_SC_FILTER = 5 };
 int stage_lane(StreamLayout layout, int stage);
+constexpr int PREP_HOME = 0, PREP_SIDE = 1;
+int prep_lane(StreamLayout layout, int placement, int home_stage);
 StreamLayout default_stream_layout();
 int acquire_stream(int device, hipStream_t* out, int lane = 0);
 void release_stream(int device, int lane = 0);
-int odom_create(const scal_odom_config* cfg, StreamLayout layout, scal_odom_t** out);
-int map_create(const scal_map_config* cfg, StreamLayout layout, scal_map_t** out);
+int odom_create(const scal_odom_config* cfg, StreamLayout layout, scal_odom_t** out, int prep_placement = PREP_HOME);
+int map_create(const scal_map_config* cfg, StreamLayout layout, scal_map_t** out, int prep_placement = PREP_HOME);
 int sc_create(const scal_sc_config* cfg, StreamLayout layout, scal_sc_t** out);
 int icp_create_on_lane(const scal_icp_config* cfg, int lane, scal_icp_t** out);
 int refine_create_on_lane(const scal_refine_config* cfg, int lane, scal_refine_t** out);
diff --git a/sc-a-loam_amd/csrc/mapping.hip b/sc-a-loam_amd/csrc/mapping.hip
--- a/sc-a-loam_amd/csrc/mapping.hip
+++ b/sc-a-loam_amd/csrc/mapping.hip
@@ -1342,6 +1342,7 @@
     scal_map_config cfg;
     LaneStream stream;
     LaneStream side;
+    LaneStream prep;
     static constexpr int NSETS = 8;
     static constexpr int MAX_STEPS = 4;
     static constexpr int MAX_PF = 3;
@@ -1411,7 +1412,7 @@
     }
 };
 
-int scal::map_create(const scal_map_config* cfg, StreamLayout layout, scal_map_t** out) {
+int scal::map_create(const scal_map_config* cfg, StreamLayout layout, scal_map_t** out, int prep_placement) {
     if (!cfg || !out || cfg->max_scan_points <= 0 || cfg->max_map_points <= 0 || !(cfg->line_res > 0) || !(cfg->plane_res > 0)) {
         set_error("scal_map_create: bad argument");
         return SCAL_E_ARG;
@@ -1487,6 +1488,7 @@
         rc = SCAL_E_HIP;
     if (rc == SCAL_OK) rc = c->stream.acquire(c->cfg.device, stage_lane(layout, STAGE_MAP));
     if (rc == SCAL_OK) rc = c->side.acquire(c->cfg.device, stage_lane(layout, STAGE_MAP_PREFETCH));
+    if (rc == SCAL_OK) rc = c->prep.acquire(c->cfg.device, prep_lane(layout, prep_placement, STAGE_MAP));
     for (int k = 0; k < scal_map::NSLOTS && rc == SCAL_OK; ++k) {
         rc = c->ev_pose[k].create(hipEventDisableTiming);
         if (rc == SCAL_OK) rc = c->ev_done[k].create(hipEventDisableTiming);
@@ -1517,6 +1519,7 @@
     (void)hipSetDevice(c->cfg.device);
     if (c->stream) (void)op_stream_synchronize(c->stream);
     if (c->side) (void)op_stream_synchronize(c->side);
+    if (c->prep) (void)op_stream_synchronize(c->prep);
     delete c;
 }
 
@@ -2191,12 +2194,14 @@
     InputSet& I = c->sets[nset];
     SCAL_TRY(I.ev_pre.ensure(EV_DEVICE_ONLY));
     SCAL_TRY(I.ev_pre_a.ensure(EV_DEVICE_ONLY));
-    hipStream_t sa = v.stream;
+    hipStream_t sa = c->prep;
+    SCAL_TRY(features_wait_done(feat, sa));
     const int nbc = std::max(1, div_up(ls_cap, 256));
     SCAL_LAUNCH("k_map_gather", k_map_gather, dim3(nbc + std::max(1, div_up(cap, 256))), dim3(256), 0, sa, v.less_xyzi, &v.P->n_less_sharp,
                      CSoA4{v.lfx, v.lfy, v.lfz, v.lfi}, &v.P->n_less_flat, I.in[0].v(), I.in[1].v(), I.C.p, c->scan_cap, nbc, I.surf_parts.p);
     SCAL_HIP(hipGetLastError());
     SCAL_TRY(enqueue_stack_filter(c, 0, c->vf_corner, sa, ls_cap, nset));
+    SCAL_TRY(features_note_reader(feat, sa));
     SCAL_HIP(op_event_record(I.ev_pre_a, sa));
     c->pf_half.push(scal_map::Prefetch{feat, nset, v.generation});
     return SCAL_OK;
@@ -2218,7 +2223,7 @@
     const scal_map::Prefetch h = c->pf_half.front();
     c->pf_half.pop();
     InputSet& I = c->sets[h.set];
-    SCAL_HIP(op_stream_wait_event(c->side, I.ev_pre_a, 0));
+    if (c->side.s != c->prep.s) SCAL_HIP(op_stream_wait_event(c->side, I.ev_pre_a, 0));
     SCAL_TRY(enqueue_stack_filter(c, 1, c->vf_side, c->side, cap, h.set, true));
     SCAL_HIP(op_event_record(I.ev_pre, c->side));
     c->pf.push(h);
diff --git a/sc-a-loam_amd/csrc/odometry.hip b/sc-a-loam_amd/csrc/odometry.hip
--- a/sc-a-loam_amd/csrc/odometry.hip
+++ b/sc-a-loam_amd/csrc/odometry.hip
@@ -10,10 +10,8 @@
 namespace scal {
 
 struct OdomCounters {
-    int n_corner_last, n_surf_last;
-    int n_sharp, n_flat, n_less_sharp, n_less_flat;
+    int n_sharp, n_flat;
     int n_slots, enable;
-    int n_live[2], n_edge[2], n_plane[2];
 };
 
 __device__ __forceinline__ float sqdist(float ax, float ay, float az, float bx, float by, float bz) {
@@ -90,7 +88,7 @@
 }
 
 __device__ __forceinline__ void k_odom_assoc_body(const CSoA4& sharp, const CSoA4& flat, const CSoA4& CL, const CSoA4& SL, const LMState* __restrict__ st, OdomCounters* C,
-                                                    int outer, const FactorSoA& f, const CellIndex& ci_corner, const CellIndex& ci_surf,
+                                                    const int* __restrict__ n_last, int outer, const FactorSoA& f, const CellIndex& ci_corner, const CellIndex& ci_surf,
                                                     const int* __restrict__ ring_tab) {
     if (!C->enable) return;
     const int ns = C->n_sharp, nf = C->n_flat;
@@ -103,7 +101,7 @@
     const int j = is_edge ? q : q - ns;
     const CSoA4& Q = is_edge ? sharp : flat;
     const CSoA4& T = is_edge ? CL : SL;
-    const int nT = is_edge ? C->n_corner_last : C->n_surf_last;
+    const int nT = n_last[is_edge ? 0 : 1];
     double x7[7];
 #pragma unroll
     for (int k = 0; k < 7; ++k) x7[k] = st->x[k];
@@ -255,56 +253,59 @@
 }
 SCAL_KERNEL(256, k_odom_assoc)
 
+constexpr int N_QSETS = 2;
+constexpr int N_TSETS = 3;
+
 __device__ __forceinline__ void k_odom_init_pose_body(LMState* st, int* ring_tab) {
     if (threadIdx.x == 0) {
         st->x[0] = st->x[1] = st->x[2] = 0.0, st->x[3] = 1.0;
         st->x[4] = st->x[5] = st->x[6] = 0.0;
     }
-    for (int t = threadIdx.x; t < 8 * RING_TAB; t += blockDim.x) ring_tab[t] = ((t / RING_TAB) & 1) ? -1 : 0x7f7f7f7f;
+    for (int t = threadIdx.x; t < N_TSETS * 4 * RING_TAB; t += blockDim.x) ring_tab[t] = ((t / RING_TAB) & 1) ? -1 : 0x7f7f7f7f;
 }
 SCAL_KERNEL(1024, k_odom_init_pose)
-struct HandoverArgs {
-    CSoA4 in[2];
-    const int* d_n[2];
-    SoA4 out[2];
-    int* d_n_out[2];
-    int cap[2];
-    int nb0;
+struct OdomGatherArgs {
+    const float* aos[4];
+    CSoA4 soa[4];
+    const int* d_n[4];
+    int cap[4];
+    SoA4 out[4];
+    int* n_last;
+    int nbs, nb0;
     int* tab_write;
-    int* tab_reset;
-    const LMState* st;
-    LMState* host_st;
-    const LMSync* sync;
     int* cell_cnt[2][OD_LEVELS];
     int* cell_rank[2][OD_LEVELS];
 };
-__device__ __forceinline__ void k_odom_handover_body(const HandoverArgs& a) {
+__device__ __forceinline__ void k_odom_gather_body(const OdomGatherArgs& a, OdomCounters* C) {
     int b = blockIdx.x;
-    const int k = b < a.nb0 ? 0 : 1;
-    if (k) b -= a.nb0;
-    if (blockIdx.x == 0) {
-        for (int t = threadIdx.x; t < 4 * RING_TAB; t += 256) a.tab_reset[t] = ((t / RING_TAB) & 1) ? -1 : 0x7f7f7f7f;
-        const unsigned* src = reinterpret_cast<const unsigned*>(a.st);
-        unsigned* dst = reinterpret_cast<unsigned*>(a.host_st);
-        const bool abandoned = a.sync->abandoned != 0;
-        constexpr int TERM_WORD = static_cast<int>(offsetof(LMState, termination) / 4);
-        for (int t = threadIdx.x; t < static_cast<int>(sizeof(LMState) / 4); t += 256) dst[t] = (abandoned && t == TERM_WORD) ? 5u : src[t];
-    }
+    int w = 0;
+    if (b >= 2 * a.nbs + a.nb0) w = 3, b -= 2 * a.nbs + a.nb0;
+    else if (b >= 2 * a.nbs) w = 2, b -= 2 * a.nbs;
+    else if (b >= a.nbs) w = 1, b -= a.nbs;
+    if (blockIdx.x == 0 && threadIdx.x == 0) C->n_slots = 0, C->enable = 1;
+    const int n = min(*a.d_n[w], a.cap[w]);
+    const int i = b * 256 + threadIdx.x;
+    if (i == 0) *(w == 0 ? &C->n_sharp : w == 1 ? &C->n_flat : a.n_last + (w - 2)) = n;
+    if (b * 256 >= n) return;
+    const int lane = lane_id();
+    const SoA4 out = a.out[w];
+    float x = 0, y = 0, z = 0, pw = 0;
+    if (i < n) {
+        if (a.aos[w]) {
+            const float4 p = reinterpret_cast<const float4*>(a.aos[w])[i];
+            x = p.x, y = p.y, z = p.z, pw = p.w;
+        } else {
+            const CSoA4 in = a.soa[w];
+            x = in.x[i], y = in.y[i], z = in.z[i], pw = in.w[i];
+        }
+        out.x[i] = x, out.y[i] = y, out.z[i] = z, out.w[i] = pw;
+    }
+    if (w < 2) return;
+    const int k = w - 2;
     int* first_idx = a.tab_write + 2 * k * RING_TAB;
     int* last_idx = first_idx + RING_TAB;
-    const CSoA4 in = a.in[k];
-    const SoA4 out = a.out[k];
-    const int n = min(*a.d_n[k], a.cap[k]);
-    const int i = b * 256 + threadIdx.x;
-    if (i == 0) *a.d_n_out[k] = n;
-    if (b * 256 >= n) return;
-    const int lane = lane_id();
-    float x = 0, y = 0, z = 0;
     if (i < n) {
-        const float w = in.w[i];
-        x = in.x[i], y = in.y[i], z = in.z[i];
-        out.x[i] = x, out.y[i] = y, out.z[i] = z, out.w[i] = w;
-        const int r = min(max(static_cast<int>(w), 0), RING_TAB - 1);
+        const int r = min(max(static_cast<int>(pw), 0), RING_TAB - 1);
         const int rp = __shfl_up(r, 1, 64);
         const int rn = __shfl_down(r, 1, 64);
         if (lane == 0 || rp != r) atomicMin(&first_idx[r], i);
@@ -326,7 +327,7 @@
         if (i < n) a.cell_rank[k][l][i] = base + (lane - head);
     }
 }
-SCAL_KERNEL(256, k_odom_handover)
+SCAL_KERNEL(256, k_odom_gather)
 constexpr int OD_START_STRIDE = OD_H + 4;
 __device__ __forceinline__ void k_odom_cellscan_body(int* cnt_all, int* start_all) {
     constexpr int PER = OD_H / 1024;
@@ -370,7 +371,7 @@
 SCAL_KERNEL(1024, k_odom_cellscan)
 struct CellFillArgs {
     CSoA4 in[2];
-    const int* d_n[2];
+    const int* n_last;
     const int* rank[2][OD_LEVELS];
     const int* start[2][OD_LEVELS];
     float4* pts[2][OD_LEVELS];
@@ -381,52 +382,22 @@
     const int k = b < a.nb0 ? 0 : 1;
     if (k) b -= a.nb0;
     const int i = b * 256 + threadIdx.x;
-    if (i >= *a.d_n[k]) return;
+    if (i >= a.n_last[k]) return;
     const float x = a.in[k].x[i], y = a.in[k].y[i], z = a.in[k].z[i];
     const float4 rec = make_float4(x, y, z, __uint_as_float(static_cast<unsigned>(i)));
 #pragma unroll
     for (int l = 0; l < OD_LEVELS; ++l) a.pts[k][l][a.start[k][l][od_bucket(x, y, z, l)] + a.rank[k][l][i]] = rec;
 }
 SCAL_KERNEL(256, k_odom_cellfill)
-struct OdomGatherArgs {
-    const float *sharp, *flat, *less;
-    CSoA4 less_flat;
-    const int *n_sharp, *n_flat, *n_less, *n_less_flat;
-    SoA4 o_sharp, o_flat, o_less, o_less_flat;
-    int slot_cap, feat_cap, cap, nbs, nbf;
-};
-__device__ __forceinline__ void k_odom_gather_body(const OdomGatherArgs& a, OdomCounters* C) {
-    int b = blockIdx.x;
-    const float* aos = nullptr;
-    const int* d_n;
-    int* d_n_out;
-    SoA4 out;
-    int cap;
-    if (b < a.nbs) {
-        aos = a.sharp, d_n = a.n_sharp, d_n_out = &C->n_sharp, out = a.o_sharp, cap = a.slot_cap;
-        if (b == 0 && threadIdx.x == 0) {
-            C->n_slots = 0, C->enable = 1;
-            C->n_live[0] = C->n_live[1] = C->n_edge[0] = C->n_edge[1] = C->n_plane[0] = C->n_plane[1] = 0;
-        }
-    } else if (b < 2 * a.nbs) {
-        b -= a.nbs, aos = a.flat, d_n = a.n_flat, d_n_out = &C->n_flat, out = a.o_flat, cap = a.slot_cap;
-    } else if (b < 2 * a.nbs + a.nbf) {
-        b -= 2 * a.nbs, aos = a.less, d_n = a.n_less, d_n_out = &C->n_less_sharp, out = a.o_less, cap = a.feat_cap;
-    } else {
-        b -= 2 * a.nbs + a.nbf, d_n = a.n_less_flat, d_n_out = &C->n_less_flat, out = a.o_less_flat, cap = a.cap;
-    }
-    const int n = min(*d_n, cap);
-    const int i = b * 256 + threadIdx.x;
-    if (i == 0) *d_n_out = n;
-    if (i >= n) return;
-    if (aos) {
-        const float4 p = reinterpret_cast<const float4*>(aos)[i];
-        out.x[i] = p.x, out.y[i] = p.y, out.z[i] = p.z, out.w[i] = p.w;
-    } else {
-        out.x[i] = a.less_flat.x[i], out.y[i] = a.less_flat.y[i], out.z[i] = a.less_flat.z[i], out.w[i] = a.less_flat.w[i];
-    }
-}
-SCAL_KERNEL(256, k_odom_gather)
+__device__ __forceinline__ void k_odom_handover_body(const LMState* st, LMState* host_st, const LMSync* sync, int* tab_reset) {
+    for (int t = threadIdx.x; t < 4 * RING_TAB; t += 256) tab_reset[t] = ((t / RING_TAB) & 1) ? -1 : 0x7f7f7f7f;
+    const unsigned* src = reinterpret_cast<const unsigned*>(st);
+    unsigned* dst = reinterpret_cast<unsigned*>(host_st);
+    const bool abandoned = sync->abandoned != 0;
+    constexpr int TERM_WORD = static_cast<int>(offsetof(LMState, termination) / 4);
+    for (int t = threadIdx.x; t < static_cast<int>(sizeof(LMState) / 4); t += 256) dst[t] = (abandoned && t == TERM_WORD) ? 5u : src[t];
+}
+SCAL_KERNEL(256, k_odom_handover)
 
 }
 
@@ -434,7 +405,8 @@
 
 struct scal_odom {
     scal_odom_config cfg;
-    LaneStream stream;
+    LaneStream stream, prep;
+    bool own_prep = false;
     int cap = 0, feat_cap = 0;
     bool systemInited = false;
     static constexpr int MAX_STEPS = 4;
@@ -444,35 +416,41 @@
     };
     std::deque<Pending> pending;
     Event ev[MAX_STEPS];
-    int next_slot = 0;
+    Event ev_prep;
+    long long n_prep = 0;
+    long long cur = 0;
     double q_w_curr[4] = {0, 0, 0, 1}, t_w_curr[3] = {0, 0, 0};
     DevBuf<float> aos;
-    SoAStore sharp, flat, less_sharp, less_flat;
-    SoAStore corner_last, surf_last;
+    SoAStore sharp[N_QSETS], flat[N_QSETS];
+    SoAStore corner_last[N_TSETS], surf_last[N_TSETS];
+    DevBuf<int> n_last;
+    SoAStore up[4];
+    DevBuf<int> up_n;
     LMStore lm;
     DevBuf<int> cell_cnt, cell_start, cell_rank;
     DevBuf<float4> cell_pts;
     int* cell_cnt_of(int k, int l) const { return cell_cnt.p + (k * OD_LEVELS + l) * OD_H; }
-    int* cell_start_of(int k, int l) const { return cell_start.p + (k * OD_LEVELS + l) * OD_START_STRIDE; }
+    int* cell_start_of(int t, int k, int l) const { return cell_start.p + ((t * 2 + k) * OD_LEVELS + l) * OD_START_STRIDE; }
     int* cell_rank_of(int k, int l) const { return cell_rank.p + (size_t)l * (feat_cap + cap) + (k ? feat_cap : 0); }
-    float4* cell_pts_of(int k, int l) const { return cell_pts.p + (size_t)l * (feat_cap + cap) + (k ? feat_cap : 0); }
-    CellIndex cell_index(int k) const {
+    float4* cell_pts_of(int t, int k, int l) const { return cell_pts.p + ((size_t)t * OD_LEVELS + l) * (feat_cap + cap) + (k ? feat_cap : 0); }
+    CellIndex cell_index(int t, int k) const {
         CellIndex ci;
-        for (int l = 0; l < OD_LEVELS; ++l) ci.start[l] = cell_start_of(k, l), ci.pts[l] = cell_pts_of(k, l);
+        for (int l = 0; l < OD_LEVELS; ++l) ci.start[l] = cell_start_of(t, k, l), ci.pts[l] = cell_pts_of(t, k, l);
         return ci;
     }
     DevBuf<int> ring_tab;
-    int tab_cur = 0;
+    int* ring_tab_of(int t) const { return ring_tab.p + t * 4 * RING_TAB; }
+    int* n_last_of(int t) const { return n_last.p + 2 * t; }
     DevBuf<OdomCounters> d_C;
     PinBuf<LMState> h_st;
-    PinBuf<OdomCounters> h_up;
+    PinBuf<int> h_up;
     HostStage hs;
     bool adapter_active = false, adapter_solve = false;
     BlockAdapter blocks;
     int outer_next = 0;
 };
 
-int scal::odom_create(const scal_odom_config* cfg, StreamLayout layout, scal_odom_t** out) {
+int scal::odom_create(const scal_odom_config* cfg, StreamLayout layout, scal_odom_t** out, int prep_placement) {
     if (!cfg || !out || cfg->max_points <= 0) {
         set_error("scal_odom_create: bad argument");
         return SCAL_E_ARG;
@@ -487,20 +465,25 @@
     auto A = [&](int r) { if (rc == SCAL_OK) rc = r; };
     A(c->lm.alloc(36 * 64));
     A(c->aos.alloc((size_t)c->cap * 4));
-    A(c->sharp.alloc(c->lm.slot_cap)); A(c->flat.alloc(c->lm.slot_cap));
-    A(c->less_sharp.alloc(c->feat_cap)); A(c->corner_last.alloc(c->feat_cap));
-    A(c->less_flat.alloc(c->cap)); A(c->surf_last.alloc(c->cap));
-    A(c->cell_cnt.alloc(2 * OD_LEVELS * OD_H)); A(c->cell_start.alloc(2 * OD_LEVELS * OD_START_STRIDE));
-    A(c->cell_rank.alloc(OD_LEVELS * ((size_t)c->feat_cap + c->cap))); A(c->cell_pts.alloc(OD_LEVELS * ((size_t)c->feat_cap + c->cap)));
-    A(c->ring_tab.alloc(8 * RING_TAB));
+    for (int q = 0; q < N_QSETS; ++q) { A(c->sharp[q].alloc(c->lm.slot_cap)); A(c->flat[q].alloc(c->lm.slot_cap)); }
+    for (int t = 0; t < N_TSETS; ++t) { A(c->corner_last[t].alloc(c->feat_cap)); A(c->surf_last[t].alloc(c->cap)); }
+    A(c->up[0].alloc(c->lm.slot_cap)); A(c->up[1].alloc(c->lm.slot_cap)); A(c->up[2].alloc(c->feat_cap)); A(c->up[3].alloc(c->cap));
+    A(c->n_last.alloc(2 * N_TSETS)); A(c->up_n.alloc(4));
+    A(c->cell_cnt.alloc(2 * OD_LEVELS * OD_H)); A(c->cell_start.alloc(N_TSETS * 2 * OD_LEVELS * OD_START_STRIDE));
+    A(c->cell_rank.alloc(OD_LEVELS * ((size_t)c->feat_cap + c->cap))); A(c->cell_pts.alloc(N_TSETS * OD_LEVELS * ((size_t)c->feat_cap + c->cap)));
+    A(c->ring_tab.alloc(N_TSETS * 4 * RING_TAB));
     A(c->blocks.alloc(c->lm.slot_cap));
-    A(c->d_C.alloc(1)); A(c->h_st.alloc(scal_odom::MAX_STEPS)); A(c->h_up.alloc(1));
+    A(c->d_C.alloc(N_QSETS)); A(c->h_st.alloc(scal_odom::MAX_STEPS)); A(c->h_up.alloc(4));
     if (rc == SCAL_OK) rc = lm_check_residency<LMNoHook, LMNoHook>(c->cfg.device);
     if (rc == SCAL_OK) rc = c->stream.acquire(c->cfg.device, stage_lane(layout, STAGE_ODOM));
+    if (rc == SCAL_OK) rc = c->prep.acquire(c->cfg.device, prep_lane(layout, prep_placement, STAGE_ODOM));
+    c->own_prep = c->prep.s != c->stream.s;
     for (int k = 0; k < scal_odom::MAX_STEPS && rc == SCAL_OK; ++k) rc = c->ev[k].create(hipEventDisableTiming);
+    if (rc == SCAL_OK) rc = c->ev_prep.create(EV_DEVICE_ONLY);
     if (rc == SCAL_OK) {
         rc = c->lm.init(c->stream);
-        if (rc == SCAL_OK && op_memset_async(c->d_C.p, 0, sizeof(OdomCounters), c->stream) != hipSuccess) rc = SCAL_E_HIP;
+        if (rc == SCAL_OK && op_memset_async(c->d_C.p, 0, N_QSETS * sizeof(OdomCounters), c->stream) != hipSuccess) rc = SCAL_E_HIP;
+        if (rc == SCAL_OK) rc = c->n_last.zero(c->stream);
         if (rc == SCAL_OK) rc = c->cell_cnt.zero(c->stream);
         if (rc == SCAL_OK) rc = c->cell_start.zero(c->stream);
         SCAL_LAUNCH("k_odom_init_pose", k_odom_init_pose, dim3(1), dim3(256), 0, c->stream, c->lm.d_st.p, c->ring_tab.p);
@@ -520,70 +503,85 @@
 extern "C" void scal_odom_destroy(scal_odom_t* c) {
     if (!c) return;
     (void)hipSetDevice(c->cfg.device);
+    if (c->prep) (void)op_stream_synchronize(c->prep);
     if (c->stream) (void)op_stream_synchronize(c->stream);
     delete c;
 }
 
 namespace {
 
-int launch_handover(scal_odom* c, int slot, hipEvent_t ev);
+struct OdomInputs {
+    const float* aos[4];
+    CSoA4 soa[4];
+    const int* d_n[4];
+    int less_flat_cap;
+};
+
+int odom_prep(scal_odom* c, const OdomInputs& in, scal_features_t* feat) {
+    hipStream_t s = c->prep;
+    const long long k = c->n_prep;
+    const int q = static_cast<int>(k % N_QSETS), t = static_cast<int>(k % N_TSETS);
+    if (c->own_prep && k >= 2) SCAL_HIP(op_stream_wait_event(s, c->ev[(k - 2) % scal_odom::MAX_STEPS], 0));
+    OdomGatherArgs a;
+    for (int w = 0; w < 4; ++w) a.aos[w] = in.aos[w], a.soa[w] = in.soa[w], a.d_n[w] = in.d_n[w];
+    a.cap[0] = a.cap[1] = c->lm.slot_cap, a.cap[2] = c->feat_cap, a.cap[3] = std::min(c->cap, in.less_flat_cap);
+    a.out[0] = c->sharp[q].v(), a.out[1] = c->flat[q].v(), a.out[2] = c->corner_last[t].v(), a.out[3] = c->surf_last[t].v();
+    a.n_last = c->n_last_of(t);
+    a.nbs = std::max(1, div_up(c->lm.slot_cap, 256)), a.nb0 = std::max(1, div_up(c->feat_cap, 256));
+    a.tab_write = c->ring_tab_of(t);
+    for (int kk = 0; kk < 2; ++kk)
+        for (int l = 0; l < OD_LEVELS; ++l) a.cell_cnt[kk][l] = c->cell_cnt_of(kk, l), a.cell_rank[kk][l] = c->cell_rank_of(kk, l);
+    const int nb_target = a.nb0 + std::max(1, div_up(c->cap, 256));
+    SCAL_LAUNCH("k_odom_gather", k_odom_gather, dim3(2 * a.nbs + nb_target), dim3(256), 0, s, a, c->d_C.p + q);
+    SCAL_LAUNCH("k_odom_cellscan", k_odom_cellscan, dim3(2 * OD_LEVELS), dim3(1024), 0, s, c->cell_cnt.p, c->cell_start_of(t, 0, 0));
+    CellFillArgs f;
+    f.in[0] = c->corner_last[t].cv(), f.in[1] = c->surf_last[t].cv();
+    f.n_last = c->n_last_of(t);
+    for (int kk = 0; kk < 2; ++kk)
+        for (int l = 0; l < OD_LEVELS; ++l) f.rank[kk][l] = c->cell_rank_of(kk, l), f.start[kk][l] = c->cell_start_of(t, kk, l), f.pts[kk][l] = c->cell_pts_of(t, kk, l);
+    f.nb0 = a.nb0;
+    SCAL_LAUNCH("k_odom_cellfill", k_odom_cellfill, dim3(nb_target), dim3(256), 0, s, f);
+    SCAL_HIP(hipGetLastError());
+    if (feat) SCAL_TRY(features_note_reader(feat, s));
+    if (c->own_prep) {
+        SCAL_HIP(op_event_record(c->ev_prep, s));
+        SCAL_HIP(op_stream_wait_event(c->stream, c->ev_prep, 0));
+    }
+    c->cur = k;
+    c->n_prep = k + 1;
+    return SCAL_OK;
+}
+
+int launch_assoc(scal_odom* c, int outer) {
+    const int q = static_cast<int>(c->cur % N_QSETS), t = static_cast<int>((c->cur + N_TSETS - 1) % N_TSETS);
+    OdomCounters* C = c->d_C.p + q;
+    SCAL_LAUNCH("k_odom_assoc", k_odom_assoc, dim3(std::max(1, c->lm.slot_cap)), dim3(256), 0, c->stream, c->sharp[q].cv(), c->flat[q].cv(), c->corner_last[t].cv(),
+                     c->surf_last[t].cv(), c->lm.d_st.p, C, c->n_last_of(t), outer, c->lm.factors(), c->cell_index(t, 0), c->cell_index(t, 1), c->ring_tab_of(t));
+    return SCAL_OK;
+}
+
+int launch_handover(scal_odom* c, bool solve) {
+    const int slot = static_cast<int>(c->cur % scal_odom::MAX_STEPS);
+    SCAL_LAUNCH("k_odom_handover", k_odom_handover, dim3(1), dim3(256), 0, c->stream, c->lm.d_st.p, c->h_st.p + slot, c->lm.lm_sync.p,
+                     c->ring_tab_of(static_cast<int>((c->cur + N_TSETS - 1) % N_TSETS)));
+    SCAL_HIP(hipGetLastError());
+    SCAL_HIP(op_event_record(c->ev[slot], c->stream));
+    c->pending.push_back({slot, solve});
+    return SCAL_OK;
+}
+
 int odom_enqueue(scal_odom* c) {
     hipStream_t s = c->stream;
-    OdomCounters* C = c->d_C.p;
-    LMState* st = c->lm.d_st.p;
-    FactorSoA F = c->lm.factors();
+    OdomCounters* C = c->d_C.p + c->cur % N_QSETS;
     const bool solve = c->systemInited;
     c->systemInited = true;
-    const int slot = c->next_slot;
-    c->next_slot = (c->next_slot + 1) % scal_odom::MAX_STEPS;
     if (solve) {
         for (int outer = 0; outer < 2; ++outer) {
-            {
-                SCAL_LAUNCH("k_odom_assoc", k_odom_assoc, dim3(std::max(1, c->lm.slot_cap)), dim3(256), 0, s, c->sharp.cv(), c->flat.cv(),
-                                   c->corner_last.cv(), c->surf_last.cv(), st, C, outer, F, c->cell_index(0), c->cell_index(1), c->ring_tab.p + c->tab_cur * 4 * RING_TAB);
-            }
-            {
-                                launch_lm_solve(s, F, &C->n_slots, st, &C->enable, c->lm.partials.p, c->lm.lm_sync.p, outer, nullptr, LMNoHook(), LMNoHook(), "k_lm_solve_odom");
-            }
-        }
-    }
-    SCAL_TRY(launch_handover(c, slot, c->ev[slot]));
-    c->pending.push_back({slot, solve});
-    return SCAL_OK;
-}
-
-int launch_handover(scal_odom* c, int slot, hipEvent_t ev) {
-    hipStream_t s = c->stream;
-    OdomCounters* C = c->d_C.p;
-    LMState* st = c->lm.d_st.p;
-    {
-        HandoverArgs h;
-        h.in[0] = c->less_sharp.cv(), h.in[1] = c->less_flat.cv();
-        h.d_n[0] = &C->n_less_sharp, h.d_n[1] = &C->n_less_flat;
-        h.out[0] = c->corner_last.v(), h.out[1] = c->surf_last.v();
-        h.d_n_out[0] = &C->n_corner_last, h.d_n_out[1] = &C->n_surf_last;
-        h.cap[0] = c->feat_cap, h.cap[1] = c->cap;
-        h.nb0 = std::max(1, div_up(c->feat_cap, 256));
-        h.tab_write = c->ring_tab.p + (c->tab_cur ^ 1) * 4 * RING_TAB;
-        h.tab_reset = c->ring_tab.p + c->tab_cur * 4 * RING_TAB;
-        h.st = st, h.host_st = c->h_st.p + slot, h.sync = c->lm.lm_sync.p;
-        for (int k = 0; k < 2; ++k)
-            for (int l = 0; l < OD_LEVELS; ++l) h.cell_cnt[k][l] = c->cell_cnt_of(k, l), h.cell_rank[k][l] = c->cell_rank_of(k, l);
-        const dim3 grid(h.nb0 + std::max(1, div_up(c->cap, 256)));
-        SCAL_LAUNCH("k_odom_handover", k_odom_handover, grid, dim3(256), 0, s, h);
-        c->tab_cur ^= 1;
-        if (ev) SCAL_HIP(op_event_record(ev, s));
-        SCAL_LAUNCH("k_odom_cellscan", k_odom_cellscan, dim3(2 * OD_LEVELS), dim3(1024), 0, s, c->cell_cnt.p, c->cell_start.p);
-        CellFillArgs f;
-        f.in[0] = c->corner_last.cv(), f.in[1] = c->surf_last.cv();
-        f.d_n[0] = &C->n_corner_last, f.d_n[1] = &C->n_surf_last;
-        for (int k = 0; k < 2; ++k)
-            for (int l = 0; l < OD_LEVELS; ++l) f.rank[k][l] = c->cell_rank_of(k, l), f.start[k][l] = c->cell_start_of(k, l), f.pts[k][l] = c->cell_pts_of(k, l);
-        f.nb0 = h.nb0;
-        SCAL_LAUNCH("k_odom_cellfill", k_odom_cellfill, grid, dim3(256), 0, s, f);
-    }
-    SCAL_HIP(hipGetLastError());
-    return SCAL_OK;
+            SCAL_TRY(launch_assoc(c, outer));
+            launch_lm_solve(s, c->lm.factors(), &C->n_slots, c->lm.d_st.p, &C->enable, c->lm.partials.p, c->lm.lm_sync.p, outer, nullptr, LMNoHook(), LMNoHook(), "k_lm_solve_odom");
+        }
+    }
+    return launch_handover(c, solve);
 }
 
 int odom_collect(scal_odom* c, double* q_lc, double* t_lc, double* q_w, double* t_w, scal_odom_stats* stats) {
@@ -628,30 +626,23 @@
 }
 
 static int odom_upload(scal_odom* c, const float* sharp, int n_sharp, const float* less_sharp, int n_less_sharp, const float* flat, int n_flat,
-                       const float* less_flat, int n_less_flat) {
-    hipStream_t s = c->stream;
+                       const float* less_flat, int n_less_flat, OdomInputs* in) {
+    hipStream_t s = c->prep;
     SCAL_HIP(op_stream_synchronize(s));
     c->hs.finish();
     (void)c->hs.reserve(((size_t)2 * c->lm.slot_cap + c->feat_cap + c->cap) * 16 + 4096);
-    OdomCounters& H = *c->h_up.p;
-    OdomCounters fresh;
-    std::memset(&fresh, 0, sizeof fresh);
-    fresh.n_sharp = n_sharp, fresh.n_flat = n_flat, fresh.n_less_sharp = n_less_sharp, fresh.n_less_flat = n_less_flat, fresh.enable = 1;
-    H = fresh;
-    const size_t off = offsetof(OdomCounters, n_sharp);
-    SCAL_HIP(op_memcpy_async(reinterpret_cast<char*>(c->d_C.p) + off, reinterpret_cast<char*>(&H) + off, sizeof(OdomCounters) - off,
-                            hipMemcpyHostToDevice, s));
-    auto up = [&](const float* src, int n, SoAStore& dst) -> int {
-        if (n > 0) {
-            SCAL_HIP(c->hs.h2d(c->aos.p, src, sizeof(float) * 4 * n, s));
-            launch_deinterleave(s, c->aos.p, n, dst.v());
-        }
-        return SCAL_OK;
-    };
-    SCAL_TRY(up(sharp, n_sharp, c->sharp));
-    SCAL_TRY(up(flat, n_flat, c->flat));
-    SCAL_TRY(up(less_sharp, n_less_sharp, c->less_sharp));
-    SCAL_TRY(up(less_flat, n_less_flat, c->less_flat));
+    const float* src[4] = {sharp, flat, less_sharp, less_flat};
+    const int n[4] = {n_sharp, n_flat, n_less_sharp, n_less_flat};
+    for (int w = 0; w < 4; ++w) c->h_up.p[w] = n[w];
+    SCAL_HIP(op_memcpy_async(c->up_n.p, c->h_up.p, 4 * sizeof(int), hipMemcpyHostToDevice, s));
+    for (int w = 0; w < 4; ++w) {
+        if (n[w] > 0) {
+            SCAL_HIP(c->hs.h2d(c->aos.p, src[w], sizeof(float) * 4 * n[w], s));
+            launch_deinterleave(s, c->aos.p, n[w], c->up[w].v());
+        }
+        in->aos[w] = nullptr, in->soa[w] = c->up[w].cv(), in->d_n[w] = c->up_n.p + w;
+    }
+    in->less_flat_cap = c->cap;
     return SCAL_OK;
 }
 
@@ -673,7 +664,9 @@
         set_error("scal_odom_step: a queued step has not been collected");
         return SCAL_E_STATE;
     }
-    SCAL_TRY(odom_upload(c, sharp, n_sharp, less_sharp, n_less_sharp, flat, n_flat, less_flat, n_less_flat));
+    OdomInputs in;
+    SCAL_TRY(odom_upload(c, sharp, n_sharp, less_sharp, n_less_sharp, flat, n_flat, less_flat, n_less_flat, &in));
+    SCAL_TRY(odom_prep(c, in, nullptr));
     SCAL_TRY(odom_enqueue(c));
     return odom_collect(c, q_lc, t_lc, q_w, t_w, stats);
 }
@@ -693,17 +686,13 @@
         return SCAL_E_ARG;
     }
     SCAL_HIP(hipSetDevice(c->cfg.device));
-    hipStream_t s = c->stream;
-    OdomGatherArgs a;
-    a.sharp = v.sharp_xyzi, a.flat = v.flat_xyzi, a.less = v.less_xyzi;
-    a.less_flat = CSoA4{v.lfx, v.lfy, v.lfz, v.lfi};
-    a.n_sharp = &v.P->n_sharp, a.n_flat = &v.P->n_flat, a.n_less = &v.P->n_less_sharp, a.n_less_flat = &v.P->n_less_flat;
-    a.o_sharp = c->sharp.v(), a.o_flat = c->flat.v(), a.o_less = c->less_sharp.v(), a.o_less_flat = c->less_flat.v();
-    a.slot_cap = c->lm.slot_cap, a.feat_cap = c->feat_cap, a.cap = std::min(c->cap, v.cap);
-    a.nbs = std::max(1, div_up(c->lm.slot_cap, 256)), a.nbf = std::max(1, div_up(c->feat_cap, 256));
-    SCAL_TRY(features_wait_done(feat, s));
-    SCAL_LAUNCH("k_odom_gather", k_odom_gather, dim3(2 * a.nbs + a.nbf + std::max(1, div_up(a.cap, 256))), dim3(256), 0, s, a, c->d_C.p);
-    SCAL_TRY(features_note_reader(feat, s));
+    OdomInputs in;
+    in.aos[0] = v.sharp_xyzi, in.aos[1] = v.flat_xyzi, in.aos[2] = v.less_xyzi, in.aos[3] = nullptr;
+    for (int w = 0; w < 4; ++w) in.soa[w] = CSoA4{v.lfx, v.lfy, v.lfz, v.lfi};
+    in.d_n[0] = &v.P->n_sharp, in.d_n[1] = &v.P->n_flat, in.d_n[2] = &v.P->n_less_sharp, in.d_n[3] = &v.P->n_less_flat;
+    in.less_flat_cap = v.cap;
+    SCAL_TRY(features_wait_done(feat, c->prep));
+    SCAL_TRY(odom_prep(c, in, feat));
     return odom_enqueue(c);
 }
 
@@ -744,7 +733,9 @@
     SCAL_HIP(hipSetDevice(c->cfg.device));
     hipStream_t s = c->stream;
     SCAL_HIP(op_stream_synchronize(s));
-    SCAL_TRY(odom_upload(c, sharp, n_sharp, less_sharp, n_less_sharp, flat, n_flat, less_flat, n_less_flat));
+    OdomInputs in;
+    SCAL_TRY(odom_upload(c, sharp, n_sharp, less_sharp, n_less_sharp, flat, n_flat, less_flat, n_less_flat, &in));
+    SCAL_TRY(odom_prep(c, in, nullptr));
     SCAL_HIP(op_memcpy_async(c->h_st.p, c->lm.d_st.p, sizeof(LMState), hipMemcpyDeviceToHost, s));
     SCAL_HIP(op_stream_synchronize(s));
     for (int i = 0; i < 4; ++i) q_last_curr[i] = c->h_st.p->x[i];
@@ -768,12 +759,10 @@
     }
     SCAL_HIP(hipSetDevice(c->cfg.device));
     hipStream_t s = c->stream;
-    OdomCounters* C = c->d_C.p;
-    LMState* st = c->lm.d_st.p;
+    OdomCounters* C = c->d_C.p + c->cur % N_QSETS;
     FactorSoA F = c->lm.factors();
     SCAL_TRY(c->blocks.set_pose(c->stream, c->lm.d_st.p->x, q_last_curr, t_last_curr));
-    SCAL_LAUNCH("k_odom_assoc", k_odom_assoc, dim3(std::max(1, c->lm.slot_cap)), dim3(256), 0, s, c->sharp.cv(), c->flat.cv(), c->corner_last.cv(),
-                     c->surf_last.cv(), st, C, std::min(c->outer_next, 1), F, c->cell_index(0), c->cell_index(1), c->ring_tab.p + c->tab_cur * 4 * RING_TAB);
+    SCAL_TRY(launch_assoc(c, std::min(c->outer_next, 1)));
     c->outer_next++;
     SCAL_TRY(c->blocks.compact(s, F, &C->n_slots));
     SCAL_HIP(op_stream_synchronize(s));
@@ -819,10 +808,7 @@
     SCAL_HIP(hipSetDevice(c->cfg.device));
     c->adapter_active = false;
     SCAL_TRY(c->blocks.set_pose(c->stream, c->lm.d_st.p->x, q_last_curr, t_last_curr));
-    const int slot = c->next_slot;
-    c->next_slot = (c->next_slot + 1) % scal_odom::MAX_STEPS;
-    SCAL_TRY(launch_handover(c, slot, c->ev[slot]));
-    c->pending.push_back({slot, c->adapter_solve});
+    SCAL_TRY(launch_handover(c, c->adapter_solve));
     double q_lc[4], t_lc[3];
     return odom_collect(c, q_lc, t_lc, q_w_curr, t_w_curr, nullptr);
 }
diff --git a/sc-a-loam_amd/csrc/pipeline.cpp b/sc-a-loam_amd/csrc/pipeline.cpp
--- a/sc-a-loam_amd/csrc/pipeline.cpp
+++ b/sc-a-loam_amd/csrc/pipeline.cpp
@@ -26,6 +26,7 @@
 }
 const int B_AHEAD = env_int("SCALOAM_PIPE_B_AHEAD", 2, 1, 3);
 const int PF_AHEAD = env_int("SCALOAM_PIPE_PF_AHEAD", 3, 1, 3);
+const int PREP_LANE = env_int("SCALOAM_PIPE_PREP_LANE", PREP_HOME, PREP_HOME, PREP_SIDE);
 
 const bool TIMING = env_int("SCALOAM_PIPE_TIMING", 0, 0, 1) != 0;
 struct HostTimer {
@@ -167,7 +168,7 @@
             p->a_run = k + 1;
             p->cv.notify_all();
             lk.unlock();
-            st = p->tm_front.run(1, "C: prefetch, lane 0 half", [&] { return p->for_all([&](int q) { return scal_map_prefetch_begin(p->mp[q], p->regs[q][slot]); }); });
+            st = p->tm_front.run(1, "C: prefetch, prep half", [&] { return p->for_all([&](int q) { return scal_map_prefetch_begin(p->mp[q], p->regs[q][slot]); }); });
         }
         lk.lock();
         if (st != SCAL_OK) {
@@ -544,13 +545,13 @@
         if (rc == SCAL_OK) {
             scal_odom_config oc{};
             oc.max_points = cfg->max_points, oc.device = cfg->device;
-            rc = odom_create(&oc, StreamLayout::PerStage, &p->od[q]);
+            rc = odom_create(&oc, StreamLayout::PerStage, &p->od[q], PREP_LANE);
         }
         if (rc == SCAL_OK) {
             scal_map_config mc{};
             mc.line_res = cfg->line_res, mc.plane_res = cfg->plane_res, mc.max_scan_points = cfg->max_points, mc.max_map_points = cfg->max_map_points;
             mc.device = cfg->device;
-            rc = map_create(&mc, StreamLayout::PerStage, &p->mp[q]);
+            rc = map_create(&mc, StreamLayout::PerStage, &p->mp[q], PREP_LANE);
         }
         if (rc == SCAL_OK && p->sc_on()) {
             scal_sc_config sc{};
```

New measurement: 4438. -2.0%, worse.
